# QWTforGithub/CDSegNet

Hardware: AMD Instinct MI355X
Metric: points/sec/node (ScanNet ~120k-pt scenes, 1-step) (higher is better)
Workload: dtype f16

## Files before the change

### cdsegnet_amd/csrc/attention.hip

```cpp
#include <cstdlib>
#include <mutex>
#include <type_traits>

#include "common.h"
#include "prof.h"

namespace {

constexpr int ATTN_ZONES = 5;
constexpr int ATTN_STORE8 = 1 << 30;

struct AttnP {
  const void* q;
  const void* k;
  const void* v;
  const int32_t* q_gidx;
  const int32_t* kv_gidx;
  const int32_t* widx;
  const int32_t* patch_start;
  void* out;
  int ldq, ldk, ldv, ldo;
  int num_heads;
  int num_patches;
  float scale_log2e;
  int flags;
  int nzones;
  int zcnt[ATTN_ZONES];
  int zsplit[ATTN_ZONES];
  int full_patches;
  int zfixed;
  int bulk_max;
};

__host__ __device__ __forceinline__ bool decode_block(const AttnP& p, int B, int& patch, int& head, int& qslice, int& qsplit) {
  const int U = p.num_patches * p.num_heads;
  const int xcd = B & 7;
  int t = B >> 3;
  const int u0 = (int)(((long)U * xcd) >> 3), u1 = (int)(((long)U * (xcd + 1)) >> 3);
  int j0 = 0;
  for (int z = 0; z < p.nzones; ++z) {
    const int fixed = p.zcnt[z];
    const int cnt = fixed >= 0 ? fixed : (u1 - u0) - p.zfixed;
    const int ext = fixed >= 0 ? fixed : p.bulk_max;
    const int split = p.zsplit[z];
    const int nb = ext * split;
    if (t < nb) {
      const int jl = t / split;
      if (jl >= cnt) return false;
      const int u = u0 + j0 + jl;
      patch = u / p.num_heads;
      head = u - patch * p.num_heads;
      qslice = t - jl * split;
      qsplit = split;
      return true;
    }
    t -= nb;
    j0 += cnt;
  }
  return false;
}

constexpr int VT_STRIDE_F32 = 4128;
constexpr int KS_BYTES_F32 = 1024 * 64;
constexpr int SMEM_F32 = KS_BYTES_F32 + 16 * VT_STRIDE_F32;

#ifndef ATTN_FIRST_STATIC
#define ATTN_FIRST_STATIC 1
#endif
#ifndef ATTN_PRIO_OUTSIDE
#define ATTN_PRIO_OUTSIDE 1
#endif
#ifndef ATTN_STORE16
#define ATTN_STORE16 1
#endif
#ifndef ATTN_LEAD_BLOCKS
#define ATTN_LEAD_BLOCKS 0
#endif
#ifndef ATTN_TAIL1_BLOCKS
#define ATTN_TAIL1_BLOCKS 64
#endif
#ifndef ATTN_TAIL2_BLOCKS
#define ATTN_TAIL2_BLOCKS 64
#endif
#ifndef ATTN_ZONE_MIN_UNITS
#define ATTN_ZONE_MIN_UNITS 96
#endif
constexpr int ATTN_THREADS = 512;
constexpr int ATTN_WAVES = ATTN_THREADS / 64;
constexpr int ATTN_RUN = 8;
#ifndef ATTN_BF16_WAVES
#define ATTN_BF16_WAVES 8
#endif
#ifndef ATTN_TILES_IN_FLIGHT
#define ATTN_TILES_IN_FLIGHT 2
#endif
constexpr int BF_WAVES = ATTN_BF16_WAVES, BF_THREADS = 64 * BF_WAVES;
static_assert(BF_WAVES >= ATTN_RUN && BF_WAVES <= 12, "the first run of a block's tiles is pre-assigned to waves 0 .. 7");
constexpr int BF_WAVES_WIDE = 16;
constexpr int KV_STAGE = 1024 * 32;
constexpr int ONES_BYTES = 2048;
constexpr int SMEM_BF16 = 2 * KV_STAGE + ONES_BYTES + 64 + 4096;

__device__ uint4 g_attn_zero[2];

#ifdef CDSEG_ATTN_TIMING
__device__ unsigned long long g_attn_t[8 * 8 * 4096];
#define ATTN_STAMP(x) const unsigned long long x = __builtin_readcyclecounter()
#else
#define ATTN_STAMP(x)
#endif

typedef __attribute__((ext_vector_type(4))) short s16x4_t;
typedef __attribute__((address_space(3))) s16x4_t lds_s16x4_t;

__device__ __forceinline__ f32x16_t qk_tile(const char* k_lane, bf16x8_t qf, const f32x16_t& c0) {
  const bf16x8_t kf = *reinterpret_cast<const bf16x8_t*>(k_lane);
  return mfma_32x32x16_bf16(kf, qf, c0);
}

__device__ __forceinline__ float tile_max(const f32x16_t& s, float m) {
  const float a = fmaxf(fmaxf(s[0], s[1]), s[2]);
  const float b = fmaxf(fmaxf(s[3], s[4]), s[5]);
  const float c = fmaxf(fmaxf(s[6], s[7]), s[8]);
  const float d = fmaxf(fmaxf(s[9], s[10]), s[11]);
  const float e = fmaxf(fmaxf(s[12], s[13]), s[14]);
  return fmaxf(fmaxf(fmaxf(a, b), fmaxf(c, d)), fmaxf(fmaxf(e, s[15]), m));
}

template <bool TAIL, bool FIRST = false>
__device__ __forceinline__ void pv_tile(const f32x16_t& s, int kt, int h, int L, unsigned va, f32x16_t& o) {
  float pr[16];
#pragma unroll
  for (int r = 0; r < 16; ++r) pr[r] = __builtin_amdgcn_exp2f(s[r]);
  if (TAIL) {
#pragma unroll
    for (int r = 0; r < 16; ++r)
      if (kt * 32 + (r & 3) + 8 * (r >> 2) + 4 * h >= L) pr[r] = 0.f;
  }
#pragma unroll
  for (int mf = 0; mf < 2; ++mf) {
    union { bf16x8_t v; uint32_t u[4]; } pf;
#pragma unroll
    for (int j = 0; j < 4; ++j) pf.u[j] = pack_truebf16x2(pr[8 * mf + 2 * j], pr[8 * mf + 2 * j + 1]);
    const s16x4_t v0 = __builtin_amdgcn_ds_read_tr16_b64_v4i16(reinterpret_cast<lds_s16x4_t*>(va + 512 * mf));
    const s16x4_t v1 = __builtin_amdgcn_ds_read_tr16_b64_v4i16(reinterpret_cast<lds_s16x4_t*>(va + 512 * mf + 256));
    const bf16x8_t vf = __builtin_shufflevector(v0, v1, 0, 1, 2, 3, 4, 5, 6, 7);
    if (FIRST && mf == 0) {
      const f32x16_t z = {0, 0, 0, 0, 0, 0, 0, 0, 0, 0, 0, 0, 0, 0, 0, 0};
      o = mfma_32x32x16_truebf16(vf, pf.v, z);
    } else {
      o = mfma_32x32x16_truebf16(vf, pf.v, o);
    }
  }
}

__device__ __forceinline__ float sq8_bf16(const uint4& a) {
  float t = dot2_bf16(a.x, a.x, 0.f);
  t = dot2_bf16(a.y, a.y, t);
  t = dot2_bf16(a.z, a.z, t);
  return dot2_bf16(a.w, a.w, t);
}

template <int WAVES>
__global__ __launch_bounds__(64 * WAVES, 4) void attn_bf16_kernel(AttnP p) {
  constexpr int BF_WAVES = WAVES, BF_THREADS = 64 * WAVES;
  constexpr int NPC = 32 / WAVES;
  extern __shared__ __attribute__((aligned(16))) char smem[];
  char* Ks = smem;
  unsigned* s_next = reinterpret_cast<unsigned*>(smem + 2 * KV_STAGE + ONES_BYTES + 48);
  int* s_qidx = reinterpret_cast<int*>(smem + 2 * KV_STAGE + ONES_BYTES + 64);
  const unsigned lds_base = (unsigned)(uintptr_t)(__attribute__((address_space(3))) char*)smem;

  const int tid = threadIdx.x;
  const int lane = tid & 63;
  const int wave = __builtin_amdgcn_readfirstlane(tid >> 6);
  int patch, head, qslice, qsplit;
  if (!decode_block(p, (int)blockIdx.x, patch, head, qslice, qsplit)) return;
#ifdef CDSEG_ATTN_TIMING
  const unsigned long long rt0 = __builtin_amdgcn_s_memrealtime();
  unsigned long long t_loop = 0, t_first = 0, t_epi = 0, n_tiles = 0;
#endif
  ATTN_STAMP(t0);
  __builtin_amdgcn_s_setprio(3);
  const int ps = p.patch_start[patch];
  const int L = p.patch_start[patch + 1] - ps;
  const int nkt = (L + 31) >> 5;
  const bf16_t* kb = (const bf16_t*)p.k + head * 16;
  const bf16_t* vb = (const bf16_t*)p.v + head * 16;

  const int ql = lane & 31;
  const int h = lane >> 5;
  const int nqt = nkt;
  auto claim = [&]() {
    for (;;) {
      unsigned i = 0;
      if (lane == 0) i = atomicAdd(s_next, 1u);
      i = __builtin_amdgcn_readfirstlane(i);
      if (ATTN_FIRST_STATIC && qsplit == 1) {
        const int t = (int)(i + i / 3u + 1u);
        return t < nqt ? t : -1;
      }
      const int base = (qslice + (int)(i >> 3) * qsplit) * ATTN_RUN;
      if (base >= nqt) return -1;
      const int t = base + (int)(i & 7);
      if (t < nqt) return t;
    }
  };
  auto load_qrow = [&](int t) {
    const int g = s_qidx[min(max(t, 0) * 32 + ql, L - 1)];
    return *reinterpret_cast<const uint4*>((const bf16_t*)p.q + (long)g * p.ldq + head * 16 + h * 8);
  };

  int qt_first = -1;
  uint4 q_first = make_uint4(0, 0, 0, 0);
  {
    const int kip = lane >> 1, hs = lane & 1;
    int gk[NPC];
#pragma unroll
    for (int i = 0; i < NPC; ++i) {
      const int s = (wave + BF_WAVES * i) * 32 + kip;
      gk[i] = s < L ? p.kv_gidx[ps + s] : -1;
    }
    int gq[2] = {0, 0};
    if (wave < ATTN_RUN) {
#pragma unroll
      for (int i = 0; i < 2; ++i) gq[i] = p.q_gidx[ps + min(wave * 128 + i * 64 + lane, L - 1)];
    }
    const int qt_slice0 = qslice * ATTN_RUN + wave;
    int gfirst = 0;
    if (ATTN_FIRST_STATIC && qsplit > 1 && wave < ATTN_RUN) gfirst = p.q_gidx[ps + min(qt_slice0 * 32 + ql, L - 1)];
    if (tid == 0) *s_next = (ATTN_FIRST_STATIC && qsplit > 1) ? 8u : 0u;
    const void* ksrc[NPC];
    const void* vsrc[NPC];
#pragma unroll
    for (int i = 0; i < NPC; ++i) {
      const int s = (wave + BF_WAVES * i) * 32 + kip;
      ksrc[i] = vsrc[i] = (const char*)g_attn_zero + hs * 16;
      if (gk[i] >= 0) {
        ksrc[i] = kb + (long)gk[i] * p.ldk + ((hs ^ ((s >> 3) & 1)) << 3);
        vsrc[i] = vb + (long)gk[i] * p.ldv + (hs << 3);
      }
      asm volatile("" : "+v"(ksrc[i]), "+v"(vsrc[i]));
    }
#pragma unroll
    for (int i = 0; i < NPC; ++i) {
      const int pc = wave + BF_WAVES * i;
      if (pc < nkt) {
        dma16(ksrc[i], lds_base + pc * 1024);
        dma16(vsrc[i], lds_base + KV_STAGE + pc * 1024);
      }
    }
    if (ATTN_FIRST_STATIC && qsplit == 1 && 4 * wave < nqt) {
      qt_first = 4 * wave;
      const int g = __shfl(gq[0], lane & 31, 64);
      q_first = *reinterpret_cast<const uint4*>((const bf16_t*)p.q + (long)g * p.ldq + head * 16 + h * 8);
    } else if (ATTN_FIRST_STATIC && qsplit > 1 && wave < ATTN_RUN && qt_slice0 < nqt) {
      qt_first = qt_slice0;
      q_first = *reinterpret_cast<const uint4*>((const bf16_t*)p.q + (long)gfirst * p.ldq + head * 16 + h * 8);
    }
    if (wave < ATTN_RUN) {
#pragma unroll
      for (int i = 0; i < 2; ++i) s_qidx[wave * 128 + i * 64 + lane] = gq[i];
    }
    for (int w = tid; w < ONES_BYTES / 8; w += BF_THREADS)
      *reinterpret_cast<uint2*>(smem + 2 * KV_STAGE + w * 8) = make_uint2(0x3F80u, 0u);
    asm volatile("s_waitcnt vmcnt(0)" ::: "memory");
    if (LP_IS_F16 && !(p.flags & CDSEG_ATTN_V_BF16)) {
#pragma unroll
      for (int i = 0; i < NPC; ++i) {
        const int pc = wave + BF_WAVES * i;
        if (pc < nkt) {
          uint4* vp = reinterpret_cast<uint4*>(smem + KV_STAGE + pc * 1024 + lane * 16);
          uint4 u = *vp;
          float a0, a1;
          unpack_bf16x2(u.x, a0, a1); u.x = pack_truebf16x2(a0, a1);
          unpack_bf16x2(u.y, a0, a1); u.y = pack_truebf16x2(a0, a1);
          unpack_bf16x2(u.z, a0, a1); u.z = pack_truebf16x2(a0, a1);
          unpack_bf16x2(u.w, a0, a1); u.w = pack_truebf16x2(a0, a1);
          *vp = u;
        }
      }
    }
    __syncthreads();
  }
  if (!ATTN_PRIO_OUTSIDE) __builtin_amdgcn_s_setprio(0);
  ATTN_STAMP(t1);
  const char* k_lane = Ks + ql * 32 + ((h ^ ((ql >> 3) & 1)) << 4);
  const bool v_lane = (lane & 16) == 0;
  const unsigned va0 = v_lane ? lds_base + KV_STAGE + (4 * h + ((lane & 15) >> 2)) * 32 + (lane & 3) * 8
                              : lds_base + 2 * KV_STAGE + (h ? 0 : 128);
  const unsigned vstep = v_lane ? 1024u : 0u;
  const float c = p.scale_log2e;
  const bool tail = (nkt << 5) != L;
  const int nfull = tail ? nkt - 1 : nkt;

  int qt = qt_first;
  uint4 q_cur = q_first;
  if (qt < 0) {
    qt = claim();
    q_cur = load_qrow(qt);
  }
  while (qt >= 0) {
    bf16x8_t qf;
    {
      union { bf16x8_t v; uint32_t u[4]; } qs;
      const uint32_t qr[4] = {q_cur.x, q_cur.y, q_cur.z, q_cur.w};
      if (p.flags & CDSEG_ATTN_Q_PRESCALED) {
#pragma unroll
        for (int j = 0; j < 4; ++j) qs.u[j] = qr[j];
      } else {
#pragma unroll
        for (int j = 0; j < 4; ++j) {
          float lo, hi;
          unpack_bf16x2(qr[j], lo, hi);
          qs.u[j] = pack_bf16x2(lo * c, hi * c);
        }
      }
      qf = qs.v;
      asm volatile("" : "+v"(qf));
    }
    const int qt_nxt = claim();
    const uint4 q_nxt = load_qrow(qt_nxt);
    const int qslot = qt * 32 + ql;
    const bool qvalid = qslot < L;
    int w = p.widx[ps + min(qslot, L - 1)];
    if (!qvalid) w = -1;
    const f32x16_t zero16 = {0, 0, 0, 0, 0, 0, 0, 0, 0, 0, 0, 0, 0, 0, 0, 0};
    auto exp_pv_pass = [&](auto shift_tag, float mrow) {
      constexpr bool SHIFT = decltype(shift_tag)::value;
      const float nm = SHIFT ? -mrow : 0.f;
      const f32x16_t negm = {nm, nm, nm, nm, nm, nm, nm, nm, nm, nm, nm, nm, nm, nm, nm, nm};
      const f32x16_t& c0 = SHIFT ? negm : zero16;
      f32x16_t acc;
      const char* kp = k_lane;
      unsigned va = va0;
      int kt;
      if (ATTN_TILES_IN_FLIGHT == 2 && nfull >= 2) {
        const f32x16_t sa = qk_tile(kp, qf, c0);
        const f32x16_t sb = qk_tile(kp + 1024, qf, c0);
        pv_tile<false, true>(sa, 0, h, L, va, acc);
        pv_tile<false>(sb, 1, h, L, va + 1024, acc);
        kp += 2048;
        va += 2 * vstep;
        kt = 2;
      } else {
        const f32x16_t s0 = qk_tile(kp, qf, c0);
        if (nfull == 0) pv_tile<true, true>(s0, 0, h, L, va, acc);
        else pv_tile<false, true>(s0, 0, h, L, va, acc);
        kp += 1024;
        va += vstep;
        kt = 1;
      }
      for (; ATTN_TILES_IN_FLIGHT == 2 && kt + 1 < nfull; kt += 2) {
        const f32x16_t sa = qk_tile(kp, qf, c0);
        const f32x16_t sb = qk_tile(kp + 1024, qf, c0);
        pv_tile<false>(sa, kt, h, L, va, acc);
        pv_tile<false>(sb, kt + 1, h, L, va + 1024, acc);
        kp += 2048;
        va += 2 * vstep;
      }
      for (; kt < nkt; ++kt) {
        const f32x16_t s = qk_tile(kp, qf, c0);
        if (kt >= nfull) pv_tile<true>(s, kt, h, L, va, acc);
        else pv_tile<false>(s, kt, h, L, va, acc);
        kp += 1024;
        va += vstep;
      }
      return acc;
    };
    if (ATTN_PRIO_OUTSIDE) __builtin_amdgcn_s_setprio(0);
    ATTN_STAMP(tl0);
    f32x16_t o = exp_pv_pass(std::false_type{}, 0.f);
    if (ATTN_PRIO_OUTSIDE) __builtin_amdgcn_s_setprio(2);
#ifdef CDSEG_ATTN_TIMING
    asm volatile("" :: "v"(o[0]), "v"(o[8]));
    const unsigned long long tl1 = __builtin_readcyclecounter();
    t_loop += tl1 - tl0;
    if (n_tiles == 0) t_first = tl0 - t1;
    ++n_tiles;
#endif
    {
      const float den = __shfl(o[8], ql, 64);
      bool fin = true;
#pragma unroll
      for (int r = 0; r < 8; ++r) fin = fin && __builtin_isfinite(o[r]);
      const bool redo = qvalid && (!(den >= 1e-30f && den <= 1e30f) || !fin);
      if (__any(redo)) {
        float m0 = -INFINITY;
        const char* kp = k_lane;
        for (int kt = 0; kt < nkt; ++kt, kp += 1024) {
          f32x16_t s = qk_tile(kp, qf, zero16);
          if (kt >= nfull) {
#pragma unroll
            for (int r = 0; r < 16; ++r)
              if (kt * 32 + (r & 3) + 8 * (r >> 2) + 4 * h >= L) s[r] = -INFINITY;
          }
          m0 = tile_max(s, m0);
        }
        m0 = fmaxf(m0, __shfl_xor(m0, 32, 64));
        o = exp_pv_pass(std::true_type{}, m0);
      }
    }
    const float lsum = __shfl(o[8], ql, 64);
    const float inv = 1.0f / lsum;
    {
      uint2 a, b;
      a.x = pack_bf16x2(o[0] * inv, o[1] * inv);
      a.y = pack_bf16x2(o[2] * inv, o[3] * inv);
      b.x = pack_bf16x2(o[4] * inv, o[5] * inv);
      b.y = pack_bf16x2(o[6] * inv, o[7] * inv);
      if (ATTN_STORE16 && !(p.flags & ATTN_STORE8)) {
        const auto sx = __builtin_amdgcn_permlane32_swap(a.x, b.x, false, false);
        const auto sy = __builtin_amdgcn_permlane32_swap(a.y, b.y, false, false);
        if (w >= 0) {
          bf16_t* orow = (bf16_t*)p.out + (long)w * p.ldo + head * 16 + 8 * h;
          *reinterpret_cast<uint4*>(orow) = make_uint4(sx[0], sy[0], sx[1], sy[1]);
        }
      } else if (w >= 0) {
        bf16_t* orow = (bf16_t*)p.out + (long)w * p.ldo + head * 16 + 4 * h;
        *reinterpret_cast<uint2*>(orow) = a;
        *reinterpret_cast<uint2*>(orow + 8) = b;
      }
    }
    qt = qt_nxt;
    q_cur = q_nxt;
#ifdef CDSEG_ATTN_TIMING
    asm volatile("s_waitcnt vmcnt(0)" ::: "memory");
    t_epi += __builtin_readcyclecounter() - tl1;
#endif
  }
#ifdef CDSEG_ATTN_TIMING
  if (lane == 0 && blockIdx.x < 4096) {
    unsigned long long* d = g_attn_t + ((size_t)blockIdx.x * 8 + wave) * 8;
    d[0] = rt0; d[1] = __builtin_amdgcn_s_memrealtime(); d[2] = t1 - t0; d[3] = t_loop;
    d[4] = __builtin_readcyclecounter() - t0;
    d[5] = t_first; d[6] = t_epi; d[7] = n_tiles;
  }
#endif
}

__global__ __launch_bounds__(ATTN_THREADS) void attn_f32_kernel(AttnP p) {
  extern __shared__ __attribute__((aligned(16))) char smem[];
  char* Ks = smem;
  char* Vt = smem + KS_BYTES_F32;

  const int tid = threadIdx.x;
  const int lane = tid & 63;
  const int wave = tid >> 6;
  int patch, head, qslice, qsplit;
  if (!decode_block(p, (int)blockIdx.x, patch, head, qslice, qsplit)) return;
  const int ps = p.patch_start[patch];
  const int L = p.patch_start[patch + 1] - ps;
  const int nkt = (L + 15) >> 4;
  const int Lp = nkt << 4;
  const float* kb = (const float*)p.k + head * 16;
  const float* vb = (const float*)p.v + head * 16;

  for (int s = tid; s < Lp; s += ATTN_THREADS) {
    uint4 kk[4], vv[4];
#pragma unroll
    for (int i = 0; i < 4; ++i) kk[i] = vv[i] = make_uint4(0, 0, 0, 0);
    if (s < L) {
      const long g = p.kv_gidx[ps + s];
      const uint4* kr = reinterpret_cast<const uint4*>(kb + g * p.ldk);
      const uint4* vr = reinterpret_cast<const uint4*>(vb + g * p.ldv);
#pragma unroll
      for (int i = 0; i < 4; ++i) { kk[i] = kr[i]; vv[i] = vr[i]; }
    }
    const int sw = (s >> 1) & 3;
#pragma unroll
    for (int i = 0; i < 4; ++i) *reinterpret_cast<uint4*>(Ks + s * 64 + ((i ^ sw) << 4)) = kk[i];
#pragma unroll
    for (int i = 0; i < 4; ++i) {
      *reinterpret_cast<uint32_t*>(Vt + (4 * i + 0) * VT_STRIDE_F32 + s * 4) = vv[i].x;
      *reinterpret_cast<uint32_t*>(Vt + (4 * i + 1) * VT_STRIDE_F32 + s * 4) = vv[i].y;
      *reinterpret_cast<uint32_t*>(Vt + (4 * i + 2) * VT_STRIDE_F32 + s * 4) = vv[i].z;
      *reinterpret_cast<uint32_t*>(Vt + (4 * i + 3) * VT_STRIDE_F32 + s * 4) = vv[i].w;
    }
  }
  __syncthreads();

  const int ql = lane & 15;
  const int g4 = lane >> 4;
  const float c = p.scale_log2e;
  const int nqt = (L + 15) >> 4;

  for (int qt = qslice * ATTN_WAVES + wave; qt < nqt; qt += qsplit * ATTN_WAVES) {
    const int qslot = qt * 16 + ql;
    const bool qvalid = qslot < L;
    f32x4_t qf = {0.f, 0.f, 0.f, 0.f};
    if (qvalid) {
      const long g = p.q_gidx[ps + qslot];
      qf = *reinterpret_cast<const f32x4_t*>((const float*)p.q + g * p.ldq + head * 16 + 4 * g4);
    }
    float mloc = -INFINITY;
    for (int kt = 0; kt < nkt; ++kt) {
      const int key = kt * 16 + ql;
      const f32x4_t kf = *reinterpret_cast<const f32x4_t*>(Ks + key * 64 + ((g4 ^ ((key >> 1) & 3)) << 4));
      f32x4_t s = {0.f, 0.f, 0.f, 0.f};
#pragma unroll
      for (int ss = 0; ss < 4; ++ss) s = __builtin_amdgcn_mfma_f32_16x16x4f32(kf[ss], qf[ss], s, 0, 0, 0);
#pragma unroll
      for (int r = 0; r < 4; ++r) {
        float sv = s[r];
        if (kt * 16 + 4 * g4 + r >= L) sv = -INFINITY;
        mloc = fmaxf(mloc, sv);
      }
    }
    float m = fmaxf(mloc, __shfl_xor(mloc, 16, 64));
    m = fmaxf(m, __shfl_xor(m, 32, 64));
    const float mc = m * c;
    f32x4_t o = {0.f, 0.f, 0.f, 0.f};
    float lloc = 0.f;
    for (int kt = 0; kt < nkt; ++kt) {
      const int key = kt * 16 + ql;
      const f32x4_t kf = *reinterpret_cast<const f32x4_t*>(Ks + key * 64 + ((g4 ^ ((key >> 1) & 3)) << 4));
      f32x4_t s = {0.f, 0.f, 0.f, 0.f};
#pragma unroll
      for (int ss = 0; ss < 4; ++ss) s = __builtin_amdgcn_mfma_f32_16x16x4f32(kf[ss], qf[ss], s, 0, 0, 0);
      const f32x4_t vf = *reinterpret_cast<const f32x4_t*>(Vt + ql * VT_STRIDE_F32 + (kt * 16 + 4 * g4) * 4);
#pragma unroll
      for (int r = 0; r < 4; ++r) {
        float pv = __builtin_amdgcn_exp2f(s[r] * c - mc);
        if (kt * 16 + 4 * g4 + r >= L) pv = 0.f;
        lloc += pv;
        o = __builtin_amdgcn_mfma_f32_16x16x4f32(vf[r], pv, o, 0, 0, 0);
      }
    }
    float l = lloc + __shfl_xor(lloc, 16, 64);
    l += __shfl_xor(l, 32, 64);
    const float inv = 1.0f / l;
    if (qvalid) {
      const int w = p.widx[ps + qslot];
      if (w >= 0) {
        float4 ov = make_float4(o[0] * inv, o[1] * inv, o[2] * inv, o[3] * inv);
        *reinterpret_cast<float4*>((float*)p.out + (long)w * p.ldo + head * 16 + 4 * g4) = ov;
      }
    }
  }
}


constexpr int X3_KH = 0, X3_KL = KV_STAGE, X3_V1 = 2 * KV_STAGE, X3_V2 = 3 * KV_STAGE;
constexpr int X3_ONES = 4 * KV_STAGE, X3_ZERO = X3_ONES + ONES_BYTES;
constexpr int SMEM_X3 = X3_ZERO + ONES_BYTES;
#ifndef ATTN_X3_WAVES
#define ATTN_X3_WAVES 8
#endif
#ifndef ATTN_X3_TILES
#define ATTN_X3_TILES 2
#endif
constexpr int X3_WAVES = ATTN_X3_WAVES, X3_THREADS = 64 * X3_WAVES, X3_TILES = ATTN_X3_TILES;
static_assert(X3_WAVES % ATTN_RUN == 0, "whole runs of query tiles per block");
typedef _Float16 x3h2_t __attribute__((ext_vector_type(2)));
typedef _Float16 x3h8_t __attribute__((ext_vector_type(8)));

__device__ __forceinline__ void x3_split_f16(float a, float b, uint32_t& hi, uint32_t& lo) {
  const hw_f32x2_t v = {__builtin_amdgcn_fmed3f(a, -65504.f, 65504.f), __builtin_amdgcn_fmed3f(b, -65504.f, 65504.f)};
  const x3h2_t hh = __builtin_convertvector(v, x3h2_t);
  const hw_f32x2_t r = v - __builtin_convertvector(hh, hw_f32x2_t);
  hi = __builtin_bit_cast(uint32_t, hh);
  lo = __builtin_bit_cast(uint32_t, __builtin_convertvector(r, x3h2_t));
}
__device__ __forceinline__ void x3_split_bf16(float a, float b, uint32_t& p1, uint32_t& p2) {
  p1 = pack_truebf16x2(a, b);
  p2 = pack_truebf16x2(a - __uint_as_float(p1 << 16), b - __uint_as_float(p1 & 0xffff0000u));
}
__device__ __forceinline__ f32x16_t x3_mfma_f16(bf16x8_t a, bf16x8_t b, f32x16_t c) {
  return __builtin_amdgcn_mfma_f32_32x32x16_f16(__builtin_bit_cast(x3h8_t, a), __builtin_bit_cast(x3h8_t, b), c, 0, 0, 0);
}

__device__ __forceinline__ f32x16_t x3_qk_tile(const char* k_lane, bf16x8_t qh, bf16x8_t ql, const f32x16_t& c0) {
  const bf16x8_t kh = *reinterpret_cast<const bf16x8_t*>(k_lane + X3_KH);
  const bf16x8_t kl = *reinterpret_cast<const bf16x8_t*>(k_lane + X3_KL);
  f32x16_t s = x3_mfma_f16(kh, qh, c0);
  s = x3_mfma_f16(kh, ql, s);
  return x3_mfma_f16(kl, qh, s);
}

template <bool TAIL, bool FIRST = false>
__device__ __forceinline__ void x3_pv_tile(const f32x16_t& s, int kt, int h, int L, unsigned va1, unsigned va2, f32x16_t& o) {
  float pr[16];
#pragma unroll
  for (int r = 0; r < 16; ++r) pr[r] = __builtin_amdgcn_exp2f(s[r]);
  if (TAIL) {
#pragma unroll
// ... 311 lines not shown
```

### cdsegnet_amd/csrc/deep.hip

```cpp
#include <atomic>

#include "deep.h"

namespace {

constexpr int DEEP_D = 4;

#ifdef CDSEG_DEEP_TIMING
__device__ unsigned long long g_deep_t[2048 * 16];
#define DT_STAMP(k) if (wave == 0 && lane == 0 && blockIdx.x < 2048) g_deep_t[blockIdx.x * 16 + (k)] = __builtin_readcyclecounter()
#else
#define DT_STAMP(k)
#endif

template <int NCH>
__device__ __forceinline__ int act_off(int row, int chunk) {
  return row * (NCH * 16) + ((chunk ^ (row & 15)) << 4);
}

__device__ __forceinline__ void lds_barrier() {
  asm volatile("s_waitcnt lgkmcnt(0)" ::: "memory");
  __builtin_amdgcn_s_barrier();
}

__device__ __forceinline__ uint4 pack8(const f32x4_t& a, const f32x4_t& b) {
  uint4 r;
  r.x = pack_bf16x2(a[0], a[1]); r.y = pack_bf16x2(a[2], a[3]);
  r.z = pack_bf16x2(b[0], b[1]); r.w = pack_bf16x2(b[2], b[3]);
  return r;
}
__device__ __forceinline__ uint4 pack8_truebf16(const f32x4_t& a, const f32x4_t& b) {
  uint4 r;
  r.x = pack_truebf16x2(a[0], a[1]); r.y = pack_truebf16x2(a[2], a[3]);
  r.z = pack_truebf16x2(b[0], b[1]); r.w = pack_truebf16x2(b[2], b[3]);
  return r;
}

template <int C, int BM>
__device__ __forceinline__ void load_tile(const bf16_t* src, int ld, long m0, long n, char* buf, int tid) {
  constexpr int NCH = C / 8, NT = 2 * C, PT = BM * NCH / NT;
  uint4 r[PT];
#pragma unroll
  for (int i = 0; i < PT; ++i) {
    const int id = i * NT + tid, row = id / NCH, c = id % NCH;
    long m = m0 + row;
    if (m >= n) m = n - 1;
    r[i] = *reinterpret_cast<const uint4*>(src + m * ld + c * 8);
  }
#pragma unroll
  for (int i = 0; i < PT; ++i) {
    const int id = i * NT + tid, row = id / NCH, c = id % NCH;
    *reinterpret_cast<uint4*>(buf + act_off<NCH>(row, c)) = r[i];
  }
}

template <int C, int BM>
__device__ __forceinline__ void load_tile_partials(const float* part, int splits, const float* bias, long m0, long n, char* buf,
                                                   int tid) {
  constexpr int NCH = C / 8, NT = 2 * C, PT = BM * NCH / NT;
  const long plane = n * (long)C;
#pragma unroll
  for (int i = 0; i < PT; ++i) {
    const int id = i * NT + tid, row = id / NCH, c = id % NCH;
    long m = m0 + row;
    if (m >= n) m = n - 1;
    const float* q = part + m * C + c * 8;
    f32x4_t a = *reinterpret_cast<const f32x4_t*>(q), b = *reinterpret_cast<const f32x4_t*>(q + 4);
    for (int s = 1; s < splits; ++s) {
      a = a + *reinterpret_cast<const f32x4_t*>(q + s * plane);
      b = b + *reinterpret_cast<const f32x4_t*>(q + s * plane + 4);
    }
    a = a + *reinterpret_cast<const f32x4_t*>(bias + c * 8);
    b = b + *reinterpret_cast<const f32x4_t*>(bias + c * 8 + 4);
    *reinterpret_cast<uint4*>(buf + act_off<NCH>(row, c)) = pack8(a, b);
  }
}

template <int C, int BM>
__device__ __forceinline__ void product(f32x4_t (&acc)[BM / 16][2], const char* bufX, uint4 (&ring)[DEEP_D][2],
                                        const uint4* wp, int step0, int last_step, int p, int g) {
  constexpr int KS = C / 32, NCH = C / 8, PTS = BM / 16;
  const char* xrow = bufX + p * (NCH * 16);
  bf16x8_t b[2][PTS];
  auto fetch = [&](int s, bf16x8_t (&dst)[PTS]) {
    const char* xs = xrow + (((4 * s + g) ^ p) << 4);
#pragma unroll
    for (int pt = 0; pt < PTS; ++pt) dst[pt] = *reinterpret_cast<const bf16x8_t*>(xs + pt * 16 * (NCH * 16));
  };
  fetch(0, b[0]);
#pragma unroll
  for (int s = 0; s < KS; ++s) {
    const bf16x8_t a0 = __builtin_bit_cast(bf16x8_t, ring[s % DEEP_D][0]);
    const bf16x8_t a1 = __builtin_bit_cast(bf16x8_t, ring[s % DEEP_D][1]);
    if (s + 1 < KS) fetch(s + 1, b[(s + 1) & 1]);
#pragma unroll
    for (int pt = 0; pt < PTS; ++pt) {
      acc[pt][0] = mfma_16x16x32_bf16(a0, b[s & 1][pt], acc[pt][0]);
      acc[pt][1] = mfma_16x16x32_bf16(a1, b[s & 1][pt], acc[pt][1]);
    }
    {
      int nx = step0 + s + DEEP_D;
      nx = nx < last_step ? nx : last_step;
      ring[s % DEEP_D][0] = wp[(nx * 2 + 0) * 64];
      ring[s % DEEP_D][1] = wp[(nx * 2 + 1) * 64];
    }
    __builtin_amdgcn_sched_barrier(0);
  }
}

__device__ __forceinline__ void prime(uint4 (&ring)[DEEP_D][2], const uint4* wp, int step0) {
#pragma unroll
  for (int d = 0; d < DEEP_D; ++d) {
    ring[d][0] = wp[((step0 + d) * 2 + 0) * 64];
    ring[d][1] = wp[((step0 + d) * 2 + 1) * 64];
  }
}

template <int PTS, int NW>
__device__ __forceinline__ void row_stats(const f32x4_t (&v)[PTS][2], float* st1, float* st2, int wave, int p, int g,
                                          float inv_c, float eps, float (&mean)[PTS], float (&rstd)[PTS]) {
  auto across = [&](float* st, int pt) {
    float t = 0.f;
    if constexpr (NW == 16) {
      const float* s0 = st + (16 * pt + p) * NW;
      const f32x4_t a = *reinterpret_cast<const f32x4_t*>(s0), b = *reinterpret_cast<const f32x4_t*>(s0 + 4);
      const f32x4_t c = *reinterpret_cast<const f32x4_t*>(s0 + 8), d = *reinterpret_cast<const f32x4_t*>(s0 + 12);
      t = (((a[0] + a[1]) + (a[2] + a[3])) + ((b[0] + b[1]) + (b[2] + b[3]))) +
          (((c[0] + c[1]) + (c[2] + c[3])) + ((d[0] + d[1]) + (d[2] + d[3])));
    } else if constexpr (NW == 8) {
      const f32x4_t a = *reinterpret_cast<const f32x4_t*>(st + (16 * pt + p) * NW);
      const f32x4_t b = *reinterpret_cast<const f32x4_t*>(st + (16 * pt + p) * NW + 4);
      t = ((a[0] + a[1]) + (a[2] + a[3])) + ((b[0] + b[1]) + (b[2] + b[3]));
    } else {
      const f32x4_t a = *reinterpret_cast<const f32x4_t*>(st + (16 * pt + p) * NW);
      t = (a[0] + a[1]) + (a[2] + a[3]);
    }
    return t;
  };
#pragma unroll
  for (int pt = 0; pt < PTS; ++pt) {
    float s = ((v[pt][0][0] + v[pt][0][1]) + (v[pt][0][2] + v[pt][0][3])) +
              ((v[pt][1][0] + v[pt][1][1]) + (v[pt][1][2] + v[pt][1][3]));
    s += __shfl_xor(s, 16, 64);
    s += __shfl_xor(s, 32, 64);
    if (g == 0) st1[(16 * pt + p) * NW + wave] = s;
  }
  lds_barrier();
#pragma unroll
  for (int pt = 0; pt < PTS; ++pt) mean[pt] = across(st1, pt) * inv_c;
#pragma unroll
  for (int pt = 0; pt < PTS; ++pt) {
    float q = 0.f;
#pragma unroll
    for (int f = 0; f < 2; ++f)
#pragma unroll
      for (int r = 0; r < 4; ++r) {
        const float d = v[pt][f][r] - mean[pt];
        q += d * d;
      }
    q += __shfl_xor(q, 16, 64);
    q += __shfl_xor(q, 32, 64);
    if (g == 0) st2[(16 * pt + p) * NW + wave] = q;
  }
  lds_barrier();
#pragma unroll
  for (int pt = 0; pt < PTS; ++pt) rstd[pt] = 1.0f / sqrtf(across(st2, pt) * inv_c + eps);
}

template <int C, int BM>
struct DeepCfg {
  static constexpr int NW = C / 32, KS = C / 32, NT = 64 * NW;
  static constexpr int ACT = BM * C * 2;
  static constexpr int STAT = 2 * BM * NW * 4;
  static constexpr int HEAD_LDS = ACT + STAT + 9 * C * 4;
  static constexpr int TAIL_LDS = 2 * ACT + STAT + 8 * C * 4;
  static constexpr int HEAD_STEPS = 4 * KS, TAIL_STEPS = 9 * KS;
};

struct DeepHeadP {
  const bf16_t* y; const uint4* wimg; const float* bl; const float* lnp_g; const float* lnp_b; const float* x;
  float* x_out;
  const float* colbias; const float* ln1_g; const float* ln1_b; const float* bqkv; bf16_t* qkv;
  long n; int ldy, ldx, ldxo, ldqkv; float eps;
  int v_bf16;
  int nsplit;
  const float* ypart; const float* ybias; int ysplits;
};

template <int C, int BM>
__global__ __launch_bounds__(2 * C, 2) void deep_head_kernel(DeepHeadP P) {
  using K = DeepCfg<C, BM>;
  constexpr int NW = K::NW, KS = K::KS, NCH = C / 8, NT = K::NT, PTS = BM / 16, S = K::HEAD_STEPS;
  extern __shared__ __attribute__((aligned(16))) char smem[];
  char* bufA = smem;
  float* st1 = reinterpret_cast<float*>(smem + K::ACT);
  float* st2 = st1 + BM * NW;
  float* pr = st2 + BM * NW;
  const int tid = threadIdx.x, lane = tid & 63;
  const int wave = __builtin_amdgcn_readfirstlane(tid >> 6);
  const int p = lane & 15, g = lane >> 4;
  const int c_lo = P.nsplit == 3 ? (int)(blockIdx.x % 3u) : 0, c_hi = P.nsplit == 3 ? c_lo + 1 : 3;
  const long m0 = (long)(P.nsplit == 3 ? blockIdx.x / 3u : blockIdx.x) * BM;
  const uint4* wp = P.wimg + (size_t)wave * S * 128 + lane;
  DT_STAMP(0);
  uint4 ring[DEEP_D][2];
  prime(ring, wp, 0);
  for (int c = tid; c < C; c += NT) {
    pr[c] = P.bl[c]; pr[C + c] = P.lnp_g[c]; pr[2 * C + c] = P.lnp_b[c]; pr[3 * C + c] = P.colbias ? P.colbias[c] : 0.f;
    pr[4 * C + c] = P.ln1_g[c]; pr[5 * C + c] = P.ln1_b[c];
  }
  for (int c = tid; c < 3 * C; c += NT) pr[6 * C + c] = P.bqkv[c];
  if (P.ysplits > 1) load_tile_partials<C, BM>(P.ypart, P.ysplits, P.ybias, m0, P.n, bufA, tid);
  else load_tile<C, BM>(P.y, P.ldy, m0, P.n, bufA, tid);
  const int ch0 = 32 * wave + 8 * g;
  lds_barrier();
  DT_STAMP(1);

  f32x4_t v[PTS][2];
  {
    const f32x4_t b0 = *reinterpret_cast<const f32x4_t*>(pr + ch0), b1 = *reinterpret_cast<const f32x4_t*>(pr + ch0 + 4);
#pragma unroll
    for (int pt = 0; pt < PTS; ++pt) { v[pt][0] = b0; v[pt][1] = b1; }
  }
  product<C, BM>(v, bufA, ring, wp, 0, KS - 1, p, g);
  DT_STAMP(2);
  asm volatile("" ::: "memory");
  __builtin_amdgcn_sched_barrier(0);
  f32x4_t xr[PTS][2];
#pragma unroll
  for (int pt = 0; pt < PTS; ++pt) {
    long m = m0 + 16 * pt + p;
    if (m >= P.n) m = P.n - 1;
#pragma unroll
    for (int f = 0; f < 2; ++f) xr[pt][f] = *reinterpret_cast<const f32x4_t*>(P.x + m * P.ldx + ch0 + 4 * f);
  }
  float mean[PTS], rstd[PTS];
  const float inv_c = 1.0f / C;
  row_stats<PTS, NW>(v, st1, st2, wave, p, g, inv_c, P.eps, mean, rstd);
  DT_STAMP(3);
#pragma unroll
  for (int f = 0; f < 2; ++f) {
    const f32x4_t ga = *reinterpret_cast<const f32x4_t*>(pr + C + ch0 + 4 * f);
    const f32x4_t be = *reinterpret_cast<const f32x4_t*>(pr + 2 * C + ch0 + 4 * f);
    const f32x4_t tb = *reinterpret_cast<const f32x4_t*>(pr + 3 * C + ch0 + 4 * f);
#pragma unroll
    for (int pt = 0; pt < PTS; ++pt) {
#pragma unroll
      for (int r = 0; r < 4; ++r) v[pt][f][r] = ((v[pt][f][r] - mean[pt]) * rstd[pt] * ga[r] + be[r]) + xr[pt][f][r] + tb[r];
      const long m = m0 + 16 * pt + p;
      if (m < P.n && c_lo == 0) *reinterpret_cast<f32x4_t*>(P.x_out + m * P.ldxo + ch0 + 4 * f) = v[pt][f];
    }
  }
  DT_STAMP(4);
  row_stats<PTS, NW>(v, st1, st2, wave, p, g, inv_c, P.eps, mean, rstd);
  DT_STAMP(5);
  prime(ring, wp, KS * (1 + c_lo));
  {
    const f32x4_t ga0 = *reinterpret_cast<const f32x4_t*>(pr + 4 * C + ch0), ga1 = *reinterpret_cast<const f32x4_t*>(pr + 4 * C + ch0 + 4);
    const f32x4_t be0 = *reinterpret_cast<const f32x4_t*>(pr + 5 * C + ch0), be1 = *reinterpret_cast<const f32x4_t*>(pr + 5 * C + ch0 + 4);
#pragma unroll
    for (int pt = 0; pt < PTS; ++pt) {
      f32x4_t h0, h1;
#pragma unroll
      for (int r = 0; r < 4; ++r) {
        h0[r] = (v[pt][0][r] - mean[pt]) * rstd[pt] * ga0[r] + be0[r];
        h1[r] = (v[pt][1][r] - mean[pt]) * rstd[pt] * ga1[r] + be1[r];
      }
      *reinterpret_cast<uint4*>(bufA + act_off<NCH>(16 * pt + p, 4 * wave + g)) = pack8(h0, h1);
    }
  }
  lds_barrier();
  DT_STAMP(6);
#pragma unroll 1
  for (int c = c_lo; c < c_hi; ++c) {
    f32x4_t a[PTS][2];
    {
      const f32x4_t b0 = *reinterpret_cast<const f32x4_t*>(pr + 6 * C + c * C + ch0);
      const f32x4_t b1 = *reinterpret_cast<const f32x4_t*>(pr + 6 * C + c * C + ch0 + 4);
#pragma unroll
      for (int pt = 0; pt < PTS; ++pt) { a[pt][0] = b0; a[pt][1] = b1; }
    }
    int po = p;
    asm volatile("" : "+v"(po));
    product<C, BM>(a, bufA, ring, wp, KS * (1 + c), S - 1, po, g);
    DT_STAMP(7 + 2 * c);
#pragma unroll
    for (int pt = 0; pt < PTS; ++pt) {
      const long m = m0 + 16 * pt + p;
      if (m < P.n)
        *reinterpret_cast<uint4*>(P.qkv + m * P.ldqkv + c * C + ch0) =
            (LP_IS_F16 && c == 2 && P.v_bf16) ? pack8_truebf16(a[pt][0], a[pt][1]) : pack8(a[pt][0], a[pt][1]);
    }
    DT_STAMP(8 + 2 * c);
  }
}

struct DeepTailP {
  const bf16_t* o; const uint4* wimg; const float* bp; const float* ln_g; const float* ln_b; const float* b1;
  const float* b2; const float* x_in; float* x; bf16_t* xc;
  long n; int ldo, ldx, ldxi, ldxc; float eps;
  int nsplit;
  float* part;
};

template <int C, int BM>
__global__ __launch_bounds__(2 * C, 2) void deep_tail_kernel(DeepTailP P) {
  using K = DeepCfg<C, BM>;
  constexpr int NW = K::NW, KS = K::KS, NCH = C / 8, NT = K::NT, PTS = BM / 16, S = K::TAIL_STEPS;
  extern __shared__ __attribute__((aligned(16))) char smem[];
  char* bufA = smem;
  char* bufU = smem + K::ACT;
  float* st1 = reinterpret_cast<float*>(smem + 2 * K::ACT);
  float* st2 = st1 + BM * NW;
  float* pr = st2 + BM * NW;
  const int tid = threadIdx.x, lane = tid & 63;
  const int wave = __builtin_amdgcn_readfirstlane(tid >> 6);
  const int p = lane & 15, g = lane >> 4;
  const int nsp = P.nsplit, js = nsp > 1 ? (int)(blockIdx.x % (unsigned)nsp) : 0;
  const int j_lo = js * (4 / nsp), j_hi = j_lo + 4 / nsp;
  const long m0 = (long)(nsp > 1 ? blockIdx.x / (unsigned)nsp : blockIdx.x) * BM;
  const uint4* wp = P.wimg + (size_t)wave * S * 128 + lane;
  DT_STAMP(0);
  uint4 ring[DEEP_D][2];
  prime(ring, wp, 0);
  for (int c = tid; c < C; c += NT) {
    pr[c] = P.bp[c]; pr[C + c] = P.ln_g[c]; pr[2 * C + c] = P.ln_b[c]; pr[3 * C + c] = P.b2[c];
  }
  for (int c = tid; c < 4 * C; c += NT) pr[4 * C + c] = P.b1[c];
  load_tile<C, BM>(P.o, P.ldo, m0, P.n, bufA, tid);
  const int ch0 = 32 * wave + 8 * g;
  f32x4_t acc2[PTS][2];
  {
    f32x4_t xr[PTS][2];
#pragma unroll
    for (int pt = 0; pt < PTS; ++pt) {
      long m = m0 + 16 * pt + p;
      if (m >= P.n) m = P.n - 1;
#pragma unroll
      for (int f = 0; f < 2; ++f) xr[pt][f] = *reinterpret_cast<const f32x4_t*>(P.x_in + m * P.ldxi + ch0 + 4 * f);
    }
    lds_barrier();
    DT_STAMP(1);
    const f32x4_t b0 = *reinterpret_cast<const f32x4_t*>(pr + ch0), b1 = *reinterpret_cast<const f32x4_t*>(pr + ch0 + 4);
#pragma unroll
    for (int pt = 0; pt < PTS; ++pt) { acc2[pt][0] = b0; acc2[pt][1] = b1; }
    product<C, BM>(acc2, bufA, ring, wp, 0, S - 1, p, g);
    DT_STAMP(2);
#pragma unroll
    for (int pt = 0; pt < PTS; ++pt) { acc2[pt][0] += xr[pt][0]; acc2[pt][1] += xr[pt][1]; }
  }
  {
    float mean[PTS], rstd[PTS];
    DT_STAMP(3);
    row_stats<PTS, NW>(acc2, st1, st2, wave, p, g, 1.0f / C, P.eps, mean, rstd);
    DT_STAMP(4);
    const f32x4_t ga0 = *reinterpret_cast<const f32x4_t*>(pr + C + ch0), ga1 = *reinterpret_cast<const f32x4_t*>(pr + C + ch0 + 4);
    const f32x4_t be0 = *reinterpret_cast<const f32x4_t*>(pr + 2 * C + ch0), be1 = *reinterpret_cast<const f32x4_t*>(pr + 2 * C + ch0 + 4);
#pragma unroll
    for (int pt = 0; pt < PTS; ++pt) {
      f32x4_t h0, h1;
#pragma unroll
      for (int r = 0; r < 4; ++r) {
        h0[r] = (acc2[pt][0][r] - mean[pt]) * rstd[pt] * ga0[r] + be0[r];
        h1[r] = (acc2[pt][1][r] - mean[pt]) * rstd[pt] * ga1[r] + be1[r];
      }
      *reinterpret_cast<uint4*>(bufA + act_off<NCH>(16 * pt + p, 4 * wave + g)) = pack8(h0, h1);
    }
  }
  if (js) {
    prime(ring, wp, KS * (1 + 2 * j_lo));
    const f32x4_t z = {0.f, 0.f, 0.f, 0.f};
#pragma unroll
    for (int pt = 0; pt < PTS; ++pt) { acc2[pt][0] = z; acc2[pt][1] = z; }
  }
  lds_barrier();
  DT_STAMP(5);
#ifdef CDSEG_DEEP_TIMING
  unsigned long long dt_fc1 = 0, dt_gelu = 0, dt_fc2 = 0;
#endif
#pragma unroll 1
  for (int j = j_lo; j < j_hi; ++j) {
#ifdef CDSEG_DEEP_TIMING
    const unsigned long long q0 = __builtin_readcyclecounter();
#endif
    f32x4_t acc1[PTS][2];
    {
      const f32x4_t b0 = *reinterpret_cast<const f32x4_t*>(pr + 4 * C + j * C + ch0);
      const f32x4_t b1 = *reinterpret_cast<const f32x4_t*>(pr + 4 * C + j * C + ch0 + 4);
#pragma unroll
      for (int pt = 0; pt < PTS; ++pt) { acc1[pt][0] = b0; acc1[pt][1] = b1; }
    }
    int po = p;
    asm volatile("" : "+v"(po));
    product<C, BM>(acc1, bufA, ring, wp, KS * (1 + 2 * j), S - 1, po, g);
#ifdef CDSEG_DEEP_TIMING
    const unsigned long long q1 = __builtin_readcyclecounter();
#endif
    if (j > j_lo) lds_barrier();
#pragma unroll
    for (int pt = 0; pt < PTS; ++pt) {
      gelu_lp4(acc1[pt][0]);
      gelu_lp4(acc1[pt][1]);
      *reinterpret_cast<uint4*>(bufU + act_off<NCH>(16 * pt + p, 4 * wave + g)) = pack8(acc1[pt][0], acc1[pt][1]);
    }
    lds_barrier();
#ifdef CDSEG_DEEP_TIMING
    const unsigned long long q2 = __builtin_readcyclecounter();
#endif
    product<C, BM>(acc2, bufU, ring, wp, KS * (2 + 2 * j), S - 1, p, g);
#ifdef CDSEG_DEEP_TIMING
    dt_fc1 += q1 - q0; dt_gelu += q2 - q1; dt_fc2 += __builtin_readcyclecounter() - q2;
#endif
  }
#ifdef CDSEG_DEEP_TIMING
  DT_STAMP(6);
  if (wave == 0 && lane == 0 && blockIdx.x < 2048) {
    g_deep_t[blockIdx.x * 16 + 8] = dt_fc1; g_deep_t[blockIdx.x * 16 + 9] = dt_gelu; g_deep_t[blockIdx.x * 16 + 10] = dt_fc2;
  }
#endif
  if (nsp > 1) {
#pragma unroll
    for (int pt = 0; pt < PTS; ++pt) {
      const long m = m0 + 16 * pt + p;
      if (m < P.n) {
        float* dst = P.part + ((size_t)js * P.n + m) * C + ch0;
        *reinterpret_cast<f32x4_t*>(dst) = acc2[pt][0];
        *reinterpret_cast<f32x4_t*>(dst + 4) = acc2[pt][1];
      }
    }
  } else {
    const f32x4_t b0 = *reinterpret_cast<const f32x4_t*>(pr + 3 * C + ch0), b1 = *reinterpret_cast<const f32x4_t*>(pr + 3 * C + ch0 + 4);
#pragma unroll
    for (int pt = 0; pt < PTS; ++pt) {
      const long m = m0 + 16 * pt + p;
      if (m < P.n) {
        const f32x4_t o0 = acc2[pt][0] + b0, o1 = acc2[pt][1] + b1;
        *reinterpret_cast<f32x4_t*>(P.x + m * P.ldx + ch0) = o0;
        *reinterpret_cast<f32x4_t*>(P.x + m * P.ldx + ch0 + 4) = o1;
        if (P.xc) *reinterpret_cast<uint4*>(P.xc + m * P.ldxc + ch0) = pack8(o0, o1);
      }
    }
  }
  DT_STAMP(7);
}

__global__ __launch_bounds__(256) void deep_tail_reduce_kernel(const float* __restrict__ part, int nsplit, long n, int C,
                                                               const float* __restrict__ b2, float* x, int ldx, bf16_t* xc,
                                                               int ldxc) {
  const long u = (long)blockIdx.x * blockDim.x + threadIdx.x;
  const int per_row = C / 8;
  if (u >= n * per_row) return;
  const long m = u / per_row;
  const int ch = (int)(u % per_row) * 8;
  f32x4_t a = *reinterpret_cast<const f32x4_t*>(part + m * C + ch), b = *reinterpret_cast<const f32x4_t*>(part + m * C + ch + 4);
  for (int js = 1; js < nsplit; ++js) {
    const float* src = part + ((size_t)js * n + m) * C + ch;
    a += *reinterpret_cast<const f32x4_t*>(src);
    b += *reinterpret_cast<const f32x4_t*>(src + 4);
  }
  a += *reinterpret_cast<const f32x4_t*>(b2 + ch);
  b += *reinterpret_cast<const f32x4_t*>(b2 + ch + 4);
  *reinterpret_cast<f32x4_t*>(x + m * ldx + ch) = a;
  *reinterpret_cast<f32x4_t*>(x + m * ldx + ch + 4) = b;
  if (xc) *reinterpret_cast<uint4*>(xc + m * ldxc + ch) = pack8(a, b);
}

struct DeepPackP {
  const bf16_t* w;
  uint4* img;
  int ld, C, S, step0, row_base, col_base;
};

__global__ void deep_pack_kernel(DeepPackP p) {
  const int KS = p.C / 32, NW = p.C / 32;
  const int u = blockIdx.x * blockDim.x + threadIdx.x;
  if (u >= NW * KS * 128) return;
  const int lane = u & 63, f = (u >> 6) & 1, s = (u >> 7) % KS, w = (u >> 7) / KS;
  const int q = lane >> 4, i = lane & 15;
  const long row = p.row_base + 32 * w + 8 * (i >> 2) + 4 * f + (i & 3);
  const long col = p.col_base + 32 * s + 8 * q;
  p.img[((size_t)(w * p.S + p.step0 + s) * 2 + f) * 64 + lane] = *reinterpret_cast<const uint4*>(p.w + row * p.ld + col);
}

int pack_phase(const void* w, int ld, int C, int S, int step0, int row_base, int col_base, void* img, hipStream_t s) {
  DeepPackP p;
  p.w = (const bf16_t*)w; p.img = (uint4*)img; p.ld = ld; p.C = C; p.S = S; p.step0 = step0; p.row_base = row_base;
  p.col_base = col_base;
  const int units = (C / 32) * (C / 32) * 128;
  hipLaunchKernelGGL(deep_pack_kernel, dim3((units + 255) / 256), dim3(256), 0, s, p);
  return hipGetLastError() == hipSuccess ? CDSEG_OK : CDSEG_ERR_LAUNCH;
}

inline int pick_bm(long n) { return (n + 127) / 128 >= 160 ? 128 : 32; }

inline int pick_head_split(long n, int C, int bm) {
  const long tiles = (n + bm - 1) / bm;
  return (bm == 32 && C >= cdseg_knob("CDSEG_DEEP_SPLIT_MIN_C", 512) && tiles * 3 <= cdseg_knob("CDSEG_DEEP_SPLIT_MAX_WGS", 256)) ? 3 : 1;
}
inline int pick_tail_split(long n, int C, int bm, size_t ws_bytes) {
  const long tiles = (n + bm - 1) / bm;
  if (bm != 32 || C < cdseg_knob("CDSEG_DEEP_SPLIT_MIN_C", 512)) return 1;
  const long cap = cdseg_knob("CDSEG_DEEP_SPLIT_MAX_WGS", 256);
  for (int k = 4; k >= 2; k >>= 1)
    if (tiles * k <= cap && (size_t)k * n * C * 4 <= ws_bytes) return k;
  return 1;
}

template <int C, int BM>
int launch_head(const DeepHeadP& p, hipStream_t s) {
  constexpr int lds = DeepCfg<C, BM>::HEAD_LDS;
  static std::atomic<bool> attr_done{false};
  if (!attr_done) {
    if (hipFuncSetAttribute((const void*)deep_head_kernel<C, BM>, hipFuncAttributeMaxDynamicSharedMemorySize, lds) != hipSuccess)
      return CDSEG_ERR_LAUNCH;
    attr_done = true;
  }
  hipLaunchKernelGGL((deep_head_kernel<C, BM>), dim3((unsigned)((p.n + BM - 1) / BM) * (unsigned)p.nsplit), dim3(2 * C), lds, s, p);
  CDSEG_CHECK_LAUNCH();
  return CDSEG_OK;
}

template <int C, int BM>
int launch_tail(const DeepTailP& p, hipStream_t s) {
  constexpr int lds = DeepCfg<C, BM>::TAIL_LDS;
  static std::atomic<bool> attr_done{false};
  if (!attr_done) {
    if (hipFuncSetAttribute((const void*)deep_tail_kernel<C, BM>, hipFuncAttributeMaxDynamicSharedMemorySize, lds) != hipSuccess)
      return CDSEG_ERR_LAUNCH;
    attr_done = true;
  }
  hipLaunchKernelGGL((deep_tail_kernel<C, BM>), dim3((unsigned)((p.n + BM - 1) / BM) * (unsigned)p.nsplit), dim3(2 * C), lds, s, p);
  CDSEG_CHECK_LAUNCH();
  if (p.nsplit > 1) {
    const long units = p.n * (C / 8);
    hipLaunchKernelGGL(deep_tail_reduce_kernel, dim3((unsigned)((units + 255) / 256)), dim3(256), 0, s, p.part, p.nsplit, p.n, C,
                       p.b2, p.x, p.ldx, p.xc, p.ldxc);
    CDSEG_CHECK_LAUNCH();
  }
  return CDSEG_OK;
}

}

#ifdef CDSEG_DEEP_TIMING
extern "C" int cdseg_debug_deep_timing(unsigned long long* host_dst, size_t count) {
  return hipMemcpyFromSymbol(host_dst, HIP_SYMBOL(g_deep_t), count * sizeof(unsigned long long)) == hipSuccess ? 0 : -2;
}
#endif

bool deep_supported(int channels) { return channels == 128 || channels == 256 || channels == 512; }

int deep_pack(int C, const void* wl, const void* wqkv, void* head_img, const void* wp, const void* w1, const void* w2,
              void* tail_img, hipStream_t s) {
  if (!deep_supported(C)) return CDSEG_ERR_UNSUPPORTED;
  const int KS = C / 32;
  int rc;
  if (head_img) {
    if (!wl || !wqkv) return CDSEG_ERR_ARG;
    if ((rc = pack_phase(wl, C, C, 4 * KS, 0, 0, 0, head_img, s)) != CDSEG_OK) return rc;
    for (int c = 0; c < 3; ++c)
      if ((rc = pack_phase(wqkv, C, C, 4 * KS, KS * (1 + c), c * C, 0, head_img, s)) != CDSEG_OK) return rc;
  }
  if (tail_img) {
    if (!wp || !w1 || !w2) return CDSEG_ERR_ARG;
    if ((rc = pack_phase(wp, C, C, 9 * KS, 0, 0, 0, tail_img, s)) != CDSEG_OK) return rc;
    for (int j = 0; j < 4; ++j) {
      if ((rc = pack_phase(w1, C, C, 9 * KS, KS * (1 + 2 * j), j * C, 0, tail_img, s)) != CDSEG_OK) return rc;
      if ((rc = pack_phase(w2, 4 * C, C, 9 * KS, KS * (2 + 2 * j), 0, j * C, tail_img, s)) != CDSEG_OK) return rc;
    }
  }
  return CDSEG_OK;
}

int deep_head(const void* y, int ldy, const void* head_img, const float* bl, const float* lnp_g, const float* lnp_b,
              const float* x, int ldx, float* x_out, int ldxo, const float* colbias, const float* ln1_g, const float* ln1_b, float eps, const float* bqkv, void* qkv,
              int ldqkv, long n, int channels, int qkv_flags, hipStream_t s, const float* ypart, int ysplits, const float* ybias) {
  DeepHeadP p;
  p.ypart = ypart; p.ybias = ybias; p.ysplits = (ypart && ybias && ysplits > 1) ? ysplits : 1;
  if (p.ysplits > 1 && ((((uintptr_t)ypart) | ((uintptr_t)ybias)) & 15)) return CDSEG_ERR_ARG;
  p.v_bf16 = (qkv_flags & CDSEG_ATTN_V_BF16) ? 1 : 0;
  p.y = (const bf16_t*)y; p.wimg = (const uint4*)head_img; p.bl = bl; p.lnp_g = lnp_g; p.lnp_b = lnp_b; p.x = x;
  p.x_out = x_out; p.ldxo = ldxo;
  p.colbias = colbias; p.ln1_g = ln1_g; p.ln1_b = ln1_b; p.bqkv = bqkv; p.qkv = (bf16_t*)qkv;
  p.n = n; p.ldy = ldy; p.ldx = ldx; p.ldqkv = ldqkv; p.eps = eps;
  const int bm = channels == 512 ? 32 : cdseg_knob("CDSEG_DEEP_BM", pick_bm(n));
  p.nsplit = (cdseg_knob("CDSEG_DEEP_SPLIT", 1) && (const float*)x_out != x) ? pick_head_split(n, channels, bm) : 1;
  if (channels == 128) return bm == 128 ? launch_head<128, 128>(p, s) : launch_head<128, 32>(p, s);
  if (channels == 256) return bm == 128 ? launch_head<256, 128>(p, s) : launch_head<256, 32>(p, s);
  if (channels == 512) return launch_head<512, 32>(p, s);
  return CDSEG_ERR_UNSUPPORTED;
}

int deep_tail(const void* o, int ldo, const void* tail_img, const float* bp, const float* ln_g, const float* ln_b, float eps,
              const float* b1, const float* b2, const float* x_in, int ldxi, float* x, int ldx, void* xc, int ldxc, long n,
              int channels, void* ws, size_t ws_bytes, hipStream_t s) {
  DeepTailP p;
  p.o = (const bf16_t*)o; p.wimg = (const uint4*)tail_img; p.bp = bp; p.ln_g = ln_g; p.ln_b = ln_b; p.b1 = b1; p.b2 = b2;
  p.x_in = x_in; p.ldxi = ldxi;
  p.x = x; p.xc = (bf16_t*)xc; p.n = n; p.ldo = ldo; p.ldx = ldx; p.ldxc = ldxc; p.eps = eps;
  const int bm = channels == 512 ? 32 : cdseg_knob("CDSEG_DEEP_BM", pick_bm(n));
  p.nsplit = (ws && cdseg_knob("CDSEG_DEEP_SPLIT", 1) && !(((uintptr_t)ws) & 15)) ? pick_tail_split(n, channels, bm, ws_bytes) : 1;
  p.part = (float*)ws;
  if (channels == 128) return bm == 128 ? launch_tail<128, 128>(p, s) : launch_tail<128, 32>(p, s);
  if (channels == 256) return bm == 128 ? launch_tail<256, 128>(p, s) : launch_tail<256, 32>(p, s);
  if (channels == 512) return launch_tail<512, 32>(p, s);
  return CDSEG_ERR_UNSUPPORTED;
}
```

### cdsegnet_amd/engine.py

```python
import math
import struct
import os
import threading

import numpy as np
import torch

from . import _lib, ops
from ._lib import CdsegError, DuplicateVoxelsError

CURVES = ("z", "z-trans", "hilbert", "hilbert-trans")


def _pooling_depth(stride):
    return (math.ceil(stride) - 1).bit_length()


class _ShareEvents(threading.local):
    on = False


SHARE_EVENTS = _ShareEvents()


def _shared(cache, key, build):
    ent = cache.get(key)
    cur = ops.current_stream_id()
    if ent is None:
        val = build()
        ent = cache[key] = (val, cur, ops.record_event() if (cur is not None and SHARE_EVENTS.on) else None)
    elif ent[1] != cur and ent[2] is not None:
        ops.wait_event(ent[2])
    return ent[0]


def _cut(lazy, cache, key):
    lz = lazy.pop(key, None)
    if lz is not None:
        sid, parts = lz
        vals = tuple(A[o:o + c] if shape is None else A[o:o + c].view(shape) for A, o, c, shape in parts)
        cache[key] = (vals[0] if len(vals) == 1 else vals, sid, None)


FUSED_CURVE_SORT = True

class Level:

    def __init__(self, cum, depth, n, grid, batch, code4, offs_host, lazy=None):
        self.cum, self.depth, self.n = cum, depth, n
        self._gbc = (grid, batch, code4) if lazy is None else None
        self._gbc_lazy = lazy
        self.offs_host = offs_host
        self.parent = None
        self._order = {}
        self._nbr = {}
        self._pad = {}
        self._slots = {}
        self._pad_lazy = {}
        self._slot_lazy = {}
        self._order_lazy = {}
        self._nbr_lazy = {}

    def _cut_gbc(self):
        A, go, bo, Q, co = self._gbc_lazy
        n = self.n
        self._gbc = (A[go:go + 3 * n].view(n, 3), A[bo:bo + n], Q[co:co + 4 * n].view(4, n))
        self._gbc_lazy = None
        return self._gbc

    @property
    def grid(self):
        return (self._gbc or self._cut_gbc())[0]

    @property
    def batch(self):
        return (self._gbc or self._cut_gbc())[1]

    @property
    def code4(self):
        return (self._gbc or self._cut_gbc())[2]

    def order(self, curve):
        if curve == 0:
            return None
        if self._order_lazy:
            _cut(self._order_lazy, self._order, curve)

        def build():
            nb = len(self.offs_host) - 1
            end_bit = min(64, 3 * self.depth + max(1, nb.bit_length()))
            return ops.sort_pairs(self.code4[curve], None, end_bit=end_bit)[1]
        return _shared(self._order, curve, build)

    def nbr(self, ksize, kmajor=False):
        if self._nbr_lazy:
            _cut(self._nbr_lazy, self._nbr, (ksize, kmajor))

        def build():
            if self.parent is not None:
                par, (cluster, seg) = self.parent
                return ops.nbr_table_from_info(self.grid, cluster, par.nbr(3, True), self.child_info(), par.n, self.depth,
                                               ksize, kmajor)
            return ops.nbr_table(self.code4[0], self.grid, self.batch, self.depth, ksize, kmajor)
        return _shared(self._nbr, (ksize, kmajor), build)

    def child_info(self):
        if self._nbr_lazy:
            _cut(self._nbr_lazy, self._nbr, "child_info")

        def build():
            par, (_, seg) = self.parent
            return ops.child_info(self.code4[0], seg, par.n)
        return _shared(self._nbr, "child_info", build)

    def pad_host_py(self, patch_size, enable_flash):
        offs = self.offs_host
        counts = [b - a for a, b in zip(offs[:-1], offs[1:])]
        K = int(patch_size) if enable_flash else int(min(min(counts), patch_size))
        offs_pad, patch_start = [0], []
        for c in counts:
            pc = (c + K - 1) // K * K if c > K else c
            patch_start.extend(range(offs_pad[-1], offs_pad[-1] + pc, K))
            offs_pad.append(offs_pad[-1] + pc)
        patch_start.append(offs_pad[-1])
        return K, offs, offs_pad, patch_start

    def pad_host(self, patch_size, enable_flash):
        K, offs, offs_pad, patch_start = self.pad_host_py(patch_size, enable_flash)
        return (K, np.asarray(offs, dtype=np.int32), np.asarray(offs_pad, dtype=np.int32),
                np.asarray(patch_start, dtype=np.int32))

    def set_pad(self, key, K, offs_pad, patch_start, offs_dev, offs_pad_dev, patch_start_dev):
        lens = [int(b) - int(a) for a, b in zip(patch_start[:-1], patch_start[1:])]
        self._pad[key] = (K, int(offs_pad[-1]), offs_dev, offs_pad_dev, patch_start_dev,
                          max(lens), float(sum(v * v for v in lens)))

    def pad(self, patch_size, enable_flash):
        key = (patch_size, enable_flash)
        lz = self._pad_lazy.pop(key, None) if self._pad_lazy else None
        if lz is not None:
            K, n_pad, max_len, sum_l2, A, oo, op, ot, nb, npatch = lz
            self._pad[key] = (K, n_pad, A[oo:oo + nb + 1], A[op:op + nb + 1], A[ot:ot + npatch + 1], max_len, sum_l2)
        if key not in self._pad:
            K, offs, offs_pad, patch_start = self.pad_host(patch_size, enable_flash)
            dev = self.grid.device
            up = torch.tensor(np.concatenate([offs, offs_pad, patch_start]), device=dev)
            a, b = len(offs), len(offs) + len(offs_pad)
            self.set_pad(key, K, offs_pad, patch_start, up[:a], up[a:b], up[b:])
        return self._pad[key]

    def slots(self, curve, patch_size, enable_flash):
        lz = self._slot_lazy.pop((curve, patch_size, enable_flash), None) if self._slot_lazy else None
        if lz is not None:
            A, go, wo, n_pad, sid = lz
            self._slots[(curve, patch_size, enable_flash)] = ((A[go:go + n_pad], A[wo:wo + n_pad]), sid, None)

        def build():
            K, n_pad, offs, offs_pad = self.pad(patch_size, enable_flash)[:4]
            return ops.pad_plan(self.order(curve), offs, offs_pad, K, n_pad)
        return _shared(self._slots, (curve, patch_size, enable_flash), build)


class Plan:
    def __init__(self):
        self.levels = {}
        self.links = {}
        self._finish = None
        self._link_lazy = {}

    def finish_pads(self):
        fin, self._finish = self._finish, None
        if fin is not None:
            fin()

    def link(self, a, b):
        if self._link_lazy:
            _cut(self._link_lazy, self.links, (a, b))

        def build():
            la, lb = self.levels[a], self.levels[b]
            if a > 0 and (0, a) in self.links and (0, b) in self.links:
                (cl0a, seg0a), (cl0b, seg0b) = self.link(0, a), self.link(0, b)
                return ops.link_derive(cl0a, seg0a, la.n, cl0b, seg0b, lb.n)
            cluster, seg, _ = ops.pool_level(la.code4[0], 3 * (lb.cum - la.cum))
            return (cluster, seg)
        return _shared(self.links, (a, b), build)


class State:

    def __init__(self, level, x, xc, curves):
        self.level, self.x, self.xc, self.curves = level, x, xc, curves
        self.parent = None


class _HeadsInFp32:
    T = torch.float32

    def __init__(self, eng):
        bb, self.device, self.w = eng.model.backbone, eng.device, {}
        for name in ("n_head", "c_head"):
            mod = getattr(bb, "_" + name, None)
            if isinstance(mod, torch.nn.Linear):
                self.w[name + ".w"] = mod.weight.detach().to(device=eng.device, dtype=torch.float32).contiguous()
                self.w[name + ".b"] = (mod.bias.detach().to(device=eng.device, dtype=torch.float32).contiguous()
                                       if mod.bias is not None else None)

    def prepare(self, device):
        assert device == self.device

    def _fit(self, st, exact=False):
        return Engine._fit(self, st, exact)


class Engine:
    PRECISIONS = ("bf16", "bf16+head", "fp16", "fp16+head", "fp32", "fp32x3")

    def __init__(self, model, precision="bf16", variant=None):
        if precision not in self.PRECISIONS:
            raise ValueError(precision)
        self.model, self.precision = model, precision
        bb = model.backbone
        if getattr(bb, "condition", False) and not (bb.c_num_stages == 3 and bb.n_num_stages == 5):
            raise ValueError(f"conditional PT-v3m1 needs 3 c-branch and 5 n-branch stages (ptv3.py:1785-1794), got "
                             f"{bb.c_num_stages} / {bb.n_num_stages}")
        self.variant = variant or ("f16" if precision.startswith("fp16") or precision == "fp32x3" else "bf16")
        self.x3 = precision == "fp32x3"
        self.T = torch.float32 if precision in ("fp32", "fp32x3") else ops.LP_DTYPES[self.variant]
        self.device = None
        self.w = None
        self.rng_offset = 0
        self._rng_seed = None
        self.use_native_blocks = True
        self.fold_attn_scale = True
        self.speculate_depth = True
        self._depth_hint = {}
        self.count_saturation = False
        self.saturation_count = None
        self.saturation_checked = 0
        self._sat = None
        self.exact_attention_core = False
        self._pad_keys = None
        self.native_plan = True
        self._plan_specs = {}
        self._tb_cache = {}
        self.eager_kernel_maps = True
        self._side = {}
        self.fork_stage = int(os.environ["CDSEG_FORK_STAGE"]) if os.environ.get("CDSEG_FORK_STAGE") else 2
        self._work_lock = threading.Lock()
        self._tls = threading.local()
        self.attn_work = 0.0
        self.conv_bytes = 0.0
        self.conv_deep_bytes = 0.0
        self.attn_bytes = 0.0
        self.hi = frozenset(("n_head", "c_head")) if precision.endswith("+head") else frozenset()
        self._twin = None

    def prepare(self, device):
        if self.w is not None and self.device == device:
            return
        with _lib.use(self.variant):
            self._prepare(device)

    def _prepare(self, device):
        self.device = device
        T = self.T
        w = {}
        self._blocks_to_describe = []

        def f32(t):
            return t.detach().to(device=device, dtype=torch.float32).contiguous()

        def lin(mod, pre):
            w[pre + ".w"] = mod.weight.detach().to(device=device, dtype=T).contiguous()
            w[pre + ".b"] = f32(mod.bias) if mod.bias is not None else None

        self.q_prescaled = T != torch.float32 and self.fold_attn_scale

        def lin_q(mod, pre, scale, rows):
            if not self.q_prescaled:
                return lin(mod, pre)
            f = float(scale) * 1.4426950408889634
            wt = mod.weight.detach().to(device=device, dtype=torch.float32).clone()
            wt[:rows] *= f
            w[pre + ".w"] = wt.to(T).contiguous()
            if mod.bias is not None:
                b = f32(mod.bias).clone()
                b[:rows] *= f
                w[pre + ".b"] = b
            else:
                w[pre + ".b"] = None

        def conv(mod, pre):
            w[pre + ".w"] = mod.weight.detach().reshape(mod.weight.shape[0], -1).to(device=device, dtype=T).contiguous()
            w[pre + ".b"] = f32(mod.bias) if mod.bias is not None else None
            if self.x3 and mod.kernel_size == 3 and hasattr(ops, "split16"):
                w[pre + ".w_hi"], w[pre + ".w_lo"] = ops.split16(w[pre + ".w"])
                cout = w[pre + ".w"].shape[0]
                if mod.in_channels == cout and cout in (32, 64) and hasattr(ops, "subm_conv3_f32"):
                    w[pre + ".wimg_hi"] = ops.subm_conv3_pack(w[pre + ".w_hi"])
                    w[pre + ".wimg_lo"] = ops.subm_conv3_pack(w[pre + ".w_lo"])
                if ("x3.scale", cout) not in w:
                    w[("x3.scale", cout)] = torch.full((cout,), 1.0 / 2048.0, dtype=torch.float32, device=device)
                    w[("x3.zero", cout)] = torch.zeros(cout, dtype=torch.float32, device=device)
            k, cin, cout = mod.kernel_size, mod.in_channels, mod.out_channels
            if (k == 3 and cin == cout and hasattr(ops, "subm_conv3_pack") and
                    ops.subm_conv3_ok(torch.empty((1, cin), dtype=T, device="meta"))):
                w[pre + ".wimg"] = ops.subm_conv3_pack(w[pre + ".w"])

        def ln(mod, pre):
            w[pre + ".g"], w[pre + ".b"] = f32(mod.weight), f32(mod.bias)

        def bn(mod, pre):
            scale = mod.weight.detach().double() / torch.sqrt(mod.running_var.detach().double() + mod.eps)
            shift = mod.bias.detach().double() - mod.running_mean.detach().double() * scale
            w[pre + ".scale"], w[pre + ".shift"] = f32(scale), f32(shift)

        self.block_desc = {}

        def block(mod, pre):
            self._blocks_to_describe.append((mod, pre))
            conv(mod.cpe[0], pre + ".cpe0")
            lin(mod.cpe[1], pre + ".cpe1")
            ln(mod.cpe[2], pre + ".cpe2")
            ln(mod.norm1[0], pre + ".norm1")
            lin_q(mod.attn.qkv, pre + ".qkv", mod.attn.scale, mod.channels)
            lin(mod.attn.proj, pre + ".proj")
            ln(mod.norm2[0], pre + ".norm2")
            lin(mod.mlp[0].fc1, pre + ".fc1")
            lin(mod.mlp[0].fc2, pre + ".fc2")

        def stem(mod, pre):
            cw = mod.stem.conv.weight.detach()
            cout, cin = cw.shape[0], cw.shape[-1]
            cpad = (cin + 7) // 8 * 8
            wp = torch.zeros(cout, cw.shape[1] ** 3, cpad, dtype=torch.float32)
            wp[:, :, :cin] = cw.reshape(cout, -1, cin).float().cpu()
            w[pre + ".w"] = wp.reshape(cout, -1).to(device=device, dtype=T).contiguous()
            w[pre + ".cpad"] = cpad
            if cw.shape[1] == 5 and cpad == 8 and hasattr(ops, "stem5_pack") and ops.stem5_ok(cout, T):
                w[pre + ".wimg"] = ops.stem5_pack(w[pre + ".w"])
            bn(mod.stem.norm, pre + ".bn")

        def pool(mod, pre):
            lin(mod.proj, pre + ".proj")
            bn(mod.norm[0], pre + ".bn")
            pw = w[pre + ".proj.w"]
            if hasattr(ops, "pool_fused_ok") and ops.pool_fused_ok(pw.shape[1], pw.shape[0], T):
                w[pre + ".proj.wimg"] = ops.pool_fused_pack(pw)

        def unpool(mod, pre):
            lin(mod.proj[0], pre + ".proj")
            bn(mod.proj[1], pre + ".proj_bn")
            lin(mod.proj_skip[0], pre + ".skip")
            bn(mod.proj_skip[1], pre + ".skip_bn")
            if mod.skip_connection_mode == "cat":
                f = (2 ** -0.5 if mod.skip_connection_scale else 1.0)
                if mod.skip_connection_scale_i is not None:
                    f *= 0.8 ** (int(mod.skip_connection_scale_i) - 1)
                wc = mod.proj_cat[0].weight.detach().float()
                c = wc.shape[0]
                w[pre + ".cat_a.w"] = (wc[:, :c] * f).to(device=device, dtype=T).contiguous()
                w[pre + ".cat_b.w"] = wc[:, c:].to(device=device, dtype=T).contiguous()
                w[pre + ".cat.b"] = f32(mod.proj_cat[0].bias)

        bb = self.model.backbone
        stem(bb._n_embedding, "n_emb")
        for s in range(bb.n_num_stages):
            enc = getattr(bb._n_enc, f"enc{s}")
            if s > 0:
                pool(enc.down, f"n_enc{s}.down")
            for name, mod in enc._modules.items():
                if name.startswith("block"):
                    block(mod, f"n_enc{s}.{name}")
        for s in range(bb.n_num_stages - 1):
            dec = getattr(bb._n_dec, f"dec{s}")
            unpool(dec.up, f"n_dec{s}.up")
            for name, mod in dec._modules.items():
                if name.startswith("block"):
                    block(mod, f"n_dec{s}.{name}")
        if isinstance(bb._n_head, torch.nn.Linear):
            lin(bb._n_head, "n_head")
        if bb.condition:
            stem(bb._c_embedding, "c_emb")
            tw, tb, toff = [], [], {}
            off = 0
            for s in range(bb.c_num_stages):
                enc = getattr(bb._c_enc, f"enc{s}")
                if s > 0:
                    pool(enc.down, f"c_enc{s}.down")
                for name, mod in enc._modules.items():
                    if name.startswith("block"):
                        block(mod, f"c_enc{s}.{name}")
                        if bb.T_dim != -1:
                            tw.append(f32(mod.t_mlp.weight))
                            tb.append(f32(mod.t_mlp.bias))
                            toff[f"c_enc{s}.{name}"] = (off, off + mod.channels)
                            off += mod.channels
            for s in range(bb.c_num_stages - 1):
                dec = getattr(bb._c_dec, f"dec{s}")
                unpool(dec.up, f"c_dec{s}.up")
                for name, mod in dec._modules.items():
                    if name.startswith("block"):
                        block(mod, f"c_dec{s}.{name}")
                        if bb.T_dim != -1:
                            tw.append(f32(mod.t_mlp.weight))
                            tb.append(f32(mod.t_mlp.bias))
                            toff[f"c_dec{s}.{name}"] = (off, off + mod.channels)
                            off += mod.channels
            if isinstance(bb._c_head, torch.nn.Linear):
                lin(bb._c_head, "c_head")
            if bb.T_dim != -1:
                w["t.fc1.w"], w["t.fc1.b"] = f32(bb.fc_t1.weight), f32(bb.fc_t1.bias)
                w["t.fc2.w"], w["t.fc2.b"] = f32(bb.fc_t2.weight), f32(bb.fc_t2.bias)
                w["t.mlp.w"], w["t.mlp.b"] = torch.cat(tw).contiguous(), torch.cat(tb).contiguous()
                w["t.table"] = f32(self.model.t_emb_table)
                self.t_slices = toff
            cb = bb._tm_dec0.cross_block2
            conv(cb.q_cpe[0], "x.q_cpe0"); lin(cb.q_cpe[1], "x.q_cpe1"); ln(cb.q_cpe[2], "x.q_cpe2")
            conv(cb.kv_cpe[0], "x.kv_cpe0"); lin(cb.kv_cpe[1], "x.kv_cpe1"); ln(cb.kv_cpe[2], "x.kv_cpe2")
            ln(cb.q_norm1[0], "x.q_norm1"); ln(cb.kv_norm1[0], "x.kv_norm1"); ln(cb.q_norm2[0], "x.q_norm2")
            lin_q(cb.attn.q, "x.q", cb.attn.scale, cb.q_channels); lin(cb.attn.kv, "x.kv"); lin(cb.attn.proj, "x.proj")
            lin(cb.mlp[0].fc1, "x.fc1"); lin(cb.mlp[0].fc2, "x.fc2")
            if cb.tm_feat != 1.0:
                c = cb.q_channels
                w["x.feat_scale"] = torch.full((c,), cb.tm_feat, dtype=torch.float32, device=device)
                w["x.feat_zero"] = torch.zeros(c, dtype=torch.float32, device=device)
            elif (hasattr(ops, "block_rr_pack") and ops.block_rr_ok(cb.q_channels, T) and cb.q_channels in ops.DEEP_CHANNELS
                  and w["x.fc1.w"].shape[0] == 4 * cb.q_channels):
                _, w["x.tail_img"] = ops.block_rr_pack(cb.q_channels, None, None, w["x.proj.w"], w["x.fc1.w"], w["x.fc2.w"])
        self.w = w
        self._tb_cache = {}
        if T == torch.float16:
            flags = [(~torch.isfinite(t)).any() for t in w.values() if torch.is_tensor(t) and t.dtype == torch.float16]
            if flags and bool(torch.stack(flags).any().item()):
                bad = [k for k, t in w.items() if torch.is_tensor(t) and t.dtype == torch.float16 and not bool(torch.isfinite(t).all())]
                raise CdsegError(f"weights outside IEEE half's range (|w| > 65504) in {bad[:4]}: run this checkpoint with "
                                 f"precision='bf16+head' (bfloat16 trunk, fp32's exponent range)")
        for mod, pre in self._blocks_to_describe:
            if hasattr(ops, "block_rr_pack") and ops.block_rr_ok(mod.channels, T) and w[pre + ".fc1.w"].shape[0] == 4 * mod.channels:
                himg, w[pre + ".tail_img"] = ops.block_rr_pack(
                    mod.channels, w[pre + ".cpe1.w"], w[pre + ".qkv.w"], w[pre + ".proj.w"], w[pre + ".fc1.w"], w[pre + ".fc2.w"])
                if ops.block_rr_head_on(mod.channels):
                    w[pre + ".head_img"] = himg
        self.native_blocks = hasattr(ops, "block_forward") and self.use_native_blocks and not self.x3
        if self.native_blocks:
            for mod, pre in self._blocks_to_describe:
                t = dict(cpe_conv_w=w[pre + ".cpe0.w"], cpe_conv_b=w[pre + ".cpe0.b"], cpe_lin_w=w[pre + ".cpe1.w"],
                         cpe_lin_b=w[pre + ".cpe1.b"], cpe_ln_g=w[pre + ".cpe2.g"], cpe_ln_b=w[pre + ".cpe2.b"],
                         norm1_g=w[pre + ".norm1.g"], norm1_b=w[pre + ".norm1.b"], qkv_w=w[pre + ".qkv.w"],
                         qkv_b=w[pre + ".qkv.b"], proj_w=w[pre + ".proj.w"], proj_b=w[pre + ".proj.b"],
                         norm2_g=w[pre + ".norm2.g"], norm2_b=w[pre + ".norm2.b"], fc1_w=w[pre + ".fc1.w"],
# ... 158 lines not shown
        slot = {}

        def pads_pin(count):
            pt, _, sl = self._pin("pads", count, ring=4)
            slot["s"] = sl
            return pt

        off, info = call.finish(m, offs_rows, pads_pin)
        slot["s"]["ev"] = ops.record_event()
        f32, f64 = call.f32, call.f64
        it = iter(off)
        sizes = [n] + m
        lv0 = plan.levels[0] = Level(0, depth, n, grid0, bat0, code0, offs0)
        levels = [lv0]
        for i in range(nlev):
            go, bo, co = next(it), next(it), next(it)
            mi, cum = m[i], all_cum[i + 1]
            lv = Level(cum, depth - cum, mi, None, None, None, offs_rows[i + 1], lazy=(f32, go, bo, f64, co))
            plan.levels[cum] = lv
            levels.append(lv)
            plan.links[(0, cum)] = ((cl_all[i], seg_all[i]), sid, None)
        for a, b in links:
            clo, sgo = next(it), next(it)
            plan._link_lazy[(all_cum[a], all_cum[b])] = (sid, ((f32, clo, sizes[a], None), (f32, sgo, sizes[b] + 1, None)))
        for i in range(nlev):
            if all_cum[i + 1] - all_cum[i] == 1:
                levels[i].parent = (levels[i + 1], plan.link(all_cum[i], all_cum[i + 1]))
        for i, lv in enumerate(levels):
            lv._nbr_lazy[(3, True)] = (sid, ((f32, next(it), 27 * sizes[i], (27, sizes[i])),))
        for i, lv in enumerate(levels):
            o = next(it)
            if o >= 0:
                lv._nbr_lazy["child_info"] = (sid, ((f64, o, sizes[i + 1], None),))
        pos = next(it)
        nc = len(used)
        for k, c in enumerate(used):
            lv0._order[c] = (orders0[k], sid, None)
        for i in range(1, nlev + 1):
            for k, c in enumerate(used):
                levels[i]._order_lazy[c] = (sid, ((f32, pos + k * sizes[i], sizes[i], None),))
            pos += nc * sizes[i]
        q = 5
        per = []
        for i, lv in enumerate(levels):
            for key in self._pad_keys:
                oo, op, ot = next(it), next(it), next(it)
                K, n_pad, npatch, max_len, bits = info[q:q + 5]
                q += 5
                lv._pad_lazy[key] = (K, n_pad, max_len, struct.unpack("d", struct.pack("q", bits))[0], f32, oo, op, ot, nb,
                                     npatch)
                per.append((lv, key, n_pad))
        gb, wb = next(it), next(it)
        pos = 0
        for lv, key, n_pad in per:
            for c in curves:
                lv._slot_lazy[(c,) + key] = (f32, gb + pos, wb + pos, n_pad, sid)
                pos += n_pad
        return plan

    def build_plan(self, grid, offset_dev, offset_host, n, _exact_depth=None, while_device_works=None, defer_pads=False):
        bb = self.model.backbone
        nb = len(offset_host) if offset_host is not None else int(offset_dev.numel())
        on_gpu = grid.is_cuda
        hint = self._depth_hint.get(grid.device) if _exact_depth is None else None
        gmax_host = gmax_dev = None
        if _exact_depth is not None:
            depth = _exact_depth
        elif hint is not None and on_gpu and self.speculate_depth:
            depth = hint
            gmax_host = getattr(self._tls, "gmax_pin", None)
            if gmax_host is None:
                gmax_host = self._tls.gmax_pin = torch.empty(1, dtype=torch.int64, pin_memory=True)
        else:
            gmax_dev = ops.grid_max(grid)
            depth = int(gmax_dev.item()).bit_length()
            self._depth_hint[grid.device] = depth
        assert depth * 3 + nb.bit_length() <= 63, "serialization code does not fit int64"
        assert depth <= 16, "grid extent exceeds 2^16 voxels per axis"
        end_bit = min(64, 3 * depth + max(1, nb.bit_length()))

        def cum_depths(strides):
            cum, d = [0], depth
            for s in strides:
                pd = _pooling_depth(s)
                if pd > d:
                    pd = 0
                d -= pd
                cum.append(cum[-1] + pd)
            return cum

        n_cum = cum_depths(bb.n_stride)
        c_cum = cum_depths(bb.c_stride) if bb.condition else [0]
        all_cum = sorted(set(n_cum + c_cum))
        coarse = [c for c in all_cum if c > 0]
        if on_gpu and self.native_plan and (gmax_host is not None or _exact_depth is not None):
            ent = self._native_spec(depth, n_cum, c_cum, all_cum, end_bit)
            if ent is not None:
                return self._build_plan_native(ent, grid, offset_dev, offset_host, n, depth, end_bit, gmax_host, n_cum, c_cum,
                                               all_cum, while_device_works)
        if offset_host is None:
            offset_host = [int(v) for v in offset_dev.cpu().tolist()]
        if gmax_dev is None:
            gmax_dev = ops.grid_max(grid)
            if gmax_host is not None:
                gmax_host.copy_(gmax_dev, non_blocking=True)
        last_idx = (offset_dev.to(torch.int32) - 1) if coarse else None
        batch = ops.offset2batch(offset_dev, n)
        zc = ops.encode(grid, batch, depth, "z")
        zs, perm0 = ops.sort_pairs(zc, None, end_bit=end_bit)
        grid0, bat0 = ops.plan_gather_grid(grid, perm0, zs, depth)
        code0 = ops.encode4(grid0, bat0, depth)

        plan = Plan()
        plan.perm0, plan.n_cum, plan.c_cum, plan.depth = perm0, n_cum, c_cum, depth
        offs0 = [0] + [int(v) for v in offset_host]
        lv0 = plan.levels[0] = Level(0, depth, n, grid0, bat0, code0, offs0)
        used = sorted({CURVES.index(o) for o in bb.order} - {0})

        def sort_level0_curves():
            if used and end_bit + 2 <= 64 and FUSED_CURVE_SORT and not all(c in lv0._order for c in used):
                srt = ops.sort_curves(code0, used, end_bit)
                for k, c in enumerate(used):
                    lv0._order[c] = (srt[k], ops.current_stream_id(), None)

        if coarse:
            dev = grid.device
            cl_all, seg_all, meta = ops.pool_levels(zs, [3 * cum for cum in coarse], last_idx)
            tmp = [(cl_all[i], seg_all[i]) for i in range(len(coarse))]
            if on_gpu:
                mt, mnp, _ = self._pin("meta", meta.numel())
                mt[:meta.numel()].copy_(meta, non_blocking=True)
                ev = ops.record_event()
                sort_level0_curves()
                if while_device_works is not None:
                    while_device_works()
                    while_device_works = None
                ev.synchronize()
                flat = mnp[:meta.numel()].tolist()
            else:
                flat = meta.cpu().tolist()
            if gmax_host is not None:
                true_depth = int(gmax_host.item()).bit_length()
                self._depth_hint[grid.device] = true_depth
                if true_depth != depth:
                    return self.build_plan(grid, offset_dev, offset_host, n, _exact_depth=true_depth, defer_pads=defer_pads)
                gmax_host = None
            if flat[-1]:
                raise DuplicateVoxelsError(
                    f"input has {flat[-1]} duplicate voxels (points sharing (batch, grid_coord) with another "
                    f"point): the model expects one point per voxel - voxelise first (GridSample)", flat[-1])
            meta_h = [flat[i * (1 + nb):(i + 1) * (1 + nb)] for i in range(len(coarse))]
            host = [r[0] for r in meta_h] + [v for r in meta_h for v in r[1:]]
            for i, cum in enumerate(coarse):
                m = host[i]
                e = host[len(coarse) + i * nb: len(coarse) + (i + 1) * nb]
                g, b, c4 = ops.pool_gather(tmp[i][1], m, n, cum, grid0, bat0, code0)
                plan.levels[cum] = Level(cum, depth - cum, m, g, b, c4, [0] + [v + 1 for v in e])
                plan.links[(0, cum)] = ((tmp[i][0], tmp[i][1]), ops.current_stream_id(), None)
            cums = sorted(plan.levels)
            for fa, co in zip(cums[:-1], cums[1:]):
                if co - fa == 1:
                    plan.levels[fa].parent = (plan.levels[co], plan.link(fa, co))
            if on_gpu and self.eager_kernel_maps:
                share, SHARE_EVENTS.on = SHARE_EVENTS.on, False
                try:
                    for cum in reversed(cums):
                        plan.levels[cum].nbr(3, True)
                finally:
                    SHARE_EVENTS.on = share
            if used:
                sort_level0_curves()
                derived = ops.coarse_orders([t[0] for t in tmp], [lv0.order(c) for c in used], host[:len(coarse)])
                for i, cum in enumerate(coarse):
                    for k, c in enumerate(used):
                        plan.levels[cum]._order[c] = (derived[i][k], ops.current_stream_id(), None)
        if while_device_works is not None:
            while_device_works()
        if gmax_host is not None:
            true_depth = int(gmax_dev.item()).bit_length()
            self._depth_hint[grid.device] = true_depth
            if true_depth != depth:
                return self.build_plan(grid, offset_dev, offset_host, n, _exact_depth=true_depth, defer_pads=defer_pads)
        def finish_pads():
            if self._pad_keys is None:
                self._pad_keys = self._collect_pad_keys()
            pad_keys = self._pad_keys
            flat_up, meta = [], []
            for cum, lv in plan.levels.items():
                for key in pad_keys:
                    K, offs, offs_pad, patch_start = lv.pad_host_py(*key)
                    meta.append((lv, key, K, offs_pad, patch_start, len(offs), len(offs_pad), len(patch_start)))
                    flat_up += offs
                    flat_up += offs_pad
                    flat_up += patch_start
            if on_gpu:
                pt, pnp, slot = self._pin("pads", len(flat_up), ring=4)
                pnp[:len(flat_up)] = flat_up
                up = torch.empty(len(flat_up), dtype=torch.int32, device=grid.device)
                up.copy_(pt[:len(flat_up)], non_blocking=True)
                slot["ev"] = ops.record_event()
            else:
                up = torch.tensor(flat_up, dtype=torch.int32, device=grid.device)
            pos = 0
            for lv, key, K, offs_pad, patch_start, la, lb, lc in meta:
                lv.set_pad(key, K, offs_pad, patch_start, up[pos:pos + la], up[pos + la:pos + la + lb],
                           up[pos + la + lb:pos + la + lb + lc])
                pos += la + lb + lc
            curves = sorted({CURVES.index(o) for o in bb.order})
            items, where = [], []
            for cum, lv in plan.levels.items():
                for key in pad_keys:
                    K, n_pad, offs, offs_pad = lv.pad(*key)[:4]
                    for c in curves:
                        items.append((lv.order(c), offs, offs_pad, K, n_pad))
                        where.append((lv, (c,) + key))
            cur = ops.current_stream_id()
            for (lv, key), gw in zip(where, ops.pad_plan_batch(items, nb)):
                lv._slots[key] = (gw, cur, None)

        if defer_pads and on_gpu:
            plan._finish = finish_pads
        else:
            finish_pads()
        return plan

    def _buf(self, rows, cols, dtype):
        return torch.empty((rows, cols), dtype=dtype, device=self.device)

    FUSE_LN_MAX_C = 512

    def _count_conv(self, n, c, esz):
        if c <= 64 and esz == 2:
            self.conv_bytes += 2.0 * n * c * esz + 27.0 * 4 * n + 27.0 * c * c * esz
        else:
            self.conv_deep_bytes += 2.0 * n * c * esz + 27.0 * 4 * n + 27.0 * c * c * esz

    def _conv3(self, xc, pre, lv, y):
        w = self.w
        self._count_conv(lv.n, xc.shape[1], xc.element_size())
        if (pre + ".w_hi") in w and y.dtype == torch.float32:
            cout = w[pre + ".w"].shape[0]
            sc, ze = w[("x3.scale", cout)], w[("x3.zero", cout)]
            xh, xl = ops.split16(xc)
            nbr = lv.nbr(3, True)
            if (pre + ".wimg_hi") in w and ops.subm_conv3_ok(xh) and y.stride(0) == y.shape[1]:
                ops.subm_conv3_f32(xh, w[pre + ".wimg_hi"], w[pre + ".b"], nbr, y)
                ops.subm_conv3_f32(xh, w[pre + ".wimg_lo"], None, nbr, y, out_scale=1.0 / 2048.0, accumulate=True)
                ops.subm_conv3_f32(xl, w[pre + ".wimg_hi"], None, nbr, y, out_scale=1.0 / 2048.0, accumulate=True)
                return
            ops.gemm(xh, w[pre + ".w_hi"], y, bias=w[pre + ".b"], nbr=nbr, nbr_kmajor=True, kvol=27)
            ops.gemm(xh, w[pre + ".w_lo"], y, scale=sc, shift=ze, res=y, nbr=nbr, nbr_kmajor=True, kvol=27)
            ops.gemm(xl, w[pre + ".w_hi"], y, scale=sc, shift=ze, res=y, nbr=nbr, nbr_kmajor=True, kvol=27)
            return
        if (pre + ".wimg") in w and ops.subm_conv3_ok(xc):
            ops.subm_conv3(xc, w[pre + ".wimg"], w[pre + ".b"], lv.nbr(3, True), y)
        else:
            ops.gemm(xc, w[pre + ".w"], y, bias=w[pre + ".b"], nbr=lv.nbr(3, True), nbr_kmajor=True, kvol=27)

    def _cpe(self, st, pre, xc, tbias=None, next_norm=None):
        w, lv = self.w, st.level
        c = st.x.shape[1]
        y = self._buf(lv.n, c, self.T)
        self._conv3(xc, pre + "0", lv, y)
        h = self._buf(lv.n, c, self.T) if next_norm else None
        if c <= self.FUSE_LN_MAX_C:
            ops.gemm(y, w[pre + "1.w"], st.x, bias=w[pre + "1.b"], ln_pre=(w[pre + "2.g"], w[pre + "2.b"]), res=st.x,
                     colbias=tbias, ln_post=(w[next_norm + ".g"], w[next_norm + ".b"]) if next_norm else None,
                     ln_out=h)
            return h
        y2 = self._buf(lv.n, c, torch.float32)
        ops.gemm(y, w[pre + "1.w"], y2, bias=w[pre + "1.b"])
        ops.layernorm(y2, w[pre + "2.g"], w[pre + "2.b"], st.x, res=st.x, colbias=tbias)
        if next_norm:
            ops.layernorm(st.x, w[next_norm + ".g"], w[next_norm + ".b"], h)
        return h

    def _mlp(self, st, pre_norm, pre_fc, h=None):
        w = self.w
        n, c = st.x.shape
        if h is None:
            h = self._buf(n, c, self.T)
            ops.layernorm(st.x, w[pre_norm + ".g"], w[pre_norm + ".b"], h)
        hid = w[pre_fc + "1.w"].shape[0]
        if ops.mlp_fused_ok(h, hid):
            st.xc = self._buf(n, c, self.T)
            ops.mlp_fused(h, w[pre_fc + "1.w"], w[pre_fc + "1.b"], w[pre_fc + "2.w"], w[pre_fc + "2.b"], st.x, st.xc)
            return
        u = self._buf(n, hid, self.T)
        ops.gemm(h, w[pre_fc + "1.w"], u, bias=w[pre_fc + "1.b"], act=ops.ACT_GELU)
        if self.T == torch.float32:
            ops.gemm(u, w[pre_fc + "2.w"], st.x, bias=w[pre_fc + "2.b"], res=st.x)
            st.xc = st.x
        else:
            st.xc = self._buf(n, c, self.T)
            ops.gemm(u, w[pre_fc + "2.w"], st.x, bias=w[pre_fc + "2.b"], res=st.x, out2=st.xc)

    def run_block(self, st, mod, pre, tbias=None):
        w, lv = self.w, st.level
        n, c = st.x.shape
        if self.native_blocks:
            att = mod.attn
            gidx, widx = lv.slots(st.curves[att.order_index], att.patch_size, att.enable_flash)
            _, _, _, _, patch_start, max_len, sum_l2 = lv.pad(att.patch_size, att.enable_flash)
            self.attn_work += 64.0 * att.num_heads * sum_l2
            self.attn_bytes += 4.0 * n * c * st.xc.element_size()
            self._count_conv(n, c, st.xc.element_size())
            desc = self.block_desc[pre]
            xc_out = st.x if self.T == torch.float32 else self._buf(n, c, self.T)
            sb = self._scratch_bytes.get((pre, n))
            if sb is None:
                if len(self._scratch_bytes) > 4096:
                    self._scratch_bytes.clear()
                sb = self._scratch_bytes[(pre, n)] = ops.block_scratch_bytes(desc, n)
            ops.block_forward(desc, n, st.x, st.xc, xc_out, tbias, lv.nbr(3, True), gidx, widx, patch_start,
                              patch_start.numel() - 1, max_len, self.scratch(sb), sat_counter=self._sat)
            if self._sat is not None:
                self.saturation_checked += n * c * (5 if xc_out is not st.x else 4)
            st.xc = xc_out
            return
        qkv = self._buf(n, 3 * c, self.T)
        aflags = ops.ATTN_Q_PRESCALED if self.q_prescaled else 0
        deep_rr = ((pre + ".head_img") in w and (pre + ".tail_img") in w and not ops.cpe_head_fused_ok(st.xc)
                   and hasattr(ops, "cpe_head_rr2"))
        xs = None
        if deep_rr:
            y = self._buf(n, c, self.T)
            self._conv3(st.xc, pre + ".cpe0", lv, y)
            xs = self._buf(n, c, torch.float32)
            ops.cpe_head_rr2(y, w[pre + ".head_img"], w[pre + ".cpe1.b"], (w[pre + ".cpe2.g"], w[pre + ".cpe2.b"]), st.x, xs,
                             tbias, (w[pre + ".norm1.g"], w[pre + ".norm1.b"]), w[pre + ".qkv.b"], qkv,
                             qkv_flags=ops.ATTN_V_BF16)
            aflags |= ops.ATTN_V_BF16
        elif ops.cpe_head_fused_ok(st.xc):
            y = self._buf(n, c, self.T)
            self._conv3(st.xc, pre + ".cpe0", lv, y)
            if (pre + ".head_img") in w:
                ops.cpe_head_rr(y, w[pre + ".head_img"], w[pre + ".cpe1.b"], (w[pre + ".cpe2.g"], w[pre + ".cpe2.b"]), st.x,
                                tbias, (w[pre + ".norm1.g"], w[pre + ".norm1.b"]), w[pre + ".qkv.b"], qkv)
            else:
                ops.cpe_head_fused(y, w[pre + ".cpe1.w"], w[pre + ".cpe1.b"], (w[pre + ".cpe2.g"], w[pre + ".cpe2.b"]), st.x,
                                   tbias, (w[pre + ".norm1.g"], w[pre + ".norm1.b"]), w[pre + ".qkv.w"], w[pre + ".qkv.b"], qkv,
                                   qkv_flags=ops.ATTN_V_BF16)
                aflags |= ops.ATTN_V_BF16
        else:
            h = self._cpe(st, pre + ".cpe", st.xc, tbias, next_norm=pre + ".norm1")
            ops.gemm(h, w[pre + ".qkv.w"], qkv, bias=w[pre + ".qkv.b"])
        att = mod.attn
        curve = st.curves[att.order_index]
        gidx, widx = lv.slots(curve, att.patch_size, att.enable_flash)
        _, _, _, _, patch_start, max_len, sum_l2 = lv.pad(att.patch_size, att.enable_flash)
        self._add_work(64.0 * att.num_heads * sum_l2, 4.0 * n * c * qkv.element_size())
        o = self._buf(n, c, self.T)
        if self.exact_attention_core and self.T != torch.float32:
            q32 = qkv.float()
            o32 = self._buf(n, c, torch.float32)
            if aflags & ops.ATTN_V_BF16 and self.T == torch.float16:
                q32[:, 2 * c:] = qkv[:, 2 * c:].view(torch.bfloat16).float()
            ops.attention(q32[:, :c], q32[:, c:2 * c], q32[:, 2 * c:], gidx, gidx, widx, patch_start, att.num_heads,
                          max_len, att.scale, o32, work=0.0, flags=aflags & ops.ATTN_Q_PRESCALED)
            o.copy_(o32)
        else:
            ops.attention(qkv[:, :c], qkv[:, c:2 * c], qkv[:, 2 * c:], gidx, gidx, widx, patch_start, att.num_heads,
                          max_len, att.scale, o, work=64.0 * att.num_heads * sum_l2, flags=aflags)
        hid = w[pre + ".fc1.w"].shape[0]
        if xs is not None:
            st.xc = self._buf(n, c, self.T)
            ops.attn_tail_rr2(o, w[pre + ".tail_img"], w[pre + ".proj.b"], w[pre + ".norm2.g"], w[pre + ".norm2.b"],
                              w[pre + ".fc1.b"], w[pre + ".fc2.b"], xs, st.x, st.xc, ws=self.scratch(4 * n * c * 4 + 256))
            return
        if ops.attn_tail_fused_ok(o, hid):
            st.xc = self._buf(n, c, self.T)
            if (pre + ".tail_img") in w:
                ops.attn_tail_rr(o, w[pre + ".tail_img"], w[pre + ".proj.b"], w[pre + ".norm2.g"], w[pre + ".norm2.b"],
                                 w[pre + ".fc1.b"], w[pre + ".fc2.b"], st.x, st.xc)
            else:
                ops.attn_tail_fused(o, w[pre + ".proj.w"], w[pre + ".proj.b"], w[pre + ".norm2.g"], w[pre + ".norm2.b"],
                                    w[pre + ".fc1.w"], w[pre + ".fc1.b"], w[pre + ".fc2.w"], w[pre + ".fc2.b"], st.x, st.xc)
            return
        if c <= self.FUSE_LN_MAX_C:
            h2 = self._buf(n, c, self.T)
            ops.gemm(o, w[pre + ".proj.w"], st.x, bias=w[pre + ".proj.b"], res=st.x,
                     ln_post=(w[pre + ".norm2.g"], w[pre + ".norm2.b"]), ln_out=h2)
        else:
            h2 = None
            ops.gemm(o, w[pre + ".proj.w"], st.x, bias=w[pre + ".proj.b"], res=st.x)
        self._mlp(st, pre + ".norm2", pre + ".fc", h2)

    def run_embedding(self, plan, feat, perm, pre, curves):
        w, lv = self.w, plan.levels[0]
        cout = w[pre + ".w"].shape[0]
        a = ops.gather_pad_cast(feat, perm, w[pre + ".cpad"], self.T)
        x = self._buf(lv.n, cout, torch.float32)
        xc = x if self.T == torch.float32 else self._buf(lv.n, cout, self.T)
        if (pre + ".wimg") in w and lv.parent is not None and lv.n < (1 << 24):
            par, (cluster, seg) = lv.parent
            ops.stem5(a, w[pre + ".wimg"], w[pre + ".bn.scale"], w[pre + ".bn.shift"], lv.grid, cluster, par.nbr(3, True),
                      lv.child_info(), lv.depth, x, None if xc is x else xc)
        else:
            ops.gemm(a, w[pre + ".w"], x, scale=w[pre + ".bn.scale"], shift=w[pre + ".bn.shift"], act=ops.ACT_GELU,
                     nbr=lv.nbr(5, True), nbr_kmajor=True, kvol=125, out2=None if xc is x else xc)
        self._sat_note(xc)
        return State(lv, x, xc, curves)

    def run_pooling(self, plan, st, pre, cum_to, perm):
        w = self.w
        fine, coarse = st.level, plan.levels[cum_to]
        _, seg = plan.link(fine.cum, cum_to)
        cout = w[pre + ".proj.w"].shape[0]
        x = self._buf(coarse.n, cout, torch.float32)
        xc = x if self.T == torch.float32 else self._buf(coarse.n, cout, self.T)
        if (pre + ".proj.wimg") in w and st.xc.stride(0) == st.xc.shape[1] and fine.n <= 5 * coarse.n:
            ops.pool_fused(st.xc, w[pre + ".proj.wimg"], w[pre + ".proj.b"], seg, coarse.n, w[pre + ".bn.scale"],
                           w[pre + ".bn.shift"], ops.ACT_GELU, x, xc)
        else:
            y = self._buf(fine.n, cout, self.T)
            ops.gemm(st.xc, w[pre + ".proj.w"], y, bias=w[pre + ".proj.b"])
            ops.segment_max(y, seg, coarse.n, w[pre + ".bn.scale"], w[pre + ".bn.shift"], ops.ACT_GELU, x,
                            None if xc is x else xc)
        self._sat_note(xc)
        curves = st.curves if perm is None else [st.curves[int(j)] for j in perm]
        out = State(coarse, x, xc, curves)
        out.parent = st
        return out

    def run_unpooling(self, plan, st, pre, mod):
        w = self.w
        parent = st.parent
        fine, coarse = parent.level, st.level
        cluster, _ = plan.link(fine.cum, coarse.cum)
        cout = w[pre + ".proj.w"].shape[0]
        f = (2 ** -0.5 if mod.skip_connection_scale else 1.0)
        if mod.skip_connection_scale_i is not None:
            f *= 0.8 ** (int(mod.skip_connection_scale_i) - 1)
        x = self._buf(fine.n, cout, torch.float32)
        xc = self._buf(fine.n, cout, self.T)
        if mod.skip_connection_mode == "add":
            assert f == 1.0, "rejected by SerializedUnpooling.__init__"
            child = self._buf(coarse.n, cout, torch.float32)
            ops.gemm(st.xc, w[pre + ".proj.w"], child, bias=w[pre + ".proj.b"], scale=w[pre + ".proj_bn.scale"],
                     shift=w[pre + ".proj_bn.shift"], act=ops.ACT_GELU)
            ops.gemm(parent.xc, w[pre + ".skip.w"], x, bias=w[pre + ".skip.b"], scale=w[pre + ".skip_bn.scale"],
                     shift=w[pre + ".skip_bn.shift"], act=ops.ACT_GELU, add_src=child, add_idx=cluster, out2=xc,
                     out2_pre_add=True)
        else:
            child = self._buf(coarse.n, cout, self.T)
            ops.gemm(st.xc, w[pre + ".proj.w"], child, bias=w[pre + ".proj.b"], scale=w[pre + ".proj_bn.scale"],
                     shift=w[pre + ".proj_bn.shift"], act=ops.ACT_GELU)
            z = self._buf(coarse.n, cout, torch.float32)
            ops.gemm(child, w[pre + ".cat_b.w"], z)
            ops.gemm(parent.xc, w[pre + ".skip.w"], xc, bias=w[pre + ".skip.b"], scale=w[pre + ".skip_bn.scale"],
                     shift=w[pre + ".skip_bn.shift"], act=ops.ACT_GELU)
            ops.gemm(xc, w[pre + ".cat_a.w"], x, bias=w[pre + ".cat.b"], add_src=z, add_idx=cluster)
        self._sat_note(xc)
        out = State(fine, x, xc, parent.curves)
        out.parent = parent.parent
        return out

    def run_cross_block(self, nst, cst):
        w = self.w
        cb = self.model.backbone._tm_dec0.cross_block2
        att = cb.attn
        lv, clv = nst.level, cst.level
        if clv is not lv and list(clv.offs_host) != list(lv.offs_host):
            raise CdsegError("cross attention needs the same number of c- and n-branch bottleneck points per batch "
                             "element (ref: ptv3.py:1009 reuses the q padding for kv)")
        n, cq = nst.x.shape
        self._cpe(nst, "x.q_cpe", nst.xc)
        self._cpe(cst, "x.kv_cpe", cst.xc)
        hq = self._buf(n, cq, self.T)
        ops.layernorm(nst.x, w["x.q_norm1.g"], w["x.q_norm1.b"], hq)
        hkv = self._buf(n, cst.x.shape[1], self.T)
        ops.layernorm(cst.x, w["x.kv_norm1.g"], w["x.kv_norm1.b"], hkv)
        cst.xc = hkv
        if self.T == torch.float32:
            cst.x = hkv
        q = self._buf(n, cq, self.T)
        ops.gemm(hq, w["x.q.w"], q, bias=w["x.q.b"])
        kv = self._buf(n, 2 * cq, self.T)
        ops.gemm(hkv, w["x.kv.w"], kv, bias=w["x.kv.b"])
        K = att.q_patch_size
        q_gidx, widx = lv.slots(nst.curves[att.order_index], K, att.enable_flash)
        kv_gidx, _ = clv.slots(cst.curves[att.order_index], K, att.enable_flash)
        _, _, _, _, patch_start, max_len, sum_l2 = lv.pad(K, att.enable_flash)
        self._add_work(64.0 * att.num_heads * sum_l2, 4.0 * n * cq * q.element_size())
        o = self._buf(n, cq, self.T)
        ops.attention(q, kv[:, :cq], kv[:, cq:], q_gidx, kv_gidx, widx, patch_start, att.num_heads, max_len, att.scale, o,
                      work=64.0 * att.num_heads * sum_l2, flags=ops.ATTN_Q_PRESCALED if self.q_prescaled else 0)
        if "x.tail_img" in w and n >= ops.DEEP512_MIN_ROWS:
            nst.xc = self._buf(n, cq, self.T)
            ops.attn_tail_rr(o, w["x.tail_img"], w["x.proj.b"], w["x.q_norm2.g"], w["x.q_norm2.b"], w["x.fc1.b"], w["x.fc2.b"],
                             nst.x, nst.xc)
            return
        if "x.tail_img" in w and hasattr(ops, "attn_tail_rr2"):
            x_new = self._buf(n, cq, torch.float32)
            nst.xc = self._buf(n, cq, self.T)
            ops.attn_tail_rr2(o, w["x.tail_img"], w["x.proj.b"], w["x.q_norm2.g"], w["x.q_norm2.b"], w["x.fc1.b"], w["x.fc2.b"],
                              nst.x, x_new, nst.xc, ws=self.scratch(4 * n * cq * 4 + 256))
            nst.x = x_new
            return
        if cb.tm_feat == 1.0:
            ops.gemm(o, w["x.proj.w"], nst.x, bias=w["x.proj.b"], res=nst.x)
        else:
            ops.gemm(o, w["x.proj.w"], nst.x, bias=w["x.proj.b"], scale=w["x.feat_scale"], shift=w["x.feat_zero"],
                     res=nst.x)
        self._mlp(nst, "x.q_norm2", "x.fc")

    def forward_work(self, plan):
        bb, w = self.model.backbone, self.w
        cache = {}

        def occ(lv, k):
            if (lv.cum, k) not in cache:
                cache[(lv.cum, k)] = float((lv.nbr(k, True) >= 0).sum().item())
            return cache[(lv.cum, k)]

        out = dict(conv=0.0, linear=0.0, attention=0.0, stem=0.0, pool_unpool=0.0, head=0.0)
        deep = [0.0]

        def block(mod, pre, lv):
            c, hid = mod.channels, w[pre + ".fc1.w"].shape[0]
            out["conv"] += 2.0 * occ(lv, 3) * c * c
            if c > 64 or self.T == torch.float32:
                deep[0] += 2.0 * occ(lv, 3) * c * c
            out["linear"] += 2.0 * lv.n * (5.0 * c * c + 2.0 * c * hid)
            out["attention"] += 64.0 * mod.attn.num_heads * lv.pad(mod.attn.patch_size, mod.attn.enable_flash)[6]

        def stages(branch, cum, n_stages):
            for s in range(n_stages):
                lv = plan.levels[cum[s]]
                enc = getattr(getattr(bb, f"_{branch}_enc"), f"enc{s}")
                if s > 0:
                    pw = w[f"{branch}_enc{s}.down.proj.w"]
                    out["pool_unpool"] += 2.0 * plan.levels[cum[s - 1]].n * pw.shape[0] * pw.shape[1]
                for name, mod in enc._modules.items():
                    if name.startswith("block"):
                        block(mod, f"{branch}_enc{s}.{name}", lv)

        lv0 = plan.levels[0]
        stem_in = w["n_emb.w"].shape[1] // 125
        out["stem"] += 2.0 * occ(lv0, 5) * min(stem_in, bb._n_embedding.stem.conv.in_channels) * w["n_emb.w"].shape[0]
        stages("n", plan.n_cum, bb.n_num_stages)
        if bb.condition:
            out["stem"] += 2.0 * occ(lv0, 5) * bb._c_embedding.stem.conv.in_channels * w["c_emb.w"].shape[0]
            stages("c", plan.c_cum, bb.c_num_stages)
            cb = bb._tm_dec0.cross_block2
            lq, lc = plan.levels[plan.n_cum[-1]], plan.levels[plan.c_cum[-1]]
            cq, ck = cb.q_channels, cb.kv_channels
            out["conv"] += 2.0 * occ(lq, 3) * cq * cq + 2.0 * occ(lc, 3) * ck * ck
            deep[0] += 2.0 * occ(lq, 3) * cq * cq + 2.0 * occ(lc, 3) * ck * ck
            out["linear"] += 2.0 * lq.n * (cq * cq * 3 + 2.0 * cq * w["x.fc1.w"].shape[0]) + 2.0 * lc.n * (ck * ck + ck * 2 * cq)
            out["attention"] += 64.0 * cb.attn.num_heads * lq.pad(cb.attn.q_patch_size, cb.attn.enable_flash)[6]
        for s in reversed(range(bb.n_num_stages - 1)):
            lf, lc = plan.levels[plan.n_cum[s]], plan.levels[plan.n_cum[s + 1]]
            pre = f"n_dec{s}.up"
            out["pool_unpool"] += 2.0 * lc.n * w[pre + ".proj.w"].numel() + 2.0 * lf.n * w[pre + ".skip.w"].numel()
            if (pre + ".cat_a.w") in w:
                out["pool_unpool"] += 2.0 * lc.n * w[pre + ".cat_b.w"].numel() + 2.0 * lf.n * w[pre + ".cat_a.w"].numel()
            dec = getattr(bb._n_dec, f"dec{s}")
            for name, mod in dec._modules.items():
                if name.startswith("block"):
                    block(mod, f"n_dec{s}.{name}", lf)
        if "n_head.w" in w:
            out["head"] += 2.0 * lv0.n * w["n_head.w"].numel()
        out["total"] = sum(out.values())
        out["conv_deep"] = deep[0]
        return out

    def draw(self, n, feat_shape, c_ch, noise_level, n_perms, always_noise=False):
        m = self.model
        d = {}
        if noise_level is not None:
            on_cpu_gen = m.noise_source == "torch_cpu" and getattr(m, "feat_noise_source", "torch_cpu") == "torch_cpu"
            d["feat_noise"] = torch.randn(feat_shape) if on_cpu_gen else None
        if m.condition and (always_noise or (m.dm and m.dm_input == "xt")):
            d["noise"] = (torch.normal(0, 1, size=(n, c_ch), dtype=torch.float32)
                          if m.noise_source == "torch_cpu" else None)
        if m.backbone.shuffle_orders:
            no = len(m.backbone.order)
            d["perms"] = [torch.randperm(no).tolist() for _ in range(n_perms)]
        return d

    def predraw(self, input_dict, noise_level=None):
        m, bb = self.model, self.model.backbone
        feat = input_dict["feat"]
        per_call = (2 + len(bb.c_stride) + len(bb.n_stride)) if bb.condition else (1 + len(bb.n_stride))
        d = self.draw(feat.shape[0], tuple(feat.shape), m.c_in_channels, noise_level, per_call)
        d["rng_base"] = self.reserve_rng()
        return d

    def _add_work(self, flops, nbytes=0.0):
        with self._work_lock:
            self.attn_work += flops
            self.attn_bytes += nbytes

    RNG_RESERVE = 8

    def reserve_rng(self, k=None):
        if self.model.noise_source == "device":
            return int(torch.randint(0, 2 ** 62, (1,), dtype=torch.int64).item())
        seed = torch.initial_seed()
        if seed != self._rng_seed:
            self._rng_seed, self.rng_offset = seed, 0
        base = self.rng_offset
        self.rng_offset += self.RNG_RESERVE if k is None else int(k)
        return base

    def _device_randn(self, shape):
        seed = torch.initial_seed()
        out = ops.randn(shape, seed, self._tls.rng, self.device)
        self._tls.rng += 1
        return out

    def inference(self, input_dict, noise_level=None, draws=None):
        prev = ops.set_f32x3(self.x3) if hasattr(ops, "set_f32x3") else None
        try:
            with _lib.use(self.variant):
                return self._inference(input_dict, noise_level, draws)
        finally:
            if prev is not None:
                ops.set_f32x3(prev)
            if hasattr(ops, "unbind_stream"):
                ops.unbind_stream()

    def inference_ddim(self, input_dict, step=1, mode="avg", noise_level=None, draws=None):
        prev = ops.set_f32x3(self.x3) if hasattr(ops, "set_f32x3") else None
        try:
            with _lib.use(self.variant):
                return self._inference_ddim(input_dict, step, mode, noise_level, draws)
        finally:
            if prev is not None:
                ops.set_f32x3(prev)
            if hasattr(ops, "unbind_stream"):
                ops.unbind_stream()

    def _setup(self, input_dict, noise_level, draws, n_backbone_calls, always_noise=False):
        m, bb = self.model, self.model.backbone
        feat = input_dict["feat"]
        dev = feat.device
        self.prepare(dev)
        if dev.type == "cuda" and hasattr(ops, "bind_stream"):
            ops.bind_stream()
        grid = input_dict["grid_coord"]
        offset = input_dict["offset"]
        n = feat.shape[0]
        offset_host = [int(v) for v in input_dict["offset_host"]] if "offset_host" in input_dict else None
        cond = bb.condition
        c_ch = m.c_in_channels
        per_call = (2 + len(bb.c_stride) + len(bb.n_stride)) if cond else (1 + len(bb.n_stride))
        box = {"draws": draws}

        def host_draws():
            if box["draws"] is None:
                box["draws"] = self.draw(n, tuple(feat.shape), c_ch, noise_level, per_call * n_backbone_calls, always_noise)
            d = box["draws"]
            self._tls.rng = (d["rng_base"] if "rng_base" in d
                             else self.reserve_rng(max(self.RNG_RESERVE, 2 + n_backbone_calls)))

        plan = self.build_plan(grid, offset.to(torch.int64), offset_host, n, while_device_works=host_draws, defer_pads=True)
        draws = box["draws"]
        feat = feat.float().contiguous()
        if noise_level is not None:
            fn = draws.get("feat_noise")
            fn = self._device_randn(tuple(feat.shape)) if fn is None else fn.to(dev, torch.float32)
            feat = ops.axpy(feat, fn.contiguous(), noise_level)
            input_dict["feat"] = feat
        perms = list(draws["perms"]) if bb.shuffle_orders else [None] * (per_call * n_backbone_calls)
        self.last_plan = plan
        return feat, draws, perms, plan, per_call

    def _t_bias(self, t):
        w = self.w
        if self.model.backbone.T_dim == -1 or "t.table" not in w:
            return {}
        ent = self._tb_cache.get(t)
        if ent is None:
            v = ops.gemv(w["t.fc1.w"], w["t.fc1.b"], w["t.table"][t + 1], ops.ACT_SWISH)
            v = ops.gemv(w["t.fc2.w"], w["t.fc2.b"], v, ops.ACT_SWISH)
            tall = ops.gemv(w["t.mlp.w"], w["t.mlp.b"], v, ops.ACT_NONE)
            if tall.is_cuda:
                torch.cuda.current_stream(tall.device).synchronize()
            ent = self._tb_cache[t] = {k: tall[a:b] for k, (a, b) in self.t_slices.items()}
        return ent

    def _sat_begin(self, dev):
        self._sat = None
        self.saturation_count, self.saturation_checked = None, 0
        if self.count_saturation and self.T == torch.float16:
            self._sat = torch.zeros(1, dtype=torch.int64, device=dev)

    def _sat_note(self, t):
        if self._sat is not None and t is not None and t.dtype == torch.float16:
            ops.count_saturated(t, self._sat)
            self.saturation_checked += t.numel()

    def _sat_end(self):
        if self._sat is not None:
            self.saturation_count = int(self._sat.item())
            self._sat = None

    def _inference(self, input_dict, noise_level=None, draws=None):
        m, bb = self.model, self.model.backbone
        feat, draws, perms, plan, _ = self._setup(input_dict, noise_level, draws, 1)
        n, dev = feat.shape[0], feat.device
        c_ch = m.c_in_channels
        c_feat = c_perm = None
        t = 0
        if bb.condition:
            if m.dm and m.dm_input == "xt":
                nz = draws.get("noise")
                if nz is None:
                    c_feat, c_perm = self._device_randn((n, c_ch)), None
                else:
                    c_feat, c_perm = nz.to(dev, torch.float32).contiguous(), plan.perm0
                t = m.T - 1
            else:
                c_feat = feat if c_ch == feat.shape[1] else input_dict["coord"].float().contiguous()
                c_perm = plan.perm0
        self._sat_begin(dev)
        logits, _ = self.backbone(plan, feat, c_feat, c_perm, t, perms, want_c=False)
        self._sat_end()
        return logits

    def _inference_ddim(self, input_dict, step, mode, noise_level, draws):
        m, bb = self.model, self.model.backbone
        if not bb.condition:
            return self._inference(input_dict, noise_level, draws)
        if m.dm_target != "noise":
            raise NotImplementedError("dm_target other than 'noise'")
        schedule = np.linspace(-1, m.T - 1, num=step + 1, dtype=int)[::-1]
        feat, draws, perms, plan, per_call = self._setup(input_dict, noise_level, draws, len(schedule), always_noise=True)
        n, dev = feat.shape[0], feat.device
        nz = draws.get("noise")
        c_xt = self._device_randn((n, m.c_in_channels)) if nz is None else \
            ops.gather_rows(nz.to(dev, torch.float32).contiguous(), plan.perm0)
        ab = m.Alpha_bar
        n_pred = None
        for k, t in enumerate(schedule):
            t = int(t)
            logits, eps = self.backbone(plan, feat, c_xt, None, t, perms[per_call * k:per_call * (k + 1)], want_c=True)
            s_ab, s_1ab = float(torch.sqrt(ab[t])), float(torch.sqrt(1 - ab[t]))
            if t == 0:
                c_xt = ops.ddim_update(c_xt, eps, 0.0, s_1ab, s_ab, 0.0, final=True)
            else:
                c_xt = ops.ddim_update(c_xt, eps, float(torch.sqrt(ab[t - 1])), s_1ab, s_ab,
                                       float(torch.sqrt(1 - ab[t - 1])), final=False)
            if mode == "avg":
                n_pred = logits if n_pred is None else ops.axpy(n_pred, logits, 1.0)
            else:
                n_pred = logits
            if t <= 0:
                break
        if mode == "avg":
            n_pred = ops.axpy(torch.zeros_like(n_pred), n_pred, 1.0 / len(schedule))
        return n_pred

    def backbone(self, plan, feat, c_feat, c_perm, t, perms, want_c):
        bb = self.model.backbone
        w = self.w
        cond = bb.condition
        n = feat.shape[0]
        dev = feat.device
        pi = iter(perms)
        base_curves = [CURVES.index(o) for o in bb.order]

        def shuffled(perm):
            return list(base_curves) if perm is None else [base_curves[int(j)] for j in perm]

        n_cum, c_cum = plan.n_cum, plan.c_cum
        if cond:
            c_curves = shuffled(next(pi))
        n_curves = shuffled(next(pi))
        tb = self._t_bias(t) if cond else {}

        def enc_stage(st, branch, s, cum, perm):
            enc = getattr(getattr(bb, f"_{branch}_enc"), f"enc{s}")
            e = self._eng(f"{branch}_enc{s}")
            e._fit(st)
            if s > 0:
                st = e.run_pooling(plan, st, f"{branch}_enc{s}.down", cum[s], perm)
            for name, mod in enc._modules.items():
                if name.startswith("block"):
                    key = f"{branch}_enc{s}.{name}"
                    e.run_block(st, mod, key, tb.get(key))
            return st

        def dec_stage(st, branch, s):
            dec = getattr(getattr(bb, f"_{branch}_dec"), f"dec{s}")
            e = self._eng(f"{branch}_dec{s}")
            e._fit(st)
            e._fit(st.parent)
            st = e.run_unpooling(plan, st, f"{branch}_dec{s}.up", dec.up)
            for name, mod in dec._modules.items():
                if name.startswith("block"):
                    key = f"{branch}_dec{s}.{name}"
                    e.run_block(st, mod, key, tb.get(key))
            return st

        if cond:
            p_c1, p_n1, p_n2, p_c2, p_n3, p_n4 = (next(pi) for _ in range(6))
            n_perms = [None, p_n1, p_n2, p_n3, p_n4]

            def c_branch():
                st = self._eng("c_emb").run_embedding(plan, c_feat, c_perm, "c_emb", c_curves)
                st = enc_stage(st, "c", 0, c_cum, None)
                st = enc_stage(st, "c", 1, c_cum, p_c1)
                return enc_stage(st, "c", 2, c_cum, p_c2)

            fork = self.fork_stage if (dev.type == "cuda" and self.fork_stage is not None) else None
            SHARE_EVENTS.on = fork is not None
            if fork is None:
                plan.finish_pads()
            cst = c_branch() if fork is None else None
            nst = self._eng("n_emb").run_embedding(plan, feat, plan.perm0, "n_emb", n_curves)
            plan.finish_pads()
            join = None
            for s in range(bb.n_num_stages):
                if fork is not None and s == fork:
                    cst, join = self._on_side_stream(c_branch)
                nst = enc_stage(nst, "n", s, n_cum, n_perms[s])
            if join is not None:
                ops.wait_event(join)
            e = self._eng("x")
            e._fit(nst)
            e._fit(cst)
            e.run_cross_block(nst, cst)
        else:
            nst = self._eng("n_emb").run_embedding(plan, feat, plan.perm0, "n_emb", n_curves)
            plan.finish_pads()
            for s in range(bb.n_num_stages):
                nst = enc_stage(nst, "n", s, n_cum, next(pi) if s > 0 else None)
        self.trace = {"n_bottleneck": nst.x}
        c_out = None
        if cond and want_c:
            for s in reversed(range(bb.c_num_stages - 1)):
                cst = dec_stage(cst, "c", s)
            e = self._eng("c_head")
            e._fit(cst, exact=True)
            c_out = torch.empty((n, w["c_head.w"].shape[0]), dtype=torch.float32, device=dev)
            ops.gemm(cst.xc, e.w["c_head.w"], c_out, bias=e.w["c_head.b"])
        for s in reversed(range(bb.n_num_stages - 1)):
            nst = dec_stage(nst, "n", s)
        if "n_head.w" in w:
            e = self._eng("n_head")
            e._fit(nst, exact=True)
            logits = torch.empty((n, w["n_head.w"].shape[0]), dtype=torch.float32, device=dev)
            ops.gemm(nst.xc, e.w["n_head.w"], logits, bias=e.w["n_head.b"], out_idx=plan.perm0)
        else:
            logits = torch.empty((n, nst.x.shape[1]), dtype=torch.float32, device=dev)
            ops.scatter_rows(nst.x, plan.perm0, logits)
        return logits, c_out
```

### cdsegnet_amd/ops.py

```python
import ctypes
import os
import threading

import torch

from . import _lib
from ._lib import ACT_GELU, ACT_NONE, ACT_SWISH, BF16, F32, GemmArgs, check

__all__ = ["ACT_NONE", "ACT_GELU", "ACT_SWISH", "F32", "BF16"]

LP_DTYPES = {"bf16": torch.bfloat16, "f16": torch.float16}


class _Dtypes:

    def __getitem__(self, dtype):
        if dtype == torch.float32:
            return F32
        if dtype == LP_DTYPES[_lib.active()]:
            return BF16
        raise _lib.CdsegError(f"{dtype} tensors do not belong to the active build of the library ({_lib.active()})")


_DT = _Dtypes()
# ... 273 lines not shown
    return cluster, seg_start, count


def pool_levels(zcode_sorted, shifts, last_idx):
    lib = _lib.load()
    n, L, nb = zcode_sorted.numel(), len(shifts), last_idx.numel()
    dev = zcode_sorted.device
    cluster = torch.empty((L, n), dtype=torch.int32, device=dev)
    seg = torch.empty((L, n + 1), dtype=torch.int32, device=dev)
    meta = torch.empty(L * (1 + nb) + 1, dtype=torch.int32, device=dev)
    ws = workspace(lib.cdseg_pool_levels_ws_bytes(n, L), dev)
    sh = (ctypes.c_int * L)(*[int(v) for v in shifts])
    check(lib.cdseg_pool_levels(_ptr(zcode_sorted), n, sh, L, _ptr(last_idx), nb, _ptr(cluster), _ptr(seg), _ptr(meta),
                                _ptr(ws), ws.numel(), _stream()), "pool_levels")
    return cluster, seg, meta


def link_derive(cl0a, seg0a, ma, cl0b, seg0b, mb):
    dev = cl0a.device
    cluster = torch.empty(int(ma), dtype=torch.int32, device=dev)
    seg = torch.empty(int(mb) + 1, dtype=torch.int32, device=dev)
    check(_lib.load().cdseg_link_derive(_ptr(cl0a), _ptr(seg0a), int(ma), _ptr(cl0b), _ptr(seg0b), int(mb),
                                         _ptr(cluster), _ptr(seg), _stream()), "link_derive")
    return cluster, seg


def coarse_orders(clusters, orders, sizes):
    lib = _lib.load()
    n0 = clusters[0].numel()
    nl, nc = len(clusters), len(orders)
    dev = clusters[0].device
    out = torch.empty(nc * int(sum(sizes)), dtype=torch.int32, device=dev)
    ws = workspace(lib.cdseg_coarse_orders_ws_bytes(n0, nl, nc), dev)
    cp = (ctypes.c_void_p * nl)(*[t.data_ptr() for t in clusters])
    op = (ctypes.c_void_p * nc)(*[t.data_ptr() for t in orders])
    check(lib.cdseg_coarse_orders(cp, nl, op, nc, n0, _ptr(out), _ptr(ws), ws.numel(), _stream()), "coarse_orders")
    parts = out.split([int(m) for m in sizes for _ in range(nc)])
    return [list(parts[i * nc:(i + 1) * nc]) for i in range(nl)]


def pool_gather(seg_start, m, n_fine, pooling_depth, grid_f, batch_f, code4_f):
    dev = grid_f.device
    grid_c = torch.empty((m, 3), dtype=torch.int32, device=dev)
    batch_c = torch.empty(m, dtype=torch.int32, device=dev)
    code_c = torch.empty((4, m), dtype=torch.int64, device=dev)
    check(_lib.load().cdseg_pool_gather(_ptr(seg_start), m, n_fine, int(pooling_depth), _ptr(grid_f), _ptr(batch_f),
                                        _ptr(code4_f), _ptr(grid_c), _ptr(batch_c), _ptr(code_c), _stream()),
          "pool_gather")
    return grid_c, batch_c, code_c


def nbr_table(zcode_sorted, grid_i32, batch_i32, depth, ksize, kmajor=False):
    n = grid_i32.shape[0]
    kv = ksize ** 3
    shape = (kv, n) if kmajor else (n, kv)
    nbr = torch.empty(shape, dtype=torch.int32, device=grid_i32.device)
    check(_lib.load().cdseg_nbr_table(_ptr(zcode_sorted), _ptr(grid_i32), _ptr(batch_i32), n, int(depth), int(ksize),
                                      1 if kmajor else 0, _ptr(nbr), _stream()), "nbr_table")
    return nbr


def nbr_table_from_parent(zcode_sorted, grid_i32, cluster, parent_nbr3, seg_start, m, depth, ksize, kmajor=False):
    n = zcode_sorted.numel()
    kv = ksize ** 3
    nbr = torch.empty((kv, n) if kmajor else (n, kv), dtype=torch.int32, device=zcode_sorted.device)
    check(_lib.load().cdseg_nbr_table_from_parent(_ptr(zcode_sorted), _ptr(grid_i32), _ptr(cluster), _ptr(parent_nbr3),
                                                   _ptr(seg_start), n, int(m), int(depth), int(ksize),
                                                   1 if kmajor else 0, _ptr(nbr), _stream()), "nbr_table_from_parent")
    return nbr


def nbr_table_from_info(grid_i32, cluster, parent_nbr3, child_info_words, m, depth, ksize, kmajor=False):
    n = grid_i32.shape[0]
    kv = ksize ** 3
    nbr = torch.empty((kv, n) if kmajor else (n, kv), dtype=torch.int32, device=grid_i32.device)
    check(_lib.load().cdseg_nbr_table_from_info(_ptr(grid_i32), _ptr(cluster), _ptr(parent_nbr3), _ptr(child_info_words), n,
                                                 int(m), int(depth), int(ksize), 1 if kmajor else 0, _ptr(nbr), _stream()),
          "nbr_table_from_info")
    return nbr


def pad_plan(order, offs, offs_pad, patch, n_pad):
    dev = offs.device
    gidx = torch.empty(n_pad, dtype=torch.int32, device=dev)
    widx = torch.empty(n_pad, dtype=torch.int32, device=dev)
    check(_lib.load().cdseg_pad_plan(_ptr(order), _ptr(offs), _ptr(offs_pad), offs.numel() - 1, int(patch), n_pad,
                                     _ptr(gidx), _ptr(widx), _stream()), "pad_plan")
    return gidx, widx


class NativePlanCall:

    def __init__(self, spec, grid, offset_dev, n, nb, depth, end_bit, gmax_pin, meta_pin):
        lib = _lib.load()
        self.lib, self.spec, self.n, self.nb, self.depth = lib, spec, int(n), int(nb), int(depth)
        self.sp = ctypes.byref(spec)
        off = (ctypes.c_long * 13)()
        tot = (ctypes.c_long * 3)()
        check(lib.cdseg_plan_begin_layout(self.sp, self.n, self.nb, off, tot), "plan_begin_layout")
        dev = grid.device
        self.b32 = torch.empty(tot[0], dtype=torch.int32, device=dev)
        self.b64 = torch.empty(tot[1], dtype=torch.int64, device=dev)
        self.ws = workspace(tot[2], dev)
        self.boff = list(off)
        io = self.bio = _lib.PlanBeginIO()
        io.grid, io.grid_elem_bytes, io.offset = grid.data_ptr(), grid.element_size(), offset_dev.data_ptr()
        io.nb, io.n, io.depth, io.end_bit = self.nb, self.n, self.depth, int(end_bit)
        io.i32, io.i64, io.ws, io.ws_bytes = self.b32.data_ptr(), self.b64.data_ptr(), self.ws.data_ptr(), self.ws.numel()
        io.gmax_host = None if gmax_pin is None else gmax_pin.data_ptr()
        io.meta_host = meta_pin.data_ptr()
        self._keep = (grid, offset_dev)

    def begin(self, phase):
        check(self.lib.cdseg_plan_begin(self.sp, ctypes.byref(self.bio), int(phase), _stream()), "plan_begin")

    def begin_views(self):
        o, n, b32, b64, L, nc = self.boff, self.n, self.b32, self.b64, self.spec.nlev, self.spec.ncurve
        return (b32[o[1]:o[1] + n], b32[o[2]:o[2] + 3 * n].view(n, 3), b32[o[3]:o[3] + n],
                b64[o[12]:o[12] + 4 * n].view(4, n), b32[o[5]:o[5] + L * n].view(L, n),
                b32[o[6]:o[6] + L * (n + 1)].view(L, n + 1), b32[o[8]:o[8] + nc * n].view(nc, n) if nc else None)

    def finish(self, m, offs_rows, pads_pin):
        lib, spec, L, npad = self.lib, self.spec, self.spec.nlev, self.spec.npad
        mh = (ctypes.c_long * L)(*m)
        flat = [v for r in offs_rows for v in r]
        oh = (ctypes.c_int * len(flat))(*flat)
        n_off = 3 * L + 2 * spec.nlink + 2 * (L + 1) + 1 + 3 * (L + 1) * npad + 2
        n_info = 5 + 5 * (L + 1) * npad
        off = (ctypes.c_long * n_off)()
        info = (ctypes.c_long * n_info)()
        check(lib.cdseg_plan_finish_layout(self.sp, self.n, self.nb, mh, oh, off, info), "plan_finish_layout")
        dev = self.b32.device
        self.f32 = torch.empty(info[0], dtype=torch.int32, device=dev)
        self.f64 = torch.empty(max(1, info[1]), dtype=torch.int64, device=dev)
        if info[2] > self.ws.numel():
            self.ws = workspace(info[2], dev)
        pin = pads_pin(info[3])
        o, n, b32, b64 = self.boff, self.n, self.b32, self.b64
        io = _lib.PlanFinishIO()
        io.n, io.nb, io.depth, io.m_host, io.offs_host = self.n, self.nb, self.depth, mh, oh
        io.grid0 = b32.data_ptr() + 4 * o[2]
        io.bat0 = b32.data_ptr() + 4 * o[3]
        io.code0 = b64.data_ptr() + 8 * o[12]
        io.cluster = b32.data_ptr() + 4 * o[5]
        io.seg = b32.data_ptr() + 4 * o[6]
        io.orders0 = b32.data_ptr() + 4 * o[8]
        io.i32, io.i64, io.ws, io.ws_bytes = self.f32.data_ptr(), self.f64.data_ptr(), self.ws.data_ptr(), self.ws.numel()
        io.pads_host = pin.data_ptr()
        check(lib.cdseg_plan_finish(self.sp, ctypes.byref(io), _stream()), "plan_finish")
        return list(off), list(info)


PAD_BATCH_MAX = 48


def pad_plan_batch(items, nb):
    lib = _lib.load()
    res = []
    for s0 in range(0, len(items), PAD_BATCH_MAX):
        chunk = items[s0:s0 + PAD_BATCH_MAX]
        k = len(chunk)
        total = sum(int(it[4]) for it in chunk)
        dev = chunk[0][1].device
        gidx = torch.empty(total, dtype=torch.int32, device=dev)
        widx = torch.empty(total, dtype=torch.int32, device=dev)
        orders = (ctypes.c_void_p * k)(*[None if it[0] is None else it[0].data_ptr() for it in chunk])
        offs = (ctypes.c_void_p * k)(*[it[1].data_ptr() for it in chunk])
        offs_pad = (ctypes.c_void_p * k)(*[it[2].data_ptr() for it in chunk])
        patch = (ctypes.c_int * k)(*[int(it[3]) for it in chunk])
        npad = (ctypes.c_long * k)(*[int(it[4]) for it in chunk])
        check(lib.cdseg_pad_plan_batch(k, orders, offs, offs_pad, patch, npad, int(nb), _ptr(gidx), _ptr(widx), _stream()),
              "pad_plan_batch")
        sizes = [int(it[4]) for it in chunk]
        res.extend(zip(gidx.split(sizes), widx.split(sizes)))
    return res


F32X3 = 2


def set_f32x3(on):
    prev, _TLS.f32x3 = _TLS.f32x3, bool(on)
    return prev


def gemm(A, W, out, *, bias=None, scale=None, shift=None, act=ACT_NONE, res=None, add_src=None, add_idx=None,
         nbr=None, out_idx=None, out2=None, out2_pre_add=False, M=None, kvol=1, colbias=None, ln_pre=None,
         nbr_kmajor=False,
         ln_post=None, ln_out=None, ln_eps=1e-5, cache=True):
    if not A.is_cuda:
        _need_gpu(A, W, out)
    x3 = _TLS.f32x3 and W.dtype == torch.float32
    key = (W.data_ptr(), _dp(bias), _dp(scale), _dp(shift), int(kvol), int(act), x3)
    cache_d = _TLS.gemm_cache
    ent = cache_d.get(key) if cache else None
    if ent is None:
        for t in (bias, scale, shift):
            if t is not None and t.dtype != torch.float32:
                raise _lib.CdsegError("gemm epilogue vectors are float32")
        a = GemmArgs()
        a.W, a.bias, a.scale, a.shift = key[0], key[1], key[2], key[3]
        a.N = W.shape[0]
        a.kvol = int(kvol)
        a.K = W.shape[1] // a.kvol
        a.compute_dtype = F32X3 if x3 else dt(W)
        a.act = int(act)
        ent = (a, ctypes.byref(a), W)
        if cache:
            if len(cache_d) > 4096:
                cache_d.clear()
            cache_d[key] = ent
    a = ent[0]
    if (res is not None and res.dtype != torch.float32) or (add_src is not None and add_src.dtype != torch.float32):
        raise _lib.CdsegError("gemm residuals are float32")
    a.A = A.data_ptr()
    a.res, a.add_src, a.add_idx, a.nbr, a.out_idx = _dp(res), _dp(add_src), _dp(add_idx), _dp(nbr), _dp(out_idx)
    a.out, a.out2 = out.data_ptr(), _dp(out2)
    m = int(M if M is not None else (nbr.shape[1 if nbr_kmajor else 0] if nbr is not None else A.shape[0]))
    a.nbr_kmajor = 1 if nbr_kmajor else 0
    a.M = m
    a.lda = A.stride(0)
    a.ldo = out.stride(0)
    a.ldo2 = out2.stride(0) if out2 is not None else 0
    a.ldres = res.stride(0) if res is not None else 0
    a.ldadd = add_src.stride(0) if add_src is not None else 0
    a.a_dtype = _DT[A.dtype]
    a.out_dtype = _DT[out.dtype]
    a.out2_dtype = _DT[out2.dtype] if out2 is not None else 0
    a.out2_pre_add = 1 if out2_pre_add else 0
    a.colbias = _dp(colbias)
    if ln_pre is not None:
        a.ln_pre_g, a.ln_pre_b = ln_pre[0].data_ptr(), ln_pre[1].data_ptr()
    else:
        a.ln_pre_g = a.ln_pre_b = None
    if ln_post is not None:
        a.ln_post_g, a.ln_post_b = ln_post[0].data_ptr(), ln_post[1].data_ptr()
        a.ln_out, a.ldln, a.ln_out_dtype = ln_out.data_ptr(), ln_out.stride(0), _DT[ln_out.dtype]
    else:
        a.ln_post_g = a.ln_post_b = a.ln_out = None
    a.ln_eps = float(ln_eps)
    if ((m + 63) >> 6) * ((a.N + 127) >> 7) < 256:
        ws = workspace(min(32 * m * a.N * 4, 64 << 20), out.device)
        a.ws, a.ws_bytes = ws.data_ptr(), ws.numel()
    elif nbr is not None and a.N >= 256 and ((m + 127) >> 7) * ((a.N + 255) >> 8) < 256:
        ws = workspace(min(8 * m * a.N * 4, 64 << 20), out.device)
        a.ws, a.ws_bytes = ws.data_ptr(), ws.numel()
    elif a.N > 128 and (ln_pre is not None or ln_post is not None):
        ws = workspace(m * a.N * 4, out.device)
        a.ws, a.ws_bytes = ws.data_ptr(), ws.numel()
    else:
        a.ws, a.ws_bytes = None, 0
    tok = TIMER.begin("conv" if nbr is not None else "gemm") if TIMER is not None else None
    check(_lib.load().cdseg_gemm(ent[1], _stream()), "gemm")
    if tok is not None:
        TIMER.end(tok, 2.0 * a.M * a.N * a.K * a.kvol)
    return out


FUSED_MLP_CHANNELS = (32, 64, 128)


def mlp_fused_ok(h, hidden):
    c = h.shape[1]
    return (is_lp(h.dtype) and c in FUSED_MLP_CHANNELS and hidden == 4 * c and
            c <= 128)


def mlp_fused(h, w1, b1, w2, b2, x, xc=None):
    _need_gpu(h, x)
    check(_lib.load().cdseg_mlp_fused(_ptr(h), h.stride(0), _ptr(w1), _ptr(b1), _ptr(w2), _ptr(b2), _ptr(x), x.stride(0),
                                       _ptr(xc), xc.stride(0) if xc is not None else 0, h.shape[0], h.shape[1], _DT[h.dtype],
                                       _stream()), "mlp_fused")
    return x


def cpe_head_fused_ok(y):
    return is_lp(y.dtype) and y.shape[1] in (32, 64)


def cpe_head_fused(y, wl, bl, lnp, x, colbias, ln1, wqkv, bqkv, qkv, eps=1e-5, qkv_flags=0):
    _need_gpu(y, x)
    check(_lib.load().cdseg_cpe_head_fused(_ptr(y), y.stride(0), _ptr(wl), _ptr(bl), _ptr(lnp[0]), _ptr(lnp[1]), _ptr(x),
                                            x.stride(0), _ptr(colbias), _ptr(ln1[0]), _ptr(ln1[1]), float(eps), _ptr(wqkv),
                                            _ptr(bqkv), _ptr(qkv), qkv.stride(0), y.shape[0], y.shape[1], _DT[y.dtype],
                                            int(qkv_flags), _stream()), "cpe_head_fused")
    return qkv


def attn_tail_fused_ok(o, hidden):
    c = o.shape[1]
    return is_lp(o.dtype) and c in (32, 64) and hidden == 4 * c


def attn_tail_fused(o, wp, bp, ln_g, ln_b, w1, b1, w2, b2, x, xc=None, eps=1e-5):
    _need_gpu(o, x)
    check(_lib.load().cdseg_attn_tail_fused(_ptr(o), o.stride(0), _ptr(wp), _ptr(bp), _ptr(ln_g), _ptr(ln_b), float(eps),
                                             _ptr(w1), _ptr(b1), _ptr(w2), _ptr(b2), _ptr(x), x.stride(0), _ptr(xc),
                                             xc.stride(0) if xc is not None else 0, o.shape[0], o.shape[1], _DT[o.dtype],
                                             _stream()), "attn_tail_fused")
    return x


DEEP512_MIN_ROWS = int(os.environ.get("CDSEG_DEEP512_MIN_ROWS", 2560))
DEEP_CHANNELS = (128, 256, 512)


def block_rr_ok(channels, dtype):
    return is_lp(dtype) and (channels in (32, 64) or channels in DEEP_CHANNELS)


def block_rr_head_on(channels=32):
    return channels in DEEP_CHANNELS


def block_rr_pack(channels, wl, wqkv, wp, w1, w2):
    _need_gpu(wl, wqkv, wp, w1, w2)
    lib = _lib.load()
    dev = wp.device
    head = torch.empty(lib.cdseg_block_rr_img_bytes(channels, 0), dtype=torch.uint8, device=dev) if wl is not None else None
    tail = torch.empty(lib.cdseg_block_rr_img_bytes(channels, 1), dtype=torch.uint8, device=dev)
    check(lib.cdseg_block_rr_pack(int(channels), _ptr(wl), _ptr(wqkv), _ptr(head), _ptr(wp), _ptr(w1), _ptr(w2), _ptr(tail),
                                  _stream()), "block_rr_pack")
    return head, tail


def cpe_head_rr(y, head_img, bl, lnp, x, colbias, ln1, bqkv, qkv, eps=1e-5, qkv_flags=0):
    check(_lib.load().cdseg_cpe_head_rr(_ptr(y), y.stride(0), _ptr(head_img), _ptr(bl), _ptr(lnp[0]), _ptr(lnp[1]), _ptr(x),
                                        x.stride(0), _ptr(colbias), _ptr(ln1[0]), _ptr(ln1[1]), float(eps), _ptr(bqkv),
                                        _ptr(qkv), qkv.stride(0), y.shape[0], y.shape[1], int(qkv_flags), _stream()),
          "cpe_head_rr")
    return qkv


def cpe_head_rr2(y, head_img, bl, lnp, x, x_out, colbias, ln1, bqkv, qkv, eps=1e-5, qkv_flags=0):
    check(_lib.load().cdseg_cpe_head_rr2(_ptr(y), y.stride(0), _ptr(head_img), _ptr(bl), _ptr(lnp[0]), _ptr(lnp[1]), _ptr(x),
                                         x.stride(0), _ptr(x_out), x_out.stride(0), _ptr(colbias), _ptr(ln1[0]), _ptr(ln1[1]),
                                         float(eps), _ptr(bqkv), _ptr(qkv), qkv.stride(0), y.shape[0], y.shape[1],
                                         int(qkv_flags), _stream()), "cpe_head_rr2")
    return qkv


def attn_tail_rr2(o, tail_img, bp, ln_g, ln_b, b1, b2, x_in, x, xc=None, ws=None, eps=1e-5):
    check(_lib.load().cdseg_attn_tail_rr2(_ptr(o), o.stride(0), _ptr(tail_img), _ptr(bp), _ptr(ln_g), _ptr(ln_b), float(eps),
                                          _ptr(b1), _ptr(b2), _ptr(x_in), x_in.stride(0), _ptr(x), x.stride(0), _ptr(xc),
                                          xc.stride(0) if xc is not None else 0, o.shape[0], o.shape[1], _ptr(ws),
                                          0 if ws is None else ws.numel() * ws.element_size(), _stream()), "attn_tail_rr2")
    return x


def attn_tail_rr(o, tail_img, bp, ln_g, ln_b, b1, b2, x, xc=None, eps=1e-5):
    check(_lib.load().cdseg_attn_tail_rr(_ptr(o), o.stride(0), _ptr(tail_img), _ptr(bp), _ptr(ln_g), _ptr(ln_b), float(eps),
                                         _ptr(b1), _ptr(b2), _ptr(x), x.stride(0), _ptr(xc),
                                         xc.stride(0) if xc is not None else 0, o.shape[0], o.shape[1], _stream()),
          "attn_tail_rr")
    return x


def _dp(t):
    return None if t is None else t.data_ptr()


def make_block_desc(dtype, channels, heads, hidden, attn_scale, ln_eps, tensors, attn_flags=0, x3=False):
    d = _lib.BlockDesc()
    d.dtype, d.channels, d.heads, d.hidden = (F32X3 if (x3 and dtype == torch.float32) else _DT[dtype]), int(channels), int(heads), int(hidden)
    d.attn_scale, d.ln_eps = float(attn_scale), float(ln_eps)
    d.attn_flags = int(attn_flags)
    for k, t in tensors.items():
        setattr(d, k, t.data_ptr())
    return (d, ctypes.byref(d), dict(tensors))


def block_scratch_bytes(desc, n):
    return _lib.load().cdseg_block_scratch_bytes(desc[1], int(n))


def count_saturated(x, counter):
    _need_gpu(x, counter)
    check(_lib.load().cdseg_count_saturated(_ptr(x), x.shape[0], x.shape[1], x.stride(0), _ptr(counter), _stream()),
          "count_saturated")


def split16(x, lo_scale=2048.0):
    _need_gpu(x)
    T = LP_DTYPES[_lib.active()]
    hi = torch.empty(x.shape, dtype=T, device=x.device)
    lo = torch.empty(x.shape, dtype=T, device=x.device)
    check(_lib.load().cdseg_split16(_ptr(x), x.stride(0), x.shape[0], x.shape[1], _ptr(hi), _ptr(lo), hi.stride(0),
                                    float(lo_scale), _stream()), "split16")
    return hi, lo


def block_forward(desc, n, x, xc_in, xc_out, tbias, nbr, gidx, widx, patch_start, num_patches, max_len, scratch,
                  sat_counter=None):
    if _TLS.block_io is None:
        io = _lib.BlockIO()
        _TLS.block_io = (io, ctypes.byref(io))
    io, ref = _TLS.block_io
    io.n = int(n)
    io.x, io.xc_in, io.xc_out, io.tbias = x.data_ptr(), xc_in.data_ptr(), xc_out.data_ptr(), _dp(tbias)
    io.nbr, io.gidx, io.widx, io.patch_start = nbr.data_ptr(), gidx.data_ptr(), widx.data_ptr(), patch_start.data_ptr()
    io.num_patches, io.max_len = int(num_patches), int(max_len)
    io.scratch, io.scratch_bytes = scratch.data_ptr(), scratch.numel()
    io.sat_counter = sat_counter.data_ptr() if sat_counter is not None else None
    check(_lib.load().cdseg_block_forward(desc[1], ref, _stream()), "block_forward")


def stem5_ok(cout, dtype):
    return cout == 32 and is_lp(dtype)


def child_info(zcode_sorted, seg_start, m):
    _need_gpu(zcode_sorted, seg_start)
    info = torch.empty(int(m), dtype=torch.int64, device=zcode_sorted.device)
    check(_lib.load().cdseg_child_info(_ptr(zcode_sorted), _ptr(seg_start), int(m), _ptr(info), _stream()), "child_info")
    return info


def stem5_pack(w):
    _need_gpu(w)
    assert is_lp(w.dtype) and tuple(w.shape) == (32, 1000)
    img = torch.empty(_lib.load().cdseg_stem5_wimg_bytes(), dtype=torch.uint8, device=w.device)
    check(_lib.load().cdseg_stem5_pack(_ptr(w), _ptr(img), _stream()), "stem5_pack")
    return img


def stem5(x8, wimg, scale, shift, grid, cluster, parent_nbr3, cinfo, depth, out, out2=None):
    _need_gpu(x8, wimg, grid, cluster, parent_nbr3, cinfo, out)
    n, m = x8.shape[0], cinfo.numel()
    check(_lib.load().cdseg_stem5(_ptr(x8), _ptr(wimg), _ptr(scale), _ptr(shift), _ptr(grid), _ptr(cluster),
                                  _ptr(parent_nbr3), _ptr(cinfo), n, m, int(depth), _ptr(out), _ptr(out2), _stream()), "stem5")
    return out


def subm_conv3_ok(x):
    n = x.shape[0]
    return (is_lp(x.dtype) and x.dim() == 2 and x.shape[1] in (32, 64) and x.stride(0) == x.shape[1] and
            n * 27 * 4 < 2 ** 31 and n * x.shape[1] * 2 < 2 ** 31 - 65536)


def subm_conv3_pack(w):
    _need_gpu(w)
    c = w.shape[0]
    img = torch.empty(_lib.load().cdseg_subm_conv3_wimg_bytes(c), dtype=torch.uint8, device=w.device)
    check(_lib.load().cdseg_subm_conv3_pack(_ptr(w), c, _ptr(img), _stream()), "subm_conv3_pack")
    return img


def subm_conv3(x, wimg, bias, nbr_kmajor, out):
    _need_gpu(x, wimg, nbr_kmajor, out)
    n, c = x.shape
    check(_lib.load().cdseg_subm_conv3(_ptr(x), x.stride(0), _ptr(wimg), _ptr(bias), _ptr(nbr_kmajor), n, c, _ptr(out),
                                       out.stride(0), _stream()), "subm_conv3")
    return out


def subm_conv3_f32(x, wimg, bias, nbr_kmajor, out, out_scale=1.0, accumulate=False):
    _need_gpu(x, wimg, nbr_kmajor, out)
    n, c = x.shape
    check(_lib.load().cdseg_subm_conv3_f32(_ptr(x), x.stride(0), _ptr(wimg), _ptr(bias), _ptr(nbr_kmajor), n, c, _ptr(out),
                                           out.stride(0), float(out_scale), 1 if accumulate else 0, _stream()),
          "subm_conv3_f32")
    return out


def layernorm(x, gamma, beta, out, *, eps=1e-5, res=None, colbias=None, out2=None):
    m, c = x.shape
    check(_lib.load().cdseg_layernorm(_ptr(x), dt(x), x.stride(0), _ptr(gamma), _ptr(beta), float(eps), _ptr(res),
                                      res.stride(0) if res is not None else 0, _ptr(colbias), _ptr(out), dt(out),
                                      out.stride(0), _ptr(out2), dt(out2) if out2 is not None else 0,
                                      out2.stride(0) if out2 is not None else 0, m, c, _stream()), "layernorm")
    return out


ATTN_Q_PRESCALED, ATTN_V_BF16 = 1, 2


def attention(q, k, v, q_gidx, kv_gidx, widx, patch_start, num_heads, max_len, scale, out, work=0.0, flags=0):
    num_patches = patch_start.numel() - 1
    if not (q.dtype == k.dtype == out.dtype) or (v.dtype != q.dtype and not (flags & ATTN_V_BF16)):
        raise _lib.CdsegError("attention: q, k, v, out must share a dtype")
    tok = TIMER.begin("attention") if TIMER is not None else None
    check(_lib.load().cdseg_attention_ex(_ptr(q), _ptr(k), _ptr(v), q.stride(0), k.stride(0), v.stride(0), _ptr(q_gidx),
                                         _ptr(kv_gidx), _ptr(widx), _ptr(patch_start), num_patches, int(num_heads),
                                         int(max_len), float(scale), _ptr(out), out.stride(0),
                                         F32X3 if (_TLS.f32x3 and q.dtype == torch.float32) else dt(q), int(flags), _stream()),
          "attention")
    if tok is not None:
        TIMER.end(tok, work)
    return out


def segment_max(y, seg_start, m, scale, shift, act, out, out2=None):
    c = y.shape[1]
    check(_lib.load().cdseg_segment_max(_ptr(y), dt(y), y.stride(0), _ptr(seg_start), m, c, _ptr(scale), _ptr(shift),
                                        int(act), _ptr(out), out.stride(0), _ptr(out2),
                                        dt(out2) if out2 is not None else 0, out2.stride(0) if out2 is not None else 0,
                                        _stream()), "segment_max")
    return out


def pool_fused_ok(cin, cout, dtype):
    return is_lp(dtype) and (int(cin), int(cout)) in ((32, 64), (64, 128))


def pool_fused_pack(w):
    _need_gpu(w)
    cout, cin = w.shape
    lib = _lib.load()
    img = torch.empty(lib.cdseg_pool_fused_img_bytes(cin, cout), dtype=torch.uint8, device=w.device)
    check(lib.cdseg_pool_fused_pack(_ptr(w), cin, cout, _ptr(img), _stream()), "pool_fused_pack")
    return img


def pool_fused(x, wimg, bias, seg_start, m, scale, shift, act, out, out2=None):
    _need_gpu(x, out)
    cin, cout = x.shape[1], out.shape[1]
    check(_lib.load().cdseg_pool_fused(_ptr(x), x.stride(0), _ptr(wimg), _ptr(bias), _ptr(seg_start), int(m), _ptr(scale),
                                       _ptr(shift), int(act), _ptr(out), out.stride(0), _ptr(out2),
                                       out2.stride(0) if out2 is not None else 0, cin, cout, _stream()), "pool_fused")
    return out


def segment_mean(x, seg_start, m):
    out = torch.empty((m, x.shape[1]), dtype=torch.float32, device=x.device)
    check(_lib.load().cdseg_segment_mean(_ptr(x), x.stride(0), _ptr(seg_start), m, x.shape[1], _ptr(out),
                                         out.stride(0), _stream()), "segment_mean")
    return out


def gemv(w, b, x, act=ACT_NONE):
    n, k = w.shape
    y = torch.empty(n, dtype=torch.float32, device=w.device)
    check(_lib.load().cdseg_gemv(_ptr(w), _ptr(b), _ptr(x), n, k, int(act), _ptr(y), _stream()), "gemv")
    return y


def randn(shape, seed, offset, device):
    out = torch.empty(shape, dtype=torch.float32, device=device)
    check(_lib.load().cdseg_randn(_ptr(out), out.numel(), int(seed) & (2 ** 64 - 1), int(offset), _stream()), "randn")
    return out


def cast(src, dtype):
    src = src.contiguous()
    out = torch.empty(src.shape, dtype=dtype, device=src.device)
    check(_lib.load().cdseg_cast(_ptr(src), dt(src), _ptr(out), _DT[dtype], src.numel(), _stream()), "cast")
    return out


def gather_pad_cast(src, idx, cpad, dtype):
    src = src.contiguous()
    n = idx.numel() if idx is not None else src.shape[0]
    out = torch.empty((n, cpad), dtype=dtype, device=src.device)
    check(_lib.load().cdseg_gather_pad_cast(_ptr(src), src.stride(0), _ptr(idx), n, src.shape[1], int(cpad), _ptr(out),
                                            _DT[dtype], _stream()), "gather_pad_cast")
    return out


def ddim_update(xt, eps, sqrt_ab_prev, sqrt_1m_ab, sqrt_ab, sqrt_1m_ab_prev, final=False):
    out = torch.empty_like(xt)
    check(_lib.load().cdseg_ddim_update(_ptr(xt), _ptr(eps), float(sqrt_ab_prev), float(sqrt_1m_ab), float(sqrt_ab),
                                 float(sqrt_1m_ab_prev), 1 if final else 0, _ptr(out), xt.numel(), _stream()),
          "ddim_update")
    return out


def axpy(a, b, alpha):
    out = torch.empty_like(a)
    check(_lib.load().cdseg_axpy(_ptr(a), _ptr(b), float(alpha), _ptr(out), a.numel(), _stream()), "axpy")
    return out


def voxelize(coord, grid_size):
    _need_gpu(coord)
    coord = coord.float().contiguous()
    n = coord.shape[0]
    grid = torch.empty((n, 3), dtype=torch.int32, device=coord.device)
    key = torch.empty(n, dtype=torch.int64, device=coord.device)
    mn = torch.empty(3, dtype=torch.int32, device=coord.device)
    check(_lib.load().cdseg_voxelize(_ptr(coord), float(grid_size), n, _ptr(grid), _ptr(key), _ptr(mn), _stream()), "voxelize")
    return grid, key, mn


def voxelize_any(coord, grid_size):
    if coord.dtype != torch.float64:
        return voxelize(coord, grid_size)
    _need_gpu(coord)
    coord = coord.contiguous()
    n = coord.shape[0]
    grid = torch.empty((n, 3), dtype=torch.int32, device=coord.device)
    key = torch.empty(n, dtype=torch.int64, device=coord.device)
    mn = torch.empty(3, dtype=torch.int32, device=coord.device)
    check(_lib.load().cdseg_voxelize_f64(_ptr(coord), float(grid_size), n, _ptr(grid), _ptr(key), _ptr(mn), _stream()),
          "voxelize_f64")
    return grid, key, mn


def center_shift(coord, apply_z=True):
    _need_gpu(coord)
    assert coord.dtype in (torch.float32, torch.float64) and coord.dim() == 2 and coord.shape[1] == 3
    coord = coord.contiguous()
    out = torch.empty_like(coord)
    ws = torch.empty(12, dtype=torch.float64, device=coord.device)
    check(_lib.load().cdseg_center_shift(_ptr(coord), 1 if coord.dtype == torch.float64 else 0, coord.shape[0],
                                         1 if apply_z else 0, _ptr(out), _ptr(ws), _stream()), "center_shift")
    return out
# ... 187 lines not shown
```

Measured before the change: 79.59 million.

## Skip padded query tiles in attention and add dual-stream 512-channel deep kernels

Result: faster. 80.73 million (median of 6 runs) (+1.4%).

```diff
diff --git a/cdsegnet_amd/csrc/attention.hip b/cdsegnet_amd/csrc/attention.hip
--- a/cdsegnet_amd/csrc/attention.hip
+++ b/cdsegnet_amd/csrc/attention.hip
@@ -167,6 +167,7 @@
   constexpr int NPC = 32 / WAVES;
   extern __shared__ __attribute__((aligned(16))) char smem[];
   char* Ks = smem;
+  int* s_live = reinterpret_cast<int*>(smem + 2 * KV_STAGE + ONES_BYTES);
   unsigned* s_next = reinterpret_cast<unsigned*>(smem + 2 * KV_STAGE + ONES_BYTES + 48);
   int* s_qidx = reinterpret_cast<int*>(smem + 2 * KV_STAGE + ONES_BYTES + 64);
   const unsigned lds_base = (unsigned)(uintptr_t)(__attribute__((address_space(3))) char*)smem;
@@ -190,7 +191,7 @@
 
   const int ql = lane & 31;
   const int h = lane >> 5;
-  const int nqt = nkt;
+  int nqt = nkt;
   auto claim = [&]() {
     for (;;) {
       unsigned i = 0;
@@ -225,6 +226,16 @@
     if (wave < ATTN_RUN) {
 #pragma unroll
       for (int i = 0; i < 2; ++i) gq[i] = p.q_gidx[ps + min(wave * 128 + i * 64 + lane, L - 1)];
+    }
+    if (wave < ATTN_RUN) {
+      int live = 0;
+#pragma unroll
+      for (int i = 0; i < 2; ++i) {
+        const int s = wave * 128 + i * 64 + lane;
+        const unsigned long long m = __ballot(s < L && p.widx[ps + min(s, L - 1)] >= 0);
+        if (m) live = wave * 128 + i * 64 + 64 - __builtin_clzll(m);
+      }
+      if (lane == 0) s_live[wave] = live;
     }
     const int qt_slice0 = qslice * ATTN_RUN + wave;
     int gfirst = 0;
@@ -282,6 +293,12 @@
       }
     }
     __syncthreads();
+  }
+  {
+    const int4 a = *reinterpret_cast<const int4*>(s_live), b = *reinterpret_cast<const int4*>(s_live + 4);
+    const int live = __builtin_amdgcn_readfirstlane(max(max(max(a.x, a.y), max(a.z, a.w)), max(max(b.x, b.y), max(b.z, b.w))));
+    nqt = (live + 31) >> 5;
+    if (qt_first >= nqt) qt_first = -1;
   }
   if (!ATTN_PRIO_OUTSIDE) __builtin_amdgcn_s_setprio(0);
   ATTN_STAMP(t1);
diff --git a/cdsegnet_amd/csrc/deep.hip b/cdsegnet_amd/csrc/deep.hip
--- a/cdsegnet_amd/csrc/deep.hip
+++ b/cdsegnet_amd/csrc/deep.hip
@@ -23,6 +23,12 @@
   __builtin_amdgcn_s_barrier();
 }
 
+template <int NS>
+__device__ __forceinline__ int fresh(int p) {
+  if (NS > 1) asm volatile("" : "+v"(p));
+  return p;
+}
+
 __device__ __forceinline__ uint4 pack8(const f32x4_t& a, const f32x4_t& b) {
   uint4 r;
   r.x = pack_bf16x2(a[0], a[1]); r.y = pack_bf16x2(a[2], a[3]);
@@ -36,9 +42,9 @@
   return r;
 }
 
-template <int C, int BM>
+template <int C, int BM, int NT = 2 * C>
 __device__ __forceinline__ void load_tile(const bf16_t* src, int ld, long m0, long n, char* buf, int tid) {
-  constexpr int NCH = C / 8, NT = 2 * C, PT = BM * NCH / NT;
+  constexpr int NCH = C / 8, PT = BM * NCH / NT;
   uint4 r[PT];
 #pragma unroll
   for (int i = 0; i < PT; ++i) {
@@ -54,10 +60,10 @@
   }
 }
 
-template <int C, int BM>
+template <int C, int BM, int NT = 2 * C>
 __device__ __forceinline__ void load_tile_partials(const float* part, int splits, const float* bias, long m0, long n, char* buf,
                                                    int tid) {
-  constexpr int NCH = C / 8, NT = 2 * C, PT = BM * NCH / NT;
+  constexpr int NCH = C / 8, PT = BM * NCH / NT;
   const long plane = n * (long)C;
 #pragma unroll
   for (int i = 0; i < PT; ++i) {
@@ -76,48 +82,87 @@
   }
 }
 
-template <int C, int BM>
-__device__ __forceinline__ void product(f32x4_t (&acc)[BM / 16][2], const char* bufX, uint4 (&ring)[DEEP_D][2],
-                                        const uint4* wp, int step0, int last_step, int p, int g) {
+template <int NS>
+struct WStream {
+  const uint4* wp;
+  __device__ __forceinline__ WStream(const uint4* wimg, int wave, int lane, int S) : wp(wimg + (size_t)wave * S * 128 + lane) {}
+  __device__ __forceinline__ uint4 at(int, int step, int f) const { return wp[(step * 2 + f) * 64]; }
+};
+template <>
+struct WStream<2> {
+  __amdgpu_buffer_rsrc_t rsrc;
+  int voff, stream_bytes;
+  __device__ __forceinline__ WStream(const uint4* wimg, int wave , int lane, int S)
+      : rsrc(__builtin_amdgcn_make_buffer_rsrc((void*)(wimg + (size_t)(2 * wave) * S * 128), 0, 2 * S * 2048, 0x00020000)),
+        voff(lane * 16), stream_bytes(S * 2048) {}
+  __device__ __forceinline__ uint4 at(int j, int step, int f) const {
+    return __builtin_bit_cast(uint4, __builtin_amdgcn_raw_buffer_load_b128(rsrc, voff, j * stream_bytes + (step * 2 + f) * 1024, 0));
+  }
+};
+
+template <int C, int BM, int NS>
+__device__ __forceinline__ void product(f32x4_t (&acc)[NS][BM / 16][2], const char* bufX, uint4 (&ring)[NS][DEEP_D][2],
+                                        const WStream<NS>& w, int step0, int last_step, int p, int g) {
   constexpr int KS = C / 32, NCH = C / 8, PTS = BM / 16;
+  if (NS > 1) asm volatile("" : "+v"(p));
   const char* xrow = bufX + p * (NCH * 16);
-  bf16x8_t b[2][PTS];
-  auto fetch = [&](int s, bf16x8_t (&dst)[PTS]) {
+  bf16x8_t b[NS > 1 ? 1 : 2][PTS];
+  auto fetch = [&](int s, bf16x8_t (&dst)[PTS], int pt0, int pt1) {
     const char* xs = xrow + (((4 * s + g) ^ p) << 4);
 #pragma unroll
-    for (int pt = 0; pt < PTS; ++pt) dst[pt] = *reinterpret_cast<const bf16x8_t*>(xs + pt * 16 * (NCH * 16));
+    for (int pt = pt0; pt < pt1; ++pt) dst[pt] = *reinterpret_cast<const bf16x8_t*>(xs + pt * 16 * (NCH * 16));
   };
-  fetch(0, b[0]);
+  auto mfmas = [&](int s, const bf16x8_t (&src)[PTS], int pt0, int pt1) {
+#pragma unroll
+    for (int j = 0; j < NS; ++j) {
+      const bf16x8_t a0 = __builtin_bit_cast(bf16x8_t, ring[j][s % DEEP_D][0]);
+      const bf16x8_t a1 = __builtin_bit_cast(bf16x8_t, ring[j][s % DEEP_D][1]);
+#pragma unroll
+      for (int pt = pt0; pt < pt1; ++pt) {
+        acc[j][pt][0] = mfma_16x16x32_bf16(a0, src[pt], acc[j][pt][0]);
+        acc[j][pt][1] = mfma_16x16x32_bf16(a1, src[pt], acc[j][pt][1]);
+      }
+    }
+  };
+  fetch(0, b[0], 0, NS > 1 ? PTS / 2 : PTS);
 #pragma unroll
   for (int s = 0; s < KS; ++s) {
-    const bf16x8_t a0 = __builtin_bit_cast(bf16x8_t, ring[s % DEEP_D][0]);
-    const bf16x8_t a1 = __builtin_bit_cast(bf16x8_t, ring[s % DEEP_D][1]);
-    if (s + 1 < KS) fetch(s + 1, b[(s + 1) & 1]);
-#pragma unroll
-    for (int pt = 0; pt < PTS; ++pt) {
-      acc[pt][0] = mfma_16x16x32_bf16(a0, b[s & 1][pt], acc[pt][0]);
-      acc[pt][1] = mfma_16x16x32_bf16(a1, b[s & 1][pt], acc[pt][1]);
+    if constexpr (NS > 1) {
+      fetch(s, b[0], PTS / 2, PTS);
+      mfmas(s, b[0], 0, PTS / 2);
+      __builtin_amdgcn_sched_barrier(0);
+      if (s + 1 < KS) fetch(s + 1, b[0], 0, PTS / 2);
+      mfmas(s, b[0], PTS / 2, PTS);
+    } else {
+      if (s + 1 < KS) fetch(s + 1, b[(s + 1) & 1], 0, PTS);
+      mfmas(s, b[s & 1], 0, PTS);
     }
     {
       int nx = step0 + s + DEEP_D;
       nx = nx < last_step ? nx : last_step;
-      ring[s % DEEP_D][0] = wp[(nx * 2 + 0) * 64];
-      ring[s % DEEP_D][1] = wp[(nx * 2 + 1) * 64];
+#pragma unroll
+      for (int j = 0; j < NS; ++j) {
+        ring[j][s % DEEP_D][0] = w.at(j, nx, 0);
+        ring[j][s % DEEP_D][1] = w.at(j, nx, 1);
+      }
     }
     __builtin_amdgcn_sched_barrier(0);
   }
 }
 
-__device__ __forceinline__ void prime(uint4 (&ring)[DEEP_D][2], const uint4* wp, int step0) {
-#pragma unroll
-  for (int d = 0; d < DEEP_D; ++d) {
-    ring[d][0] = wp[((step0 + d) * 2 + 0) * 64];
-    ring[d][1] = wp[((step0 + d) * 2 + 1) * 64];
-  }
-}
-
-template <int PTS, int NW>
-__device__ __forceinline__ void row_stats(const f32x4_t (&v)[PTS][2], float* st1, float* st2, int wave, int p, int g,
+template <int NS>
+__device__ __forceinline__ void prime(uint4 (&ring)[NS][DEEP_D][2], const WStream<NS>& w, int step0) {
+#pragma unroll
+  for (int d = 0; d < DEEP_D; ++d)
+#pragma unroll
+    for (int j = 0; j < NS; ++j) {
+      ring[j][d][0] = w.at(j, step0 + d, 0);
+      ring[j][d][1] = w.at(j, step0 + d, 1);
+    }
+}
+
+template <int PTS, int NW, int NS, bool SQ_UNFUSED = false>
+__device__ __forceinline__ void row_stats(const f32x4_t (&v)[NS][PTS][2], float* st1, float* st2, int wave, int p, int g,
                                           float inv_c, float eps, float (&mean)[PTS], float (&rstd)[PTS]) {
   auto across = [&](float* st, int pt) {
     float t = 0.f;
@@ -138,38 +183,48 @@
     return t;
   };
 #pragma unroll
-  for (int pt = 0; pt < PTS; ++pt) {
-    float s = ((v[pt][0][0] + v[pt][0][1]) + (v[pt][0][2] + v[pt][0][3])) +
-              ((v[pt][1][0] + v[pt][1][1]) + (v[pt][1][2] + v[pt][1][3]));
-    s += __shfl_xor(s, 16, 64);
-    s += __shfl_xor(s, 32, 64);
-    if (g == 0) st1[(16 * pt + p) * NW + wave] = s;
-  }
+  for (int j = 0; j < NS; ++j)
+#pragma unroll
+    for (int pt = 0; pt < PTS; ++pt) {
+      float s = ((v[j][pt][0][0] + v[j][pt][0][1]) + (v[j][pt][0][2] + v[j][pt][0][3])) +
+                ((v[j][pt][1][0] + v[j][pt][1][1]) + (v[j][pt][1][2] + v[j][pt][1][3]));
+      s += __shfl_xor(s, 16, 64);
+      s += __shfl_xor(s, 32, 64);
+      if (g == 0) st1[(16 * pt + p) * NW + NS * wave + j] = s;
+    }
   lds_barrier();
 #pragma unroll
   for (int pt = 0; pt < PTS; ++pt) mean[pt] = across(st1, pt) * inv_c;
 #pragma unroll
-  for (int pt = 0; pt < PTS; ++pt) {
-    float q = 0.f;
-#pragma unroll
-    for (int f = 0; f < 2; ++f)
-#pragma unroll
-      for (int r = 0; r < 4; ++r) {
-        const float d = v[pt][f][r] - mean[pt];
-        q += d * d;
-      }
-    q += __shfl_xor(q, 16, 64);
-    q += __shfl_xor(q, 32, 64);
-    if (g == 0) st2[(16 * pt + p) * NW + wave] = q;
-  }
+  for (int j = 0; j < NS; ++j)
+#pragma unroll
+    for (int pt = 0; pt < PTS; ++pt) {
+      float q = 0.f;
+#pragma unroll
+      for (int f = 0; f < 2; ++f)
+#pragma unroll
+        for (int r = 0; r < 4; ++r) {
+          const float d = v[j][pt][f][r] - mean[pt];
+          if constexpr (SQ_UNFUSED) {
+#pragma clang fp contract(off)
+            const float sq = d * d;
+            q = q + sq;
+          } else {
+            q += d * d;
+          }
+        }
+      q += __shfl_xor(q, 16, 64);
+      q += __shfl_xor(q, 32, 64);
+      if (g == 0) st2[(16 * pt + p) * NW + NS * wave + j] = q;
+    }
   lds_barrier();
 #pragma unroll
   for (int pt = 0; pt < PTS; ++pt) rstd[pt] = 1.0f / sqrtf(across(st2, pt) * inv_c + eps);
 }
 
-template <int C, int BM>
+template <int C, int BM, int NS = 1>
 struct DeepCfg {
-  static constexpr int NW = C / 32, KS = C / 32, NT = 64 * NW;
+  static constexpr int NW = C / 32, KS = C / 32, NT = 64 * NW / NS;
   static constexpr int ACT = BM * C * 2;
   static constexpr int STAT = 2 * BM * NW * 4;
   static constexpr int HEAD_LDS = ACT + STAT + 9 * C * 4;
@@ -187,9 +242,9 @@
   const float* ypart; const float* ybias; int ysplits;
 };
 
-template <int C, int BM>
-__global__ __launch_bounds__(2 * C, 2) void deep_head_kernel(DeepHeadP P) {
-  using K = DeepCfg<C, BM>;
+template <int C, int BM, int NS = 1>
+__global__ __launch_bounds__(2 * C / NS, 2) void deep_head_kernel(DeepHeadP P) {
+  using K = DeepCfg<C, BM, NS>;
   constexpr int NW = K::NW, KS = K::KS, NCH = C / 8, NT = K::NT, PTS = BM / 16, S = K::HEAD_STEPS;
   extern __shared__ __attribute__((aligned(16))) char smem[];
   char* bufA = smem;
@@ -201,96 +256,107 @@
   const int p = lane & 15, g = lane >> 4;
   const int c_lo = P.nsplit == 3 ? (int)(blockIdx.x % 3u) : 0, c_hi = P.nsplit == 3 ? c_lo + 1 : 3;
   const long m0 = (long)(P.nsplit == 3 ? blockIdx.x / 3u : blockIdx.x) * BM;
-  const uint4* wp = P.wimg + (size_t)wave * S * 128 + lane;
+  const WStream<NS> wp(P.wimg, wave, lane, S);
   DT_STAMP(0);
-  uint4 ring[DEEP_D][2];
-  prime(ring, wp, 0);
+  uint4 ring[NS][DEEP_D][2];
+  prime<NS>(ring, wp, 0);
   for (int c = tid; c < C; c += NT) {
     pr[c] = P.bl[c]; pr[C + c] = P.lnp_g[c]; pr[2 * C + c] = P.lnp_b[c]; pr[3 * C + c] = P.colbias ? P.colbias[c] : 0.f;
     pr[4 * C + c] = P.ln1_g[c]; pr[5 * C + c] = P.ln1_b[c];
   }
   for (int c = tid; c < 3 * C; c += NT) pr[6 * C + c] = P.bqkv[c];
-  if (P.ysplits > 1) load_tile_partials<C, BM>(P.ypart, P.ysplits, P.ybias, m0, P.n, bufA, tid);
-  else load_tile<C, BM>(P.y, P.ldy, m0, P.n, bufA, tid);
-  const int ch0 = 32 * wave + 8 * g;
+  if (P.ysplits > 1) load_tile_partials<C, BM, NT>(P.ypart, P.ysplits, P.ybias, m0, P.n, bufA, tid);
+  else load_tile<C, BM, NT>(P.y, P.ldy, m0, P.n, bufA, tid);
+  const int ch0 = 32 * NS * wave + 8 * g;
   lds_barrier();
   DT_STAMP(1);
 
-  f32x4_t v[PTS][2];
-  {
-    const f32x4_t b0 = *reinterpret_cast<const f32x4_t*>(pr + ch0), b1 = *reinterpret_cast<const f32x4_t*>(pr + ch0 + 4);
-#pragma unroll
-    for (int pt = 0; pt < PTS; ++pt) { v[pt][0] = b0; v[pt][1] = b1; }
-  }
-  product<C, BM>(v, bufA, ring, wp, 0, KS - 1, p, g);
+  f32x4_t v[NS][PTS][2];
+#pragma unroll
+  for (int j = 0; j < NS; ++j) {
+    const f32x4_t b0 = *reinterpret_cast<const f32x4_t*>(pr + ch0 + 32 * j), b1 = *reinterpret_cast<const f32x4_t*>(pr + ch0 + 32 * j + 4);
+#pragma unroll
+    for (int pt = 0; pt < PTS; ++pt) { v[j][pt][0] = b0; v[j][pt][1] = b1; }
+  }
+  product<C, BM, NS>(v, bufA, ring, wp, 0, KS - 1, p, g);
   DT_STAMP(2);
   asm volatile("" ::: "memory");
   __builtin_amdgcn_sched_barrier(0);
-  f32x4_t xr[PTS][2];
-#pragma unroll
-  for (int pt = 0; pt < PTS; ++pt) {
-    long m = m0 + 16 * pt + p;
-    if (m >= P.n) m = P.n - 1;
-#pragma unroll
-    for (int f = 0; f < 2; ++f) xr[pt][f] = *reinterpret_cast<const f32x4_t*>(P.x + m * P.ldx + ch0 + 4 * f);
-  }
+  f32x4_t xr[NS][PTS][2];
+#pragma unroll
+  for (int j = 0; j < NS; ++j)
+#pragma unroll
+    for (int pt = 0; pt < PTS; ++pt) {
+      long m = m0 + 16 * pt + p;
+      if (m >= P.n) m = P.n - 1;
+#pragma unroll
+      for (int f = 0; f < 2; ++f) xr[j][pt][f] = *reinterpret_cast<const f32x4_t*>(P.x + m * P.ldx + ch0 + 32 * j + 4 * f);
+    }
   float mean[PTS], rstd[PTS];
   const float inv_c = 1.0f / C;
-  row_stats<PTS, NW>(v, st1, st2, wave, p, g, inv_c, P.eps, mean, rstd);
+  row_stats<PTS, NW, NS>(v, st1, st2, wave, p, g, inv_c, P.eps, mean, rstd);
   DT_STAMP(3);
 #pragma unroll
-  for (int f = 0; f < 2; ++f) {
-    const f32x4_t ga = *reinterpret_cast<const f32x4_t*>(pr + C + ch0 + 4 * f);
-    const f32x4_t be = *reinterpret_cast<const f32x4_t*>(pr + 2 * C + ch0 + 4 * f);
-    const f32x4_t tb = *reinterpret_cast<const f32x4_t*>(pr + 3 * C + ch0 + 4 * f);
-#pragma unroll
-    for (int pt = 0; pt < PTS; ++pt) {
-#pragma unroll
-      for (int r = 0; r < 4; ++r) v[pt][f][r] = ((v[pt][f][r] - mean[pt]) * rstd[pt] * ga[r] + be[r]) + xr[pt][f][r] + tb[r];
-      const long m = m0 + 16 * pt + p;
-      if (m < P.n && c_lo == 0) *reinterpret_cast<f32x4_t*>(P.x_out + m * P.ldxo + ch0 + 4 * f) = v[pt][f];
-    }
-  }
+  for (int j = 0; j < NS; ++j)
+#pragma unroll
+    for (int f = 0; f < 2; ++f) {
+      const f32x4_t ga = *reinterpret_cast<const f32x4_t*>(pr + C + ch0 + 32 * j + 4 * f);
+      const f32x4_t be = *reinterpret_cast<const f32x4_t*>(pr + 2 * C + ch0 + 32 * j + 4 * f);
+      const f32x4_t tb = *reinterpret_cast<const f32x4_t*>(pr + 3 * C + ch0 + 32 * j + 4 * f);
+#pragma unroll
+      for (int pt = 0; pt < PTS; ++pt) {
+#pragma unroll
+        for (int r = 0; r < 4; ++r)
+          v[j][pt][f][r] = ((v[j][pt][f][r] - mean[pt]) * rstd[pt] * ga[r] + be[r]) + xr[j][pt][f][r] + tb[r];
+        const long m = m0 + 16 * pt + p;
+        if (m < P.n && c_lo == 0) *reinterpret_cast<f32x4_t*>(P.x_out + m * P.ldxo + ch0 + 32 * j + 4 * f) = v[j][pt][f];
+      }
+    }
   DT_STAMP(4);
-  row_stats<PTS, NW>(v, st1, st2, wave, p, g, inv_c, P.eps, mean, rstd);
+  row_stats<PTS, NW, NS>(v, st1, st2, wave, p, g, inv_c, P.eps, mean, rstd);
   DT_STAMP(5);
-  prime(ring, wp, KS * (1 + c_lo));
-  {
-    const f32x4_t ga0 = *reinterpret_cast<const f32x4_t*>(pr + 4 * C + ch0), ga1 = *reinterpret_cast<const f32x4_t*>(pr + 4 * C + ch0 + 4);
-    const f32x4_t be0 = *reinterpret_cast<const f32x4_t*>(pr + 5 * C + ch0), be1 = *reinterpret_cast<const f32x4_t*>(pr + 5 * C + ch0 + 4);
+  prime<NS>(ring, wp, KS * (1 + c_lo));
+#pragma unroll
+  for (int j = 0; j < NS; ++j) {
+    const float* pj = pr + ch0 + 32 * j;
+    const f32x4_t ga0 = *reinterpret_cast<const f32x4_t*>(pj + 4 * C), ga1 = *reinterpret_cast<const f32x4_t*>(pj + 4 * C + 4);
+    const f32x4_t be0 = *reinterpret_cast<const f32x4_t*>(pj + 5 * C), be1 = *reinterpret_cast<const f32x4_t*>(pj + 5 * C + 4);
 #pragma unroll
     for (int pt = 0; pt < PTS; ++pt) {
       f32x4_t h0, h1;
 #pragma unroll
       for (int r = 0; r < 4; ++r) {
-        h0[r] = (v[pt][0][r] - mean[pt]) * rstd[pt] * ga0[r] + be0[r];
-        h1[r] = (v[pt][1][r] - mean[pt]) * rstd[pt] * ga1[r] + be1[r];
-      }
-      *reinterpret_cast<uint4*>(bufA + act_off<NCH>(16 * pt + p, 4 * wave + g)) = pack8(h0, h1);
+        h0[r] = (v[j][pt][0][r] - mean[pt]) * rstd[pt] * ga0[r] + be0[r];
+        h1[r] = (v[j][pt][1][r] - mean[pt]) * rstd[pt] * ga1[r] + be1[r];
+      }
+      *reinterpret_cast<uint4*>(bufA + act_off<NCH>(16 * pt + p, 4 * (NS * wave + j) + g)) = pack8(h0, h1);
     }
   }
   lds_barrier();
   DT_STAMP(6);
 #pragma unroll 1
   for (int c = c_lo; c < c_hi; ++c) {
-    f32x4_t a[PTS][2];
-    {
-      const f32x4_t b0 = *reinterpret_cast<const f32x4_t*>(pr + 6 * C + c * C + ch0);
-      const f32x4_t b1 = *reinterpret_cast<const f32x4_t*>(pr + 6 * C + c * C + ch0 + 4);
-#pragma unroll
-      for (int pt = 0; pt < PTS; ++pt) { a[pt][0] = b0; a[pt][1] = b1; }
+    f32x4_t a[NS][PTS][2];
+#pragma unroll
+    for (int j = 0; j < NS; ++j) {
+      const f32x4_t b0 = *reinterpret_cast<const f32x4_t*>(pr + 6 * C + c * C + ch0 + 32 * j);
+      const f32x4_t b1 = *reinterpret_cast<const f32x4_t*>(pr + 6 * C + c * C + ch0 + 32 * j + 4);
+#pragma unroll
+      for (int pt = 0; pt < PTS; ++pt) { a[j][pt][0] = b0; a[j][pt][1] = b1; }
     }
     int po = p;
     asm volatile("" : "+v"(po));
-    product<C, BM>(a, bufA, ring, wp, KS * (1 + c), S - 1, po, g);
+    product<C, BM, NS>(a, bufA, ring, wp, KS * (1 + c), S - 1, po, g);
     DT_STAMP(7 + 2 * c);
 #pragma unroll
-    for (int pt = 0; pt < PTS; ++pt) {
-      const long m = m0 + 16 * pt + p;
-      if (m < P.n)
-        *reinterpret_cast<uint4*>(P.qkv + m * P.ldqkv + c * C + ch0) =
-            (LP_IS_F16 && c == 2 && P.v_bf16) ? pack8_truebf16(a[pt][0], a[pt][1]) : pack8(a[pt][0], a[pt][1]);
-    }
+    for (int j = 0; j < NS; ++j)
+#pragma unroll
+      for (int pt = 0; pt < PTS; ++pt) {
+        const long m = m0 + 16 * pt + p;
+        if (m < P.n)
+          *reinterpret_cast<uint4*>(P.qkv + m * P.ldqkv + c * C + ch0 + 32 * j) =
+              (LP_IS_F16 && c == 2 && P.v_bf16) ? pack8_truebf16(a[j][pt][0], a[j][pt][1]) : pack8(a[j][pt][0], a[j][pt][1]);
+      }
     DT_STAMP(8 + 2 * c);
   }
 }
@@ -303,9 +369,9 @@
   float* part;
 };
 
-template <int C, int BM>
-__global__ __launch_bounds__(2 * C, 2) void deep_tail_kernel(DeepTailP P) {
-  using K = DeepCfg<C, BM>;
+template <int C, int BM, int NS = 1>
+__global__ __launch_bounds__(2 * C / NS, 2) void deep_tail_kernel(DeepTailP P) {
+  using K = DeepCfg<C, BM, NS>;
   constexpr int NW = K::NW, KS = K::KS, NCH = C / 8, NT = K::NT, PTS = BM / 16, S = K::TAIL_STEPS;
   extern __shared__ __attribute__((aligned(16))) char smem[];
   char* bufA = smem;
@@ -319,59 +385,82 @@
   const int nsp = P.nsplit, js = nsp > 1 ? (int)(blockIdx.x % (unsigned)nsp) : 0;
   const int j_lo = js * (4 / nsp), j_hi = j_lo + 4 / nsp;
   const long m0 = (long)(nsp > 1 ? blockIdx.x / (unsigned)nsp : blockIdx.x) * BM;
-  const uint4* wp = P.wimg + (size_t)wave * S * 128 + lane;
+  const WStream<NS> wp(P.wimg, wave, lane, S);
   DT_STAMP(0);
-  uint4 ring[DEEP_D][2];
-  prime(ring, wp, 0);
+  uint4 ring[NS][DEEP_D][2];
+  prime<NS>(ring, wp, 0);
   for (int c = tid; c < C; c += NT) {
     pr[c] = P.bp[c]; pr[C + c] = P.ln_g[c]; pr[2 * C + c] = P.ln_b[c]; pr[3 * C + c] = P.b2[c];
   }
   for (int c = tid; c < 4 * C; c += NT) pr[4 * C + c] = P.b1[c];
-  load_tile<C, BM>(P.o, P.ldo, m0, P.n, bufA, tid);
-  const int ch0 = 32 * wave + 8 * g;
-  f32x4_t acc2[PTS][2];
+  load_tile<C, BM, NT>(P.o, P.ldo, m0, P.n, bufA, tid);
+  const int ch0 = 32 * NS * wave + 8 * g;
+  f32x4_t acc2[NS][PTS][2];
   {
-    f32x4_t xr[PTS][2];
-#pragma unroll
-    for (int pt = 0; pt < PTS; ++pt) {
-      long m = m0 + 16 * pt + p;
-      if (m >= P.n) m = P.n - 1;
-#pragma unroll
-      for (int f = 0; f < 2; ++f) xr[pt][f] = *reinterpret_cast<const f32x4_t*>(P.x_in + m * P.ldxi + ch0 + 4 * f);
-    }
+    f32x4_t xr[NS][PTS][2];
+    auto load_xr = [&]() {
+      const int px = fresh<NS>(p);
+#pragma unroll
+      for (int i = 0; i < NS; ++i)
+#pragma unroll
+        for (int pt = 0; pt < PTS; ++pt) {
+          long m = m0 + 16 * pt + px;
+          if (m >= P.n) m = P.n - 1;
+#pragma unroll
+          for (int f = 0; f < 2; ++f) xr[i][pt][f] = *reinterpret_cast<const f32x4_t*>(P.x_in + m * P.ldxi + ch0 + 32 * i + 4 * f);
+        }
+    };
+    if (NS == 1) load_xr();
     lds_barrier();
     DT_STAMP(1);
-    const f32x4_t b0 = *reinterpret_cast<const f32x4_t*>(pr + ch0), b1 = *reinterpret_cast<const f32x4_t*>(pr + ch0 + 4);
-#pragma unroll
-    for (int pt = 0; pt < PTS; ++pt) { acc2[pt][0] = b0; acc2[pt][1] = b1; }
-    product<C, BM>(acc2, bufA, ring, wp, 0, S - 1, p, g);
+#pragma unroll
+    for (int i = 0; i < NS; ++i) {
+      const f32x4_t b0 = *reinterpret_cast<const f32x4_t*>(pr + ch0 + 32 * i), b1 = *reinterpret_cast<const f32x4_t*>(pr + ch0 + 32 * i + 4);
+#pragma unroll
+      for (int pt = 0; pt < PTS; ++pt) { acc2[i][pt][0] = b0; acc2[i][pt][1] = b1; }
+    }
+    product<C, BM, NS>(acc2, bufA, ring, wp, 0, S - 1, p, g);
     DT_STAMP(2);
-#pragma unroll
-    for (int pt = 0; pt < PTS; ++pt) { acc2[pt][0] += xr[pt][0]; acc2[pt][1] += xr[pt][1]; }
+    if (NS > 1) {
+      asm volatile("" ::: "memory");
+      __builtin_amdgcn_sched_barrier(0);
+      load_xr();
+    }
+#pragma unroll
+    for (int i = 0; i < NS; ++i)
+#pragma unroll
+      for (int pt = 0; pt < PTS; ++pt) { acc2[i][pt][0] += xr[i][pt][0]; acc2[i][pt][1] += xr[i][pt][1]; }
   }
   {
     float mean[PTS], rstd[PTS];
     DT_STAMP(3);
-    row_stats<PTS, NW>(acc2, st1, st2, wave, p, g, 1.0f / C, P.eps, mean, rstd);
+    row_stats<PTS, NW, NS, (NS > 1 && !LP_IS_F16)>(acc2, st1, st2, wave, p, g, 1.0f / C, P.eps, mean, rstd);
     DT_STAMP(4);
-    const f32x4_t ga0 = *reinterpret_cast<const f32x4_t*>(pr + C + ch0), ga1 = *reinterpret_cast<const f32x4_t*>(pr + C + ch0 + 4);
-    const f32x4_t be0 = *reinterpret_cast<const f32x4_t*>(pr + 2 * C + ch0), be1 = *reinterpret_cast<const f32x4_t*>(pr + 2 * C + ch0 + 4);
-#pragma unroll
-    for (int pt = 0; pt < PTS; ++pt) {
-      f32x4_t h0, h1;
-#pragma unroll
-      for (int r = 0; r < 4; ++r) {
-        h0[r] = (acc2[pt][0][r] - mean[pt]) * rstd[pt] * ga0[r] + be0[r];
-        h1[r] = (acc2[pt][1][r] - mean[pt]) * rstd[pt] * ga1[r] + be1[r];
-      }
-      *reinterpret_cast<uint4*>(bufA + act_off<NCH>(16 * pt + p, 4 * wave + g)) = pack8(h0, h1);
+    const int ph = fresh<NS>(p);
+#pragma unroll
+    for (int i = 0; i < NS; ++i) {
+      const float* pi = pr + ch0 + 32 * i;
+      const f32x4_t ga0 = *reinterpret_cast<const f32x4_t*>(pi + C), ga1 = *reinterpret_cast<const f32x4_t*>(pi + C + 4);
+      const f32x4_t be0 = *reinterpret_cast<const f32x4_t*>(pi + 2 * C), be1 = *reinterpret_cast<const f32x4_t*>(pi + 2 * C + 4);
+#pragma unroll
+      for (int pt = 0; pt < PTS; ++pt) {
+        f32x4_t h0, h1;
+#pragma unroll
+        for (int r = 0; r < 4; ++r) {
+          h0[r] = (acc2[i][pt][0][r] - mean[pt]) * rstd[pt] * ga0[r] + be0[r];
+          h1[r] = (acc2[i][pt][1][r] - mean[pt]) * rstd[pt] * ga1[r] + be1[r];
+        }
+        *reinterpret_cast<uint4*>(bufA + act_off<NCH>(16 * pt + ph, 4 * (NS * wave + i) + g)) = pack8(h0, h1);
+      }
     }
   }
   if (js) {
-    prime(ring, wp, KS * (1 + 2 * j_lo));
+    prime<NS>(ring, wp, KS * (1 + 2 * j_lo));
     const f32x4_t z = {0.f, 0.f, 0.f, 0.f};
 #pragma unroll
-    for (int pt = 0; pt < PTS; ++pt) { acc2[pt][0] = z; acc2[pt][1] = z; }
+    for (int i = 0; i < NS; ++i)
+#pragma unroll
+      for (int pt = 0; pt < PTS; ++pt) { acc2[i][pt][0] = z; acc2[i][pt][1] = z; }
   }
   lds_barrier();
   DT_STAMP(5);
@@ -383,31 +472,36 @@
 #ifdef CDSEG_DEEP_TIMING
     const unsigned long long q0 = __builtin_readcyclecounter();
 #endif
-    f32x4_t acc1[PTS][2];
-    {
-      const f32x4_t b0 = *reinterpret_cast<const f32x4_t*>(pr + 4 * C + j * C + ch0);
-      const f32x4_t b1 = *reinterpret_cast<const f32x4_t*>(pr + 4 * C + j * C + ch0 + 4);
-#pragma unroll
-      for (int pt = 0; pt < PTS; ++pt) { acc1[pt][0] = b0; acc1[pt][1] = b1; }
+    f32x4_t acc1[NS][PTS][2];
+#pragma unroll
+    for (int i = 0; i < NS; ++i) {
+      const f32x4_t b0 = *reinterpret_cast<const f32x4_t*>(pr + 4 * C + j * C + ch0 + 32 * i);
+      const f32x4_t b1 = *reinterpret_cast<const f32x4_t*>(pr + 4 * C + j * C + ch0 + 32 * i + 4);
+#pragma unroll
+      for (int pt = 0; pt < PTS; ++pt) { acc1[i][pt][0] = b0; acc1[i][pt][1] = b1; }
     }
     int po = p;
     asm volatile("" : "+v"(po));
-    product<C, BM>(acc1, bufA, ring, wp, KS * (1 + 2 * j), S - 1, po, g);
+    product<C, BM, NS>(acc1, bufA, ring, wp, KS * (1 + 2 * j), S - 1, po, g);
 #ifdef CDSEG_DEEP_TIMING
     const unsigned long long q1 = __builtin_readcyclecounter();
 #endif
     if (j > j_lo) lds_barrier();
-#pragma unroll
-    for (int pt = 0; pt < PTS; ++pt) {
-      gelu_lp4(acc1[pt][0]);
-      gelu_lp4(acc1[pt][1]);
-      *reinterpret_cast<uint4*>(bufU + act_off<NCH>(16 * pt + p, 4 * wave + g)) = pack8(acc1[pt][0], acc1[pt][1]);
-    }
+    const int pu = fresh<NS>(po), gu = fresh<NS>(g);
+#pragma unroll
+    for (int i = 0; i < NS; ++i)
+#pragma unroll
+      for (int pt = 0; pt < PTS; ++pt) {
+        gelu_lp4(acc1[i][pt][0]);
+        gelu_lp4(acc1[i][pt][1]);
+        *reinterpret_cast<uint4*>(bufU + act_off<NCH>(16 * pt + pu, 4 * (NS * wave + i) + gu)) = pack8(acc1[i][pt][0], acc1[i][pt][1]);
+        if (NS > 1) __builtin_amdgcn_sched_barrier(0);
+      }
     lds_barrier();
 #ifdef CDSEG_DEEP_TIMING
     const unsigned long long q2 = __builtin_readcyclecounter();
 #endif
-    product<C, BM>(acc2, bufU, ring, wp, KS * (2 + 2 * j), S - 1, p, g);
+    product<C, BM, NS>(acc2, bufU, ring, wp, KS * (2 + 2 * j), S - 1, p, g);
 #ifdef CDSEG_DEEP_TIMING
     dt_fc1 += q1 - q0; dt_gelu += q2 - q1; dt_fc2 += __builtin_readcyclecounter() - q2;
 #endif
@@ -418,26 +512,32 @@
     g_deep_t[blockIdx.x * 16 + 8] = dt_fc1; g_deep_t[blockIdx.x * 16 + 9] = dt_gelu; g_deep_t[blockIdx.x * 16 + 10] = dt_fc2;
   }
 #endif
+  const int pe = fresh<NS>(p), che = 32 * NS * wave + 8 * fresh<NS>(g);
   if (nsp > 1) {
 #pragma unroll
-    for (int pt = 0; pt < PTS; ++pt) {
-      const long m = m0 + 16 * pt + p;
-      if (m < P.n) {
-        float* dst = P.part + ((size_t)js * P.n + m) * C + ch0;
-        *reinterpret_cast<f32x4_t*>(dst) = acc2[pt][0];
-        *reinterpret_cast<f32x4_t*>(dst + 4) = acc2[pt][1];
-      }
-    }
+    for (int i = 0; i < NS; ++i)
+#pragma unroll
+      for (int pt = 0; pt < PTS; ++pt) {
+        const long m = m0 + 16 * pt + pe;
+        if (m < P.n) {
+          float* dst = P.part + ((size_t)js * P.n + m) * C + che + 32 * i;
+          *reinterpret_cast<f32x4_t*>(dst) = acc2[i][pt][0];
+          *reinterpret_cast<f32x4_t*>(dst + 4) = acc2[i][pt][1];
+        }
+      }
   } else {
-    const f32x4_t b0 = *reinterpret_cast<const f32x4_t*>(pr + 3 * C + ch0), b1 = *reinterpret_cast<const f32x4_t*>(pr + 3 * C + ch0 + 4);
-#pragma unroll
-    for (int pt = 0; pt < PTS; ++pt) {
-      const long m = m0 + 16 * pt + p;
-      if (m < P.n) {
-        const f32x4_t o0 = acc2[pt][0] + b0, o1 = acc2[pt][1] + b1;
-        *reinterpret_cast<f32x4_t*>(P.x + m * P.ldx + ch0) = o0;
-        *reinterpret_cast<f32x4_t*>(P.x + m * P.ldx + ch0 + 4) = o1;
-        if (P.xc) *reinterpret_cast<uint4*>(P.xc + m * P.ldxc + ch0) = pack8(o0, o1);
+#pragma unroll
+    for (int i = 0; i < NS; ++i) {
+      const f32x4_t b0 = *reinterpret_cast<const f32x4_t*>(pr + 3 * C + che + 32 * i), b1 = *reinterpret_cast<const f32x4_t*>(pr + 3 * C + che + 32 * i + 4);
+#pragma unroll
+      for (int pt = 0; pt < PTS; ++pt) {
+        const long m = m0 + 16 * pt + pe;
+        if (m < P.n) {
+          const f32x4_t o0 = acc2[i][pt][0] + b0, o1 = acc2[i][pt][1] + b1;
+          *reinterpret_cast<f32x4_t*>(P.x + m * P.ldx + che + 32 * i) = o0;
+          *reinterpret_cast<f32x4_t*>(P.x + m * P.ldx + che + 32 * i + 4) = o1;
+          if (P.xc) *reinterpret_cast<uint4*>(P.xc + m * P.ldxc + che + 32 * i) = pack8(o0, o1);
+        }
       }
     }
   }
@@ -492,6 +592,8 @@
 }
 
 inline int pick_bm(long n) { return (n + 127) / 128 >= 160 ? 128 : 32; }
+constexpr long DEEP512_ROWS64_MIN = 256 * 32 + 1;
+inline int pick_bm512(long n) { return n >= cdseg_knob("CDSEG_DEEP512_ROWS64_MIN", DEEP512_ROWS64_MIN) ? 64 : 32; }
 
 inline int pick_head_split(long n, int C, int bm) {
   const long tiles = (n + bm - 1) / bm;
@@ -506,30 +608,30 @@
   return 1;
 }
 
-template <int C, int BM>
+template <int C, int BM, int NS = 1>
 int launch_head(const DeepHeadP& p, hipStream_t s) {
-  constexpr int lds = DeepCfg<C, BM>::HEAD_LDS;
+  constexpr int lds = DeepCfg<C, BM, NS>::HEAD_LDS;
   static std::atomic<bool> attr_done{false};
   if (!attr_done) {
-    if (hipFuncSetAttribute((const void*)deep_head_kernel<C, BM>, hipFuncAttributeMaxDynamicSharedMemorySize, lds) != hipSuccess)
+    if (hipFuncSetAttribute((const void*)deep_head_kernel<C, BM, NS>, hipFuncAttributeMaxDynamicSharedMemorySize, lds) != hipSuccess)
       return CDSEG_ERR_LAUNCH;
     attr_done = true;
   }
-  hipLaunchKernelGGL((deep_head_kernel<C, BM>), dim3((unsigned)((p.n + BM - 1) / BM) * (unsigned)p.nsplit), dim3(2 * C), lds, s, p);
+  hipLaunchKernelGGL((deep_head_kernel<C, BM, NS>), dim3((unsigned)((p.n + BM - 1) / BM) * (unsigned)p.nsplit), dim3(2 * C / NS), lds, s, p);
   CDSEG_CHECK_LAUNCH();
   return CDSEG_OK;
 }
 
-template <int C, int BM>
+template <int C, int BM, int NS = 1>
 int launch_tail(const DeepTailP& p, hipStream_t s) {
-  constexpr int lds = DeepCfg<C, BM>::TAIL_LDS;
+  constexpr int lds = DeepCfg<C, BM, NS>::TAIL_LDS;
   static std::atomic<bool> attr_done{false};
   if (!attr_done) {
-    if (hipFuncSetAttribute((const void*)deep_tail_kernel<C, BM>, hipFuncAttributeMaxDynamicSharedMemorySize, lds) != hipSuccess)
+    if (hipFuncSetAttribute((const void*)deep_tail_kernel<C, BM, NS>, hipFuncAttributeMaxDynamicSharedMemorySize, lds) != hipSuccess)
       return CDSEG_ERR_LAUNCH;
     attr_done = true;
   }
-  hipLaunchKernelGGL((deep_tail_kernel<C, BM>), dim3((unsigned)((p.n + BM - 1) / BM) * (unsigned)p.nsplit), dim3(2 * C), lds, s, p);
+  hipLaunchKernelGGL((deep_tail_kernel<C, BM, NS>), dim3((unsigned)((p.n + BM - 1) / BM) * (unsigned)p.nsplit), dim3(2 * C / NS), lds, s, p);
   CDSEG_CHECK_LAUNCH();
   if (p.nsplit > 1) {
     const long units = p.n * (C / 8);
@@ -583,11 +685,11 @@
   p.x_out = x_out; p.ldxo = ldxo;
   p.colbias = colbias; p.ln1_g = ln1_g; p.ln1_b = ln1_b; p.bqkv = bqkv; p.qkv = (bf16_t*)qkv;
   p.n = n; p.ldy = ldy; p.ldx = ldx; p.ldqkv = ldqkv; p.eps = eps;
-  const int bm = channels == 512 ? 32 : cdseg_knob("CDSEG_DEEP_BM", pick_bm(n));
+  const int bm = channels == 512 ? pick_bm512(n) : cdseg_knob("CDSEG_DEEP_BM", pick_bm(n));
   p.nsplit = (cdseg_knob("CDSEG_DEEP_SPLIT", 1) && (const float*)x_out != x) ? pick_head_split(n, channels, bm) : 1;
   if (channels == 128) return bm == 128 ? launch_head<128, 128>(p, s) : launch_head<128, 32>(p, s);
   if (channels == 256) return bm == 128 ? launch_head<256, 128>(p, s) : launch_head<256, 32>(p, s);
-  if (channels == 512) return launch_head<512, 32>(p, s);
+  if (channels == 512) return bm == 64 ? launch_head<512, 64, 2>(p, s) : launch_head<512, 32>(p, s);
   return CDSEG_ERR_UNSUPPORTED;
 }
 
@@ -598,11 +700,11 @@
   p.o = (const bf16_t*)o; p.wimg = (const uint4*)tail_img; p.bp = bp; p.ln_g = ln_g; p.ln_b = ln_b; p.b1 = b1; p.b2 = b2;
   p.x_in = x_in; p.ldxi = ldxi;
   p.x = x; p.xc = (bf16_t*)xc; p.n = n; p.ldo = ldo; p.ldx = ldx; p.ldxc = ldxc; p.eps = eps;
-  const int bm = channels == 512 ? 32 : cdseg_knob("CDSEG_DEEP_BM", pick_bm(n));
+  const int bm = channels == 512 ? pick_bm512(n) : cdseg_knob("CDSEG_DEEP_BM", pick_bm(n));
   p.nsplit = (ws && cdseg_knob("CDSEG_DEEP_SPLIT", 1) && !(((uintptr_t)ws) & 15)) ? pick_tail_split(n, channels, bm, ws_bytes) : 1;
   p.part = (float*)ws;
   if (channels == 128) return bm == 128 ? launch_tail<128, 128>(p, s) : launch_tail<128, 32>(p, s);
   if (channels == 256) return bm == 128 ? launch_tail<256, 128>(p, s) : launch_tail<256, 32>(p, s);
-  if (channels == 512) return launch_tail<512, 32>(p, s);
+  if (channels == 512) return bm == 64 ? launch_tail<512, 64, 2>(p, s) : launch_tail<512, 32>(p, s);
   return CDSEG_ERR_UNSUPPORTED;
 }
diff --git a/cdsegnet_amd/engine.py b/cdsegnet_amd/engine.py
--- a/cdsegnet_amd/engine.py
+++ b/cdsegnet_amd/engine.py
@@ -148,6 +148,10 @@
             a, b = len(offs), len(offs) + len(offs_pad)
             self.set_pad(key, K, offs_pad, patch_start, up[:a], up[a:b], up[b:])
         return self._pad[key]
+
+    def attn_l2(self, patch_size, enable_flash):
+        K, n_pad, _, _, _, _, sum_l2 = self.pad(patch_size, enable_flash)
+        return sum_l2 - float(K) * (n_pad - self.n)
 
     def slots(self, curve, patch_size, enable_flash):
         lz = self._slot_lazy.pop((curve, patch_size, enable_flash), None) if self._slot_lazy else None
@@ -912,7 +916,7 @@
             att = mod.attn
             gidx, widx = lv.slots(st.curves[att.order_index], att.patch_size, att.enable_flash)
             _, _, _, _, patch_start, max_len, sum_l2 = lv.pad(att.patch_size, att.enable_flash)
-            self.attn_work += 64.0 * att.num_heads * sum_l2
+            self.attn_work += 64.0 * att.num_heads * lv.attn_l2(att.patch_size, att.enable_flash)
             self.attn_bytes += 4.0 * n * c * st.xc.element_size()
             self._count_conv(n, c, st.xc.element_size())
             desc = self.block_desc[pre]
@@ -959,7 +963,8 @@
         curve = st.curves[att.order_index]
         gidx, widx = lv.slots(curve, att.patch_size, att.enable_flash)
         _, _, _, _, patch_start, max_len, sum_l2 = lv.pad(att.patch_size, att.enable_flash)
-        self._add_work(64.0 * att.num_heads * sum_l2, 4.0 * n * c * qkv.element_size())
+        work = 64.0 * att.num_heads * lv.attn_l2(att.patch_size, att.enable_flash)
+        self._add_work(work, 4.0 * n * c * qkv.element_size())
         o = self._buf(n, c, self.T)
         if self.exact_attention_core and self.T != torch.float32:
             q32 = qkv.float()
@@ -971,7 +976,7 @@
             o.copy_(o32)
         else:
             ops.attention(qkv[:, :c], qkv[:, c:2 * c], qkv[:, 2 * c:], gidx, gidx, widx, patch_start, att.num_heads,
-                          max_len, att.scale, o, work=64.0 * att.num_heads * sum_l2, flags=aflags)
+                          max_len, att.scale, o, work=work, flags=aflags)
         hid = w[pre + ".fc1.w"].shape[0]
         if xs is not None:
             st.xc = self._buf(n, c, self.T)
@@ -1092,10 +1097,11 @@
         q_gidx, widx = lv.slots(nst.curves[att.order_index], K, att.enable_flash)
         kv_gidx, _ = clv.slots(cst.curves[att.order_index], K, att.enable_flash)
         _, _, _, _, patch_start, max_len, sum_l2 = lv.pad(K, att.enable_flash)
-        self._add_work(64.0 * att.num_heads * sum_l2, 4.0 * n * cq * q.element_size())
+        work = 64.0 * att.num_heads * lv.attn_l2(K, att.enable_flash)
+        self._add_work(work, 4.0 * n * cq * q.element_size())
         o = self._buf(n, cq, self.T)
         ops.attention(q, kv[:, :cq], kv[:, cq:], q_gidx, kv_gidx, widx, patch_start, att.num_heads, max_len, att.scale, o,
-                      work=64.0 * att.num_heads * sum_l2, flags=ops.ATTN_Q_PRESCALED if self.q_prescaled else 0)
+                      work=work, flags=ops.ATTN_Q_PRESCALED if self.q_prescaled else 0)
         if "x.tail_img" in w and n >= ops.DEEP512_MIN_ROWS:
             nst.xc = self._buf(n, cq, self.T)
             ops.attn_tail_rr(o, w["x.tail_img"], w["x.proj.b"], w["x.q_norm2.g"], w["x.q_norm2.b"], w["x.fc1.b"], w["x.fc2.b"],
@@ -1133,7 +1139,7 @@
             if c > 64 or self.T == torch.float32:
                 deep[0] += 2.0 * occ(lv, 3) * c * c
             out["linear"] += 2.0 * lv.n * (5.0 * c * c + 2.0 * c * hid)
-            out["attention"] += 64.0 * mod.attn.num_heads * lv.pad(mod.attn.patch_size, mod.attn.enable_flash)[6]
+            out["attention"] += 64.0 * mod.attn.num_heads * lv.attn_l2(mod.attn.patch_size, mod.attn.enable_flash)
 
         def stages(branch, cum, n_stages):
             for s in range(n_stages):
@@ -1159,7 +1165,7 @@
             out["conv"] += 2.0 * occ(lq, 3) * cq * cq + 2.0 * occ(lc, 3) * ck * ck
             deep[0] += 2.0 * occ(lq, 3) * cq * cq + 2.0 * occ(lc, 3) * ck * ck
             out["linear"] += 2.0 * lq.n * (cq * cq * 3 + 2.0 * cq * w["x.fc1.w"].shape[0]) + 2.0 * lc.n * (ck * ck + ck * 2 * cq)
-            out["attention"] += 64.0 * cb.attn.num_heads * lq.pad(cb.attn.q_patch_size, cb.attn.enable_flash)[6]
+            out["attention"] += 64.0 * cb.attn.num_heads * lq.attn_l2(cb.attn.q_patch_size, cb.attn.enable_flash)
         for s in reversed(range(bb.n_num_stages - 1)):
             lf, lc = plan.levels[plan.n_cum[s]], plan.levels[plan.n_cum[s + 1]]
             pre = f"n_dec{s}.up"
diff --git a/cdsegnet_amd/ops.py b/cdsegnet_amd/ops.py
--- a/cdsegnet_amd/ops.py
+++ b/cdsegnet_amd/ops.py
@@ -599,6 +599,7 @@
 
 
 DEEP512_MIN_ROWS = int(os.environ.get("CDSEG_DEEP512_MIN_ROWS", 2560))
+DEEP512_ROWS64_MIN = 256 * 32 + 1
 DEEP_CHANNELS = (128, 256, 512)
 
 
```
